# foolwood/SiamMask

Measured on AMD Instinct MI355X. Metric: frames/sec (255x255 search, 127x127 template), higher is better.
Workload: dtype f16

## Files before the change

siammask_amd/_lib.py:

```python
import ctypes
import os
import subprocess

import torch

_HERE = os.path.dirname(os.path.abspath(__file__))
LIB_PATH = os.environ.get("SMK_LIB") or os.path.join(_HERE, "libsiammask_hip.so")
CSRC = os.path.join(_HERE, "csrc")

DTYPE = {"f32": 0, "fp32": 0, "float32": 0, "f16": 1, "fp16": 1, "float16": 1, "half": 1,
         "f16x3": 2}
VARIANT = {"rpn": 0, "base": 1, "sharp": 2}
TRACK_BOX, TRACK_MASK, TRACK_NO_MASK_HEAD = 0, 1, 2
HP_STRIDE = 4

SYMBOLS = (
    "smk_version", "smk_last_error", "smk_create", "smk_destroy", "smk_set_weight",
    "smk_finalize_weights", "smk_template", "smk_track", "smk_refine", "smk_set_decode_params", "smk_decode", "smk_step", "smk_set_graph_mode", "smk_seq_status", "smk_seq_sync_check", "smk_set_result_ring", "smk_result_ring_cursor", "smk_set_pipeline", "smk_pipeline_join", "smk_pipeline_observe",
    "smk_debug_read", "smk_debug_seq_inject", "smk_tune", "smk_tune_get", "smk_profile", "smk_profile_dump", "smk_op_conv2d_ex", "smk_op_conv2d", "smk_op_dw_xcorr",
    "smk_op_maxpool3x3s2", "smk_op_stem_pool", "smk_op_l1_block", "smk_op_conv_seq", "smk_host_conv2d_ex", "smk_host_plan_conv", "smk_host_plan_seq", "smk_host_arena_elems", "smk_bench_conv", "smk_packed_size", "smk_export_packed",
    "smk_import_packed", "smk_crop_resize", "smk_paste_mask", "smk_paste_labels", "smk_mask_rbox_workspace", "smk_mask_rbox",
    "smk_trk_state_bytes", "smk_trk_set", "smk_trk_plan", "smk_trk_advance", "smk_crop_resize_dev", "smk_paste_mask_dev",
    "smk_vos_score", "smk_vos_score_dev", "smk_host_trk_plan", "smk_host_trk_advance",
    "smk_vos_score_ex", "smk_vos_score_dev_ex", "smk_label_rects", "smk_frame_sums", "smk_trk_start", "smk_crop_exemplar_dev",
    "smk_host_trk_start", "smk_vot_overlap", "smk_host_vot_overlap",
    "smk_crop_resize_dev_v", "smk_crop_exemplar_dev_v", "smk_frame_sums_v", "smk_trk_start_v", "smk_host_trk_start_v",
    "smk_paste_mask_dev_v", "smk_vot_overlap_dev",
    "smk_set_stream_hp", "smk_trk_advance_hp", "smk_host_trk_advance_hp",
)


class ConvGeom(ctypes.Structure):
    _fields_ = [(n, ctypes.c_int) for n in (
        "B", "Cin", "H", "W", "Cout", "k", "stride", "pad", "dil", "relu", "res_mode",
        "win", "ups", "Hl", "Wl", "org_y", "org_x", "pos_mul", "pos_add", "cin_off", "cin_len")]


class SeqOp(ctypes.Structure):
    _fields_ = [("g", ConvGeom), ("src", ctypes.c_int), ("res_src", ctypes.c_int), ("sync", ctypes.c_int),
                ("cfg", ctypes.c_int), ("kstag", ctypes.c_int), ("w_host", ctypes.c_void_p), ("b_host", ctypes.c_void_p),
                ("y_dev", ctypes.c_void_p)]


class TrkCfg(ctypes.Structure):
    _fields_ = [("context_amount", ctypes.c_double), ("lr", ctypes.c_double)] + [(n, ctypes.c_int) for n in (
        "exemplar_size", "instance_size", "total_stride", "base_size", "score_size", "mask_size")]


class ImageRef(ctypes.Structure):
    _fields_ = [("data", ctypes.c_void_p), ("row_bytes", ctypes.c_int64), ("w", ctypes.c_int32), ("h", ctypes.c_int32)]


class SmkError(RuntimeError):
    code = 0


E_SEQ = -6


def build_library(force=False, verbose=False):
    if force:
        subprocess.check_call(["make", "-C", CSRC, "clean"], stdout=subprocess.DEVNULL)
    out = subprocess.run(["make", "-C", CSRC, "-j", "4"], stdout=subprocess.PIPE,
                         stderr=subprocess.STDOUT, universal_newlines=True)
    if verbose or out.returncode != 0:
        print(out.stdout)
    if out.returncode != 0:
        raise SmkError("building libsiammask_hip.so failed")
    return LIB_PATH


_lib = None


def lib():
    global _lib
    if _lib is not None:
        return _lib
    if not os.path.exists(LIB_PATH):
        raise SmkError(
            "%s is missing: the HIP extension has not been built (run `python -c 'import "
            "__graft_entry__ as g; g.build()'` or `make -C siammask_amd/csrc`). There is no "
            "CPU fallback." % LIB_PATH)
    L = ctypes.CDLL(LIB_PATH)
    vp, ci, fp = ctypes.c_void_p, ctypes.c_int, ctypes.c_void_p
    L.smk_version.restype = ci
    L.smk_last_error.restype = ctypes.c_char_p
    L.smk_create.argtypes = [ctypes.POINTER(vp), ci, ci, ci, ci]
    L.smk_destroy.argtypes = [vp]
    L.smk_set_weight.argtypes = [vp, ctypes.c_char_p, fp, ctypes.POINTER(ctypes.c_int64), ci]
    L.smk_finalize_weights.argtypes = [vp]
    L.smk_template.argtypes = [vp, fp, ci, vp]
    L.smk_track.argtypes = [vp, fp, ci, ci, fp, fp, fp, vp]
    L.smk_refine.argtypes = [vp, vp, ci, ci, fp, vp]
    L.smk_set_decode_params.argtypes = [vp, fp, ci, ci, ctypes.c_double, ctypes.c_double]
    L.smk_decode.argtypes = [vp, fp, fp, ci, fp, vp, fp, vp]
    L.smk_step.argtypes = [vp, fp, ci, ci, fp, fp, fp, fp, fp, fp, vp]
    L.smk_set_graph_mode.argtypes = [vp, ci]
    L.smk_debug_seq_inject.argtypes = [vp, ci]
    L.smk_set_result_ring.argtypes = [vp, vp, vp, ci, ci]
    L.smk_set_pipeline.argtypes = [vp, ci]
    L.smk_pipeline_join.argtypes = [vp, vp]
    L.smk_pipeline_observe.argtypes = [vp, vp]
    L.smk_result_ring_cursor.argtypes = [vp, ctypes.POINTER(ci), ci, vp]
    L.smk_seq_sync_check.argtypes = [vp, vp, ctypes.POINTER(ci)]
    L.smk_tune.argtypes = [ctypes.c_char_p, ci]
    L.smk_tune_get.argtypes = [ctypes.c_char_p, ctypes.POINTER(ci)]
    L.smk_profile.argtypes = [vp, ci]
    L.smk_profile_dump.argtypes = [vp, ctypes.c_char_p, ci]
    ip = ctypes.POINTER(ci)
    L.smk_debug_read.argtypes = [vp, ctypes.c_char_p, fp, ip, ip, ip, vp]
    gp = ctypes.POINTER(ConvGeom)
    L.smk_op_conv2d_ex.argtypes = [ci, ci, gp, fp, fp, fp, fp, vp, fp, vp]
    L.smk_op_conv2d.argtypes = [ci, ci, fp, ci, ci, ci, ci, fp, fp, ci, ci, ci, ci, ci, ci, fp, fp, vp]
    L.smk_op_dw_xcorr.argtypes = [ci, fp, fp, ci, ci, ci, ci, ci, ci, fp, vp]
    L.smk_op_maxpool3x3s2.argtypes = [ci, fp, ci, ci, ci, ci, fp, vp]
    L.smk_op_stem_pool.argtypes = [fp, fp, fp, ci, ci, fp, fp, vp]
    L.smk_op_l1_block.argtypes = [fp] * 9 + [ci, ci, ci, fp, vp]
    L.smk_host_conv2d_ex.argtypes = [gp, fp, fp, fp, fp, vp, fp]
    L.smk_host_plan_conv.argtypes = [gp, ci, ci, ip, ip, ip, ip]
    L.smk_host_arena_elems.argtypes = [ci, ci, ci, ctypes.POINTER(ctypes.c_uint64)]
    L.smk_packed_size.argtypes = [vp, ctypes.POINTER(ctypes.c_uint64)]
    L.smk_export_packed.argtypes = [vp, vp, ctypes.c_uint64]
    L.smk_import_packed.argtypes = [vp, vp, ctypes.c_uint64]
    L.smk_crop_resize.argtypes = [vp, ctypes.c_int64, ci, ci, vp, vp, ci, ci, fp, vp]
    L.smk_paste_mask.argtypes = [fp, ci, vp, ci, ci, ci, ctypes.c_float, ctypes.c_float, vp, fp, vp]
    L.smk_paste_labels.argtypes = [fp, ci, vp, ci, ci, ci, ctypes.c_float, ctypes.c_float, vp, vp]
    L.smk_mask_rbox_workspace.argtypes = [ci, ci, ci]
    L.smk_mask_rbox.argtypes = [vp, ci, ci, ci, ctypes.c_double, vp, ctypes.c_size_t, vp, vp]
    cp = ctypes.POINTER(TrkCfg)
    L.smk_trk_state_bytes.argtypes = [ci]
    L.smk_trk_set.argtypes = [vp, ci, vp, vp, vp, ci, ci, vp]
    L.smk_trk_plan.argtypes = [vp, ci, cp, vp]
    L.smk_trk_advance.argtypes = [vp, ci, cp, vp, ci, vp, ci, vp]
    L.smk_host_trk_plan.argtypes = [vp, ci, cp]
    L.smk_host_trk_advance.argtypes = [vp, ci, cp, vp, ci, vp, ci]
    L.smk_crop_resize_dev.argtypes = [vp, ctypes.c_int64, ci, ci, vp, ci, ci, fp, vp]
    L.smk_paste_mask_dev.argtypes = [fp, fp, ci, ci, vp, ci, ci, ci, ci, ctypes.c_float, ctypes.c_float, vp, fp, vp]
    cf, u32 = ctypes.c_float, ctypes.c_uint32
    L.smk_vos_score.argtypes = [fp, ci, vp, ci, ci, ci, cf, vp, vp, u32, vp, ci, cf, vp, vp, vp]
    L.smk_vos_score_dev.argtypes = [fp, fp, ci, ci, vp, ci, ci, ci, ci, cf, vp, vp, u32, vp, ci, cf, vp, vp, vp]
    L.smk_vos_score_ex.argtypes = L.smk_vos_score.argtypes[:-1] + [u32, vp, vp]
    L.smk_vos_score_dev_ex.argtypes = L.smk_vos_score_dev.argtypes[:-1] + [u32, vp, vp]
    i64 = ctypes.c_int64
    L.smk_label_rects.argtypes = [vp, ci, ci, vp, ci, vp, vp]
    L.smk_frame_sums.argtypes = [vp, i64, ci, ci, ci, vp, vp]
    L.smk_trk_start.argtypes = [vp, ci, cp, u32, vp, vp, vp, vp, i64, ci, ci, vp, vp, vp]
    L.smk_host_trk_start.argtypes = [vp, ci, cp, u32, vp, vp, vp, vp, i64, ci, ci, vp, vp]
    L.smk_crop_exemplar_dev.argtypes = [vp, i64, ci, ci, vp, vp, vp, u32, ci, ci, fp, vp]
    L.smk_vot_overlap.argtypes = [vp, ci, vp, vp, ci, ci, ci, vp, vp, vp]
    L.smk_host_vot_overlap.argtypes = [vp, vp, ci, ci, ci, vp, vp]
    L.smk_crop_resize_dev_v.argtypes = [vp, vp, ci, ci, fp, vp]
    L.smk_crop_exemplar_dev_v.argtypes = [vp, vp, vp, vp, u32, ci, ci, fp, vp]
    L.smk_frame_sums_v.argtypes = [vp, ci, vp, vp]
    L.smk_trk_start_v.argtypes = [vp, ci, cp, u32, vp, vp, vp, vp, i64, vp, vp, vp, vp]
    L.smk_host_trk_start_v.argtypes = [vp, ci, cp, u32, vp, vp, vp, vp, i64, vp, vp, vp]
    L.smk_paste_mask_dev_v.argtypes = [fp, fp, ci, ci, vp, ci, ci, ci, ci, vp, cf, cf, vp, vp]
    L.smk_vot_overlap_dev.argtypes = [vp, ci, vp, vp, vp, ci, vp, vp, vp]
    L.smk_set_stream_hp.argtypes = [vp, vp]
    L.smk_trk_advance_hp.argtypes = [vp, ci, cp, vp, vp, ci, vp, ci, vp]
    L.smk_host_trk_advance_hp.argtypes = [vp, ci, cp, vp, vp, ci, vp, ci]
    L.smk_op_conv_seq.argtypes = [ctypes.POINTER(SeqOp), ci, fp, ci, ctypes.POINTER(ctypes.c_float), fp, ip, vp]
    L.smk_host_plan_seq.argtypes = [ctypes.POINTER(SeqOp), ci, ci, ip, ip, ip]
    L.smk_bench_conv.argtypes = [ci, ci, gp, ci, ci, ctypes.POINTER(ctypes.c_float), vp]
    for name in SYMBOLS:
        fn = getattr(L, name)
        if name not in ("smk_last_error",):
            fn.restype = ctypes.c_size_t if name in ("smk_mask_rbox_workspace", "smk_trk_state_bytes") else ci
    _lib = L
    for kv in filter(None, os.environ.get("SMK_TUNE", "").split(",")):
        k, v = kv.split("=")
        check(L.smk_tune(k.strip().encode(), int(v)))
    return L


def check(rc):
    if rc != 0:
        msg = lib().smk_last_error()
        e = SmkError("libsiammask_hip error %d: %s" % (rc, msg.decode() if msg else "?"))
        e.code = rc
        raise e


def current_stream_ptr():
    return ctypes.c_void_p(torch.cuda.current_stream().cuda_stream)


def tune(**kw):
    for k, v in kw.items():
        check(lib().smk_tune(k.encode(), int(v)))


def tune_get(key):
    v = ctypes.c_int(0)
    check(lib().smk_tune_get(key.encode(), ctypes.byref(v)))
    return v.value
```

siammask_amd/csrc/conv_plan.cpp:

```cpp
#include "conv_plan.h"

#include <algorithm>
#include <cstdio>
#include <cstdlib>
#include <cstring>

using namespace smk;

TileChoice tile_from_code(int code, const ConvParams &p, int dtype) {
    TileChoice t = choose_tile(p, dtype);
    static const int tb[6][2] = {{0, 0}, {128, 128}, {128, 64}, {64, 128}, {64, 64}, {256, 128}};
    const int tile = code & 15, kt = (code >> 4) & 3, st = (code >> 6) & 3;
    if (tile >= 1 && tile <= 5) {
        t.bm = tb[tile][0]; t.bn = tb[tile][1];
        t.kt = (t.bm == 64 && t.bn == 64) ? 256 : 128;
        t.stages = (t.bm == 128 && t.bn == 128) ? 2 : 3;
    }
    if (kt) t.kt = kt == 2 ? 256 : 128;
    if (t.bm == 64 && t.bn == 64) t.kt = 256;
    if (t.bm == 256) t.kt = 128;
    if (st) t.stages = st + 1;
    return t;
}

// ... 85 lines not shown
                (int)L[i].Kpad, (int)L[i].Nst, (int)L[i + 1].Nst, L[i].res, (int)L[i].relu, (int)L[i + 1].relu, (int)L[i + 1].Ho, (int)L[i + 1].Hs);
    return ok;
}
static bool seq_pair_fusable_why(const SeqLayer *L, int i, int *code, int *why) {
    const SeqLayer &a = L[i], &b = L[i + 1];
    auto plain1x1 = [](const SeqLayer &l) {
        return l.kh == 1 && l.kw == 1 && l.stride == 1 && l.stride_x == 1 && l.pad == 0 && l.org_y == 0 && l.org_x == 0 &&
               l.Hl == l.Hs && l.Wl == l.Ws && l.Ho == l.Hs && l.Wo == l.Ws && l.Ci == l.Kpad;
    };
    if (!plain1x1(a) || !a.sync) { *why = 1; return false; }
    if (!plain1x1(b)) { *why = 2; return false; }
    if (!a.res || a.res_mode != RES_PRE_RELU || !a.relu) { *why = 1; return false; }
    if (b.res || b.res_mode != RES_NONE) { *why = 3; return false; }
    if (b.in != a.out) { *why = 1; return false; }
    if (b.cin_off != a.cout_off || b.Cs != a.Cos || b.Ci != a.Nst || b.Hs != a.Ho || b.Ws != a.Wo) { *why = 4; return false; }
    if (b.out == a.out || b.out == a.res || b.out == a.in) { *why = 5; return false; }
    auto has_bar = [&](int k) { return L[k].sync && L[k].cfg != SEQ_CFG_C3C1_L3 && L[k].cfg != SEQ_CFG_C3C1_L2 && L[k].cfg != SEQ_CFG_C3C1P_L3 && L[k].cfg != SEQ_CFG_C3C1P_L2; };
    int pend = -1;
    for (int k = i - 1; k >= 0; --k)
        if (has_bar(k)) { pend = k; break; }
    for (int j = i - 1; j >= 0; --j)
        if (L[j].out == a.res) {
            bool passed = false;
            for (int k = j; k < pend; ++k) passed = passed || has_bar(k);
            if (!passed) { *why = 6; return false; }
            break;
        }
    for (int j = i - 1; j >= 0; --j)
        if (L[j].out == a.in) {
            if (j > pend) { *why = 7; return false; }
            break;
        }
    if (a.Kpad == 256 && a.Nst == 1024 && b.Nst == 256) *code = SEQ_CFG_C3C1_L3;
    else if (a.Kpad == 128 && a.Nst == 512 && b.Nst == 128) *code = SEQ_CFG_C3C1_L2;
    else { *why = 8; return false; }
    return true;
}

bool seq_pair_fits(const SeqLayer *L, int i, int B, int *code) {
    if (!seq_pair_fusable(L, i, code)) return false;
    const size_t px = (size_t)B * L[i].Ho * L[i].Wo;
    const size_t widest = std::max(std::max((size_t)L[i].Cs, (size_t)L[i].Cos), std::max((size_t)L[i].res_Cs, (size_t)L[i + 1].Cos));
    return px * widest * 2 < 0x7fff0000u && L[i].in_bytes < 0x7fff0000u;
}


static int seq_fuse_pairs(SeqLayer *L, int n, int B, const char *locked, bool have_xch) {
    if (!g_tune.seq_fuse) return 0;
    int fused = 0;
    for (int i = 0; i + 1 < n; ++i) {
        int code = 0;
        if (locked && (locked[i] || locked[i + 1])) continue;
        if (L[i].cfg >= SEQ_CFG_C3C1_L3 || L[i + 1].cfg >= SEQ_CFG_C3C1_L3 || !seq_pair_fits(L, i, B, &code)) continue;
        if (g_tune.seq_fuse == 2 && code != SEQ_CFG_C3C1_L3) continue;
        if (have_xch && g_tune.seq_pair2d && (g_tune.seq_pair2d == 1 || code == SEQ_CFG_C3C1_L3))
            code = code == SEQ_CFG_C3C1_L3 ? SEQ_CFG_C3C1P_L3 : SEQ_CFG_C3C1P_L2;
        L[i].cfg = (signed char)code;
        L[i + 1].cfg = (signed char)SEQ_CFG_C3C1_2ND;
        if (!(g_tune.seq_kstag_mask & 1)) L[i].kstag = 0;
        ++fused;
        ++i;
    }
    return fused;
}

static bool read_after_list(const std::vector<const void *> &read_after, const void *y) {
    return std::find(read_after.begin(), read_after.end(), y) != read_after.end();
}

static int seq_fuse_triples(SeqLayer *L, int i0, int i1, int n, const void *const *wstd, const char *locked,
                            const std::vector<const void *> &read_after) {
    if (!g_tune.seq_fuse3) return 0;
    auto group_has_bar = [&](int k) {
        const int cf = L[k].cfg;
        if (cf == SEQ_CFG_C3C1_L3 || cf == SEQ_CFG_C3C1_L2 || cf == SEQ_CFG_C3C1P_L3 || cf == SEQ_CFG_C3C1P_L2 || cf == SEQ_CFG_C2C3C1_L3 ||
            cf == SEQ_CFG_C2C3C1_L2 || cf == SEQ_CFG_C2C3C1_MID)
            return false;
        return L[k].sync != 0;
    };
    int fused = 0;
    for (int i = i0; i + 2 < i1; ++i) {
        SeqLayer &c2 = L[i], &c3 = L[i + 1], &c1 = L[i + 2];
        if (locked && (locked[i] || locked[i + 1] || locked[i + 2])) continue;
        if ((c3.cfg != SEQ_CFG_C3C1_L3 && c3.cfg != SEQ_CFG_C3C1_L2) || c1.cfg != SEQ_CFG_C3C1_2ND) continue;
        if (c2.cfg != SEQ_CFG_HALO128 && c2.cfg != SEQ_CFG_HALO64 && c2.cfg > 9) continue;
        const int code = c3.cfg == SEQ_CFG_C3C1_L3 ? SEQ_CFG_C2C3C1_L3 : SEQ_CFG_C2C3C1_L2;
        if (g_tune.seq_fuse3 == 2 && code != SEQ_CFG_C2C3C1_L3) continue;
        const int kc = c3.Kpad;
        if (c2.kh != 3 || c2.kw != 3 || c2.stride != 1 || c2.stride_x != 1 || c2.pad != c2.dil || c2.dil < 1 || c2.dil > 2) continue;
        if (c2.Ci != kc || c2.Nst != kc || c2.Kpad != 9 * kc || !c2.relu || c2.res || c2.res_mode != RES_NONE || !c2.sync) continue;
        if (c2.org_y || c2.org_x || c2.Hl != c2.Hs || c2.Wl != c2.Ws || c2.Ho != c2.Hs || c2.Wo != c2.Ws) continue;
        if (c2.Wo > 32 || c2.Wo < 24 || c2.Wo + 2 * c2.dil > 35) continue;
        if (c3.in != c2.out || c3.cin_off != c2.cout_off || c3.Cs != c2.Cos || c3.Hs != c2.Ho || c3.Ws != c2.Wo) continue;
        if (!wstd[i]) continue;
        bool other_reader = read_after_list(read_after, c2.out);
        for (int j = i + 2; j < n; ++j) {
            if (L[j].in == c2.out || L[j].res == c2.out) { other_reader = true; break; }
            if (L[j].out == c2.out) { other_reader = false; break; }
        }
        if (other_reader || c2.out == c3.res || c2.out == c1.out || c2.out == c3.out) continue;
        int pend = -1;
        for (int k = i - 1; k >= i0; --k)
            if (group_has_bar(k)) { pend = k; break; }
        bool in_ok = true;
        for (int j = i - 1; j >= i0; --j)
            if (L[j].out == c2.in) { in_ok = j <= pend; break; }
        if (!in_ok) continue;
        int res_late = 0;
        for (int j = i - 1; j >= i0; --j)
            if (L[j].out == c3.res) {
                bool passed = false;
                for (int k = j; k < pend; ++k) passed = passed || group_has_bar(k);
                const bool own_rows = L[j].cfg == SEQ_CFG_C2C3C1_MID && L[j].Ho == c3.Ho && L[j].Wo == c3.Wo;
                if (!passed && !own_rows) res_late = 1;
                break;
            }
        c2.cfg = (signed char)code;
        c2.wgt_frag = wstd[i];
        c2.sync = 0;
        c3.cfg = (signed char)SEQ_CFG_C2C3C1_MID;
        c3.a_stage = (signed char)res_late;
        ++fused;
        i += 2;
    }
    return fused;
}

static int seq_mark_resident(SeqLayer *L, int i0, int i1, int n, const SeqPlanEnv &env, const std::vector<const void *> &read_after) {
    if (!g_tune.seq_yres || env.B > 8) return 0;
    int prev = -1, marked = 0;
    for (int i = i0; i + 1 < i1; ++i) {
        const int cfg = L[i].cfg;
        if (cfg != SEQ_CFG_C3C1_L3 && cfg != SEQ_CFG_C3C1_L2) continue;
        const int p = prev;
        prev = i;
        if (p < 0 || L[p].cfg != cfg || i != p + 3) continue;
        const int mid = L[p + 2].cfg;
        if (mid != SEQ_CFG_HALO64 && mid != SEQ_CFG_HALO128) continue;
        if ((L[i].Ho * L[i].Wo + 31) / 32 > env.nslots || L[i].Ho != L[p].Ho || L[i].Wo != L[p].Wo) continue;
        if (L[i].res != L[p].out || L[i].res_Cs != L[p].Cos || L[i].res_coff != L[p].cout_off) continue;
        L[i].a_stage |= SEQ_YRES_IN;
        L[p + 2].a_stage |= SEQ_LDS_HI;
        ++marked;
        bool others = read_after_list(read_after, L[p].out);
        for (int j = 0; j < n && !others; ++j) {
            if (j != p + 1 && L[j].in == L[p].out) others = true;
            if (j != i && L[j].res == L[p].out) others = true;
        }
        if (!others) L[p].a_stage |= SEQ_YRES_NOSTORE;
    }
    return marked;
}

SeqPlanStats plan_seq(std::vector<SeqRec> &rec, const SeqPlanEnv &env, const char *locked, const std::vector<const void *> &read_after) {
    const int n = (int)rec.size();
    std::vector<SeqLayer> L(n);
    std::vector<const void *> wstd(n);
    for (int i = 0; i < n; ++i) { L[i] = rec[i].L; wstd[i] = rec[i].wstd; }
    const bool xch = env.have_xch && env.nslots % 2 == 0 && env.nslots / 2 <= SEQ_XCH_PAIRS;
    SeqPlanStats st;
    for (int i0 = 0; i0 < n; i0 += SEQ_MAX) {
        const int i1 = std::min(n, i0 + SEQ_MAX);
        st.pairs = seq_fuse_pairs(L.data() + i0, i1 - i0, env.B, locked ? locked + i0 : nullptr, xch);
        st.triples = seq_fuse_triples(L.data(), i0, i1, n, wstd.data(), locked, read_after);
        st.resident = seq_mark_resident(L.data(), i0, i1, n, env, read_after);
    }
    for (int i = 0; i < n; ++i) rec[i].L = L[i];
    return st;
}

double seq_fabric_bytes(const SeqLayer *L, int n, int B, const void *late_read) {
    double ext = 0.0;
    for (int i = 0; i < n; ++i) {
        const SeqLayer &l = L[i];
        bool in_inside = false, res_inside = l.res == nullptr, out_read = false;
        for (int j = 0; j < n; ++j) {
            if (j < i && L[j].out == l.in) in_inside = true;
            if (j < i && l.res && L[j].out == l.res) res_inside = true;
            if (j > i && (L[j].in == l.out || L[j].res == l.out)) out_read = true;
        }
        bool in_counted = false, res_counted = false;
        for (int j = 0; j < i; ++j) {
            if (L[j].in == l.in || L[j].res == l.in) in_counted = true;
            if (l.res && (L[j].in == l.res || L[j].res == l.res)) res_counted = true;
        }
        const double px_in = (double)B * l.Hs * l.Ws, px_out = (double)B * l.Ho * l.Wo;
        ext += (double)l.Nst * l.Kpad * 2.0;
        if (!in_inside && !in_counted) ext += px_in * l.Cs * 2.0;
        if (!res_inside && !res_counted) ext += px_out * l.res_Cs * 2.0;
        if (!out_read || l.out == late_read) ext += px_out * l.Nst * 2.0;
    }
    return ext;
}

const int WREG_TILE[9][2] = {{0, 0}, {64, 256}, {64, 128}, {64, 64}, {128, 256}, {128, 128}, {128, 64}, {96, 256}, {32, 64}};
int wreg_choice(const ConvParams &p, const ConvOpt &o, int dtype, long ncu) {
    if (o.algo_naive || !conv_wreg_eligible(p, dtype)) return 0;
    if (o.wreg) return o.wreg;
    if (g_tune.wreg >= 2) return g_tune.wreg - 1;
    if (!g_tune.wreg) return 0;
    const long K = (long)p.kh * p.kw * p.Ci;
    if (g_tune.wreg_policy == 1) {
        if (p.kh > 3) return 0;
        if (p.kh == 3 && p.stride == 1 && K <= 1152) return 0;
        if (p.M > 16384 && !(p.Nst >= 512 || (K >= 2304 && p.Nst >= 128) || (K >= 1024 && p.Nst >= 256) ||
                             (p.kh == 3 && p.stride == 2)))
            return 0;
        static const int cand[4] = {4, 1, 2, 3};
        const int nr = (p.Nst + 63) / 64 * 64, ng = p.groups > 0 ? p.groups : 1;
        for (int ci = 0; ci < 4; ++ci) {
            const int bm = WREG_TILE[cand[ci]][0], bn = WREG_TILE[cand[ci]][1];
            if (bn > nr && bn > 64) continue;
            if ((long)((p.M + bm - 1) / bm) * ((p.Nst + bn - 1) / bn) * ng >= 150) {
                if (cand[ci] == 4 && g_tune.wreg96) {
                    const long tn = (p.Nst + 255) / 256 * ng;
                    const long t128 = (long)((p.M + 127) / 128) * tn, t96 = (long)((p.M + 95) / 96) * tn;
                    if (((t128 + ncu - 1) / ncu) * 128 > ((t96 + ncu - 1) / ncu) * 96 && t96 <= 4 * ncu) return 7;
                }
                return cand[ci];
            }
        }
        if (g_tune.wreg32 && (long)((p.M + 63) / 64) * ((p.Nst + 63) / 64) * ng < g_tune.wreg32) return 8;
        return 3;
    }
    if (p.M < 4096) return 0;
    if (p.kh == 3 && K >= 2304 && p.Nst >= 512)
        return ((long)((p.M + 127) / 128) * ((p.Nst + 255) / 256) >= 200) ? 4 : 1;
    if (p.M > 16384) return 0;
    if (p.kh == 1 && K >= 512 && p.Nst <= 256) return p.Nst >= 192 ? 2 : 3;
    if (p.kh == 3 && p.stride == 2 && K >= 1152 && p.Nst <= 128) return 3;
    return 0;
}
int wreg_stages(int ctx_dtype, int B) {
    if (g_tune.wreg_stages) return g_tune.wreg_stages;
    return (ctx_dtype == DT_F16X3 || (B >= 1 && B <= 2)) ? 4 : 3;
}
int wreg_stages_from_code(int code) {
    const int st = (code >> 6) & 3;
    return st == 0 ? wreg_stages(DT_F16, 0) : (st == 1 ? 8 : (st == 2 ? 3 : 4));
}

bool pp_choice(const ConvParams &p, const ConvOpt &o, int dtype, long ncu) {
    if (!g_tune.pp || o.algo_naive || o.halo || o.wreg || o.tile_code || !conv_pp_eligible(p, dtype)) return false;
    const long K = (long)p.kh * p.kw * p.Ci;
    const long tiles = (long)((p.M + 255) / 256) * ((p.Nst + 255) / 256);
    const long rounds = (tiles + ncu - 1) / ncu;
    if (tiles < 200 || tiles * 10 < rounds * ncu * 9 || p.Nst < 256 || (p.Nst % 256) != 0) return false;
    return g_tune.pp == 2 || K >= 2304;
}

ConvPlan plan_conv(const ConvParams &p, const ConvOpt &o, const PackedConv &pc, int dtype, int B, long ncu) {
    const int kd = kdtype(dtype);
    ConvPlan pl;
    pl.tile = tile_from_code(o.tile_code, p, kd);
    if (o.algo_naive) { pl.kind = CK_NAIVE; return pl; }
    if (dtype == DT_F16 && g_tune.chain_mask != 2 && !o.tile_code && !o.halo && !o.wreg && mask_head_eligible(p, kd)) { pl.kind = CK_MHEAD; return pl; }
    int bm = halo_choice(pc, p, o, kd);
    if (bm && !o.halo && conv_ksplit(p, kd, pl.tile) > 1) bm = 0;
    if (pp_choice(p, o, kd, ncu)) { pl.kind = CK_PP; return pl; }
    const int wr = (o.halo || (bm && !o.wreg && g_tune.wreg < 2 && g_tune.wreg_policy == 0)) ? 0 : wreg_choice(p, o, kd, ncu);
    if (wr) {
        pl.kind = CK_WREG; pl.wreg = wr; pl.stages = wreg_stages(dtype, B);
    } else if (bm && conv_halo_eligible(p, kd, bm)) {
        pl.kind = CK_HALO; pl.halo_bm = bm;
    }
    return pl;
}

ConvPlan plan_conv_batch(const ConvBatch &cb, const ConvOpt *const o[], int lead, int dtype, int B, long ncu) {
    const int kd = kdtype(dtype);
    ConvPlan pl;
    int wr = wreg_choice(cb.p[lead], *o[lead], kd, ncu);
    for (int i = 0; i < cb.n && wr; ++i)
        if (!wreg_choice(cb.p[i], *o[i], kd, ncu) || (cb.p[i].groups > 1) != (cb.p[0].groups > 1)) wr = 0;
    if (wr) {
        pl.kind = CK_WREG; pl.wreg = wr; pl.stages = wreg_stages(dtype, B);
    } else {
        pl.tile = tile_from_code(o[lead]->tile_code, cb.p[lead], kd);
    }
    return pl;
}

std::string plan_kernel_name(const ConvPlan &pl, int dtype, int out_mode, int merged) {
    const char *dt = dtname(kdtype(dtype));
    char kn[80], mg[16] = "";
    if (merged) snprintf(mg, sizeof(mg), ",merged%d", merged);
    switch (pl.kind) {
    case CK_NAIVE: return "conv_naive";
    case CK_PP: return "conv_pp<f16,256x256>";
    case CK_MHEAD: return "mask_head<f16,128px,nchw>";
    case CK_HALO: snprintf(kn, sizeof(kn), "conv3x3_halo<%s,%dx128>", dt, pl.halo_bm); break;
    case CK_WREG: snprintf(kn, sizeof(kn), "conv_wreg<%s,%dx%d,s%d%s>", dt, WREG_TILE[pl.wreg][0], WREG_TILE[pl.wreg][1], pl.stages, mg); break;
    default:
        snprintf(kn, sizeof(kn), "conv_igemm<%s,%dx%dx%d,s%d,%s%s>", dt, pl.tile.bm, pl.tile.bn, pl.tile.kt, pl.tile.stages,
                 out_mode == OUT_NCHW_F32 ? "nchw" : "nhwc", mg);
    }
    return kn;
}
```

siammask_amd/csrc/conv_plan.h:

```cpp
#pragma once
#include <string>
#include <vector>

#include "smk_kernels.h"

struct Act {
    void *p = nullptr;
    int H = 0, W = 0, C = 0;
};

struct PackedConv {
    void *w = nullptr;
    void *w_halo = nullptr;
    void *w_frag = nullptr;
    void *w_frag_halo = nullptr;
    void *w_frag16 = nullptr;
    float *bias = nullptr;
    int N = 0;
    int rows = 0;
    int group_rows = 0;
    int groups = 1;
    int Ci = 0, k = 1, K = 0, Kpad = 0;
    int kw = 0;
    int alg_k = 0;
    float *oscale = nullptr;
    int x3_ct = 0, x3_nreal = 0;
    bool x3 = false;
};

struct ConvOpt {
    int stride = 1, pad = 0, dil = 1, relu = 0;
    int stride_x = 0;
    const Act *res = nullptr;
    int res_mode = smk::RES_NONE;
    int res_coff = 0;
    int cin_off = 0;
    int cout_off = 0;
    int n_override = 0;
    int groups = 1;
    bool win = false;
    int Hl = 0, Wl = 0, org_y = 0, org_x = 0;
    const int *pos = nullptr;
    int pos_mul = 0, pos_add = 0;
    bool ups = false;
    float *nchw_out = nullptr;
    int algo_naive = 0;
    int tile_code = 0;
    int halo = 0;
    int wreg = 0;
};

inline int kdtype(int dtype) { return dtype == smk::DT_F16X3 ? smk::DT_F16 : dtype; }
inline const char *dtname(int dt) { return dt == smk::DT_F16 ? "f16" : "f32"; }

#pragma GCC visibility push(hidden)

enum ConvKernel { CK_NAIVE, CK_IGEMM, CK_HALO, CK_WREG, CK_PP, CK_MHEAD };
struct ConvPlan {
    int kind = CK_IGEMM;
    smk::TileChoice tile{};
    int halo_bm = 0;
    int wreg = 0;
    int stages = 0;
};

extern const int WREG_TILE[9][2];

smk::TileChoice tile_from_code(int code, const smk::ConvParams &p, int dtype);
int halo_choice(const PackedConv &pc, const smk::ConvParams &p, const ConvOpt &o, int dtype);
int wreg_choice(const smk::ConvParams &p, const ConvOpt &o, int dtype, long ncu);
int wreg_stages(int ctx_dtype, int B);
int wreg_stages_from_code(int code);
bool pp_choice(const smk::ConvParams &p, const ConvOpt &o, int dtype, long ncu);

ConvPlan plan_conv(const smk::ConvParams &p, const ConvOpt &o, const PackedConv &pc, int dtype, int B, long ncu);
ConvPlan plan_conv_batch(const smk::ConvBatch &cb, const ConvOpt *const *o, int lead, int dtype, int B, long ncu);
std::string plan_kernel_name(const ConvPlan &pl, int dtype, int out_mode, int merged = 0);

bool seq_halo_ok(const smk::ConvParams &p, int bm);
bool seq_layer_from(const smk::ConvParams &p, int dtype, smk::SeqLayer &L, int force_halo = 0);
bool seq_pair_fusable(const smk::SeqLayer *L, int i, int *code);
bool seq_pair_fits(const smk::SeqLayer *L, int i, int B, int *code);

struct SeqRec {
    smk::SeqLayer L;
    const void *wstd = nullptr;
    std::string id;
};
struct SeqPlanEnv {
    int B = 0;
    int nslots = 0;
    bool have_xch = false;
};
struct SeqPlanStats { int pairs = 0, triples = 0, resident = 0; };

SeqPlanStats plan_seq(std::vector<SeqRec> &rec, const SeqPlanEnv &env, const char *locked, const std::vector<const void *> &read_after);
double seq_fabric_bytes(const smk::SeqLayer *L, int n, int B, const void *late_read);

#pragma GCC visibility pop
```

siammask_amd/csrc/conv_seq.hip:

```cpp
#include <hip/hip_runtime.h>
#include <type_traits>
#include "smk_kernels.h"

namespace smk {

#include "wreg_tile.inc"
#include "c3c1_tile.inc"
#ifdef SMK_MEASURE
#include "c3c1p_tile.inc"
#endif
#include "c3c1s_tile.inc"
#include "wreg_halo_tile.inc"

#ifndef SMK_HALO_D128
#define SMK_HALO_D128 3
#endif
#ifndef SMK_HALO_SB128
#define SMK_HALO_SB128 0
#endif
constexpr int HALO_D128 = SMK_HALO_D128, HALO_SB128 = SMK_HALO_SB128, HALO_D64 = 6;
constexpr int SEQ_POLL_TID = 256;
constexpr int SEQ_CLK2_STRIDE = 12;

__device__ __forceinline__ void seq_raise(const SeqArgs &a, int code) {
    __hip_atomic_store(a.err, code, __ATOMIC_RELAXED, __HIP_MEMORY_SCOPE_AGENT);
    if (a.err_host) __hip_atomic_store(a.err_host, code, __ATOMIC_RELAXED, __HIP_MEMORY_SCOPE_SYSTEM);
}

__device__ __forceinline__ void team_arrive(unsigned *cnt) {
    asm volatile("s_waitcnt vmcnt(0) lgkmcnt(0)" ::: "memory");
    __builtin_amdgcn_s_barrier();
    asm volatile("" ::: "memory");
    if (threadIdx.x == SEQ_POLL_TID)
        __hip_atomic_fetch_add(cnt, 1u, __ATOMIC_RELAXED, __HIP_MEMORY_SCOPE_WORKGROUP);
}

__device__ __forceinline__ unsigned team_poll(const unsigned *cnt, bool spoll) {
    if (spoll) {
        unsigned v;
        asm volatile("s_load_dword %0, %1, 0x0 glc\n\ts_waitcnt lgkmcnt(0)" : "=s"(v) : "s"(cnt) : "memory");
        return v;
    }
    return __hip_atomic_load(cnt, __ATOMIC_RELAXED, __HIP_MEMORY_SCOPE_AGENT);
}

struct TeamWait {
    const SeqArgs *a;
    unsigned *cnt;
    unsigned target;
    int *abort_sh;
    __device__ __forceinline__ bool operator()() const {
        if (target == 0) return true;
        if (threadIdx.x == SEQ_POLL_TID) {
            const unsigned long long t0 = wall_clock64();
            while (team_poll(cnt, (a->flags & 1) != 0) < target) {
                __builtin_amdgcn_s_sleep(1);
                if (wall_clock64() - t0 > 20000000ull) {
                    seq_raise(*a, 2);
                    *abort_sh = 1;
                    break;
                }
            }
        }
        asm volatile("s_waitcnt lgkmcnt(0)" ::: "memory");
        __builtin_amdgcn_s_barrier();
        asm volatile("" ::: "memory");
        return *(__attribute__((address_space(3))) volatile int *)abort_sh == 0;
    }
};

template <int NPW, int CLK = 0, int T3 = 0>
__global__ __launch_bounds__((4 + NPW) * 64, 1) void conv_seq_kernel(const SeqArgs a) {
    constexpr int SEQ_LDS0 = (!T3 || WregLds<4, 3>::v > C3C1Lds<256, 1024, 256>::vx) ? WregLds<4, 3>::v : C3C1Lds<256, 1024, 256>::vx;
    constexpr int SEQ_LDS = SEQ_LDS0 > SEQ_YRES_BYTES + 2 * HALO_PB ? SEQ_LDS0 : SEQ_YRES_BYTES + 2 * HALO_PB;
    static_assert(4 * 64 * 68 * 4 <= 2 * HALO_PB && C3C1Lds<256, 1024, 256>::A_OFF == SEQ_YRES_BYTES && C3C1Lds<128, 512, 128>::A_OFF <= SEQ_YRES_BYTES, "resident Y");
    __shared__ __attribute__((aligned(16))) unsigned char smem[SEQ_LDS];
    static_assert(C3C1Lds<256, 1024, 256>::v <= WregLds<4, 3>::v && C3C1Lds<128, 512, 128>::vx <= SEQ_LDS && SEQ_LDS + 64 <= 160 * 1024, "LDS of the fused tiles");
    static_assert(NPW == 4, "c3c1_tile computes on all eight waves");
    __shared__ int ctl[4];
    const int nslots = gridDim.x >> 3;
    unsigned xcc;
    asm volatile("s_getreg_b32 %0, hwreg(HW_REG_XCC_ID)" : "=s"(xcc));
    const int team = (int)(xcc & 7);
    unsigned *cnt = a.bar + team * 32;
    if (threadIdx.x == 0) {
        const unsigned t = __hip_atomic_fetch_add(cnt + 2, 1u, __ATOMIC_RELAXED, __HIP_MEMORY_SCOPE_WORKGROUP);
        const int e = __hip_atomic_load(a.err, __ATOMIC_RELAXED, __HIP_MEMORY_SCOPE_AGENT);
        ctl[0] = (int)t;
        ctl[1] = e;
        ctl[2] = 0;
    }
    __syncthreads();
    const int slot = ctl[0];
    if (ctl[1]) return;
    if (slot >= nslots) {
        if (threadIdx.x == 0) seq_raise(a, 1);
        return;
    }
    unsigned pending = 0;
    const bool clk = CLK != 0 && a.clk && team == 0 && slot == 0 && threadIdx.x == 0;
    if (clk) a.clk[0] = wall_clock64();
    bool alive = true;
    for (int li = 0; li < a.n && alive; ++li) {
        const SeqLayer &L = a.L[li];
        const int cfg = L.cfg;
        const bool fusedp = cfg == SEQ_CFG_C3C1P_L3 || cfg == SEQ_CFG_C3C1P_L2;
        const bool fused = cfg == SEQ_CFG_C3C1_L3 || cfg == SEQ_CFG_C3C1_L2;
        const bool fused3 = cfg == SEQ_CFG_C2C3C1_L3 || cfg == SEQ_CFG_C2C3C1_L2;
        const bool halo = cfg == SEQ_CFG_HALO128 || cfg == SEQ_CFG_HALO64;
        const int bn = (cfg == 0 || cfg == 3 || cfg == 16 || cfg == 17) ? 256 : ((cfg == 2 || cfg == 9 || cfg == 18) ? 64 : 128);
        const int bm = (cfg == 3 || cfg == 4 || cfg == 9 || cfg == 16) ? 128 : 64;
        const int tilesN = (L.Nst + bn - 1) / bn;
        const int hw = L.Ho * L.Wo;
        const int halo_rpt = halo ? (cfg == SEQ_CFG_HALO128 ? 128 : 64) / L.Wo : 1;
        const int halo_tn = (L.Nst + 63) >> 6;
        const int tiles = fused3 ? L.Ho : fused ? (hw + 31) / 32 : (halo ? ((L.Ho + halo_rpt - 1) / halo_rpt) * halo_tn : ((hw + bm - 1) / bm) * tilesN);
#ifdef SMK_MEASURE
        if (T3 != 0 && fusedp) {
            const int npairs = nslots >> 1, pr = slot >> 1, hcu = slot & 1;
            int rt = (hw + npairs - 1) / npairs;
            if (rt > 64) rt = 64;
            const int ptiles = (hw + rt - 1) / rt;
            float *slabs = (float *)((unsigned char *)a.xch + (size_t)((team * SEQ_XCH_PAIRS + pr) * 4) * SEQ_XCH_SLAB);
            for (int img = team; img < a.B && alive; img += 8)
                for (int t = pr; t < ptiles && alive; t += npairs) {
                    unsigned long long *tclk = nullptr;
                    if constexpr (CLK != 0)
                        tclk = (a.clk2 && team == 0 && slot == 0 && img == team && t == pr) ? a.clk2 + SEQ_CLK2_STRIDE * li : nullptr;
                    const TeamWait w{&a, cnt, pending, &ctl[2]};
                    pending = 0;
                    const int fm0 = img * hw + t * rt;
                    int fme = fm0 + rt;
                    if (fme > (img + 1) * hw) fme = (img + 1) * hw;
                    if constexpr (T3 != 0) {
                    if (cfg == SEQ_CFG_C3C1P_L3)
                        alive = c3c1p_tile<256, 1024, 256, CLK>(L, a.L[li + 1], fm0, fme, a.B * hw, hcu, pr, npairs, cnt + 8 + pr, slabs, a, &ctl[2], &ctl[3], smem, tclk, w);
                    else
                        alive = c3c1p_tile<128, 512, 128, CLK>(L, a.L[li + 1], fm0, fme, a.B * hw, hcu, pr, npairs, cnt + 8 + pr, slabs, a, &ctl[2], &ctl[3], smem, tclk, w);
                    }
                }
        } else
#endif
        {
        const int nk = L.Kpad >> 6;
        const int kt0 = L.kstag ? (slot * nk) / nslots : 0;
        for (int img = team; img < a.B && alive; img += 8)
            for (int t = slot; t < tiles && alive; t += nslots) {
                const int tm = t / tilesN, tn = t - tm * tilesN;
                const int m0 = img * hw + tm * bm, m_end = (img + 1) * hw;
                unsigned long long *tclk = nullptr;
                if constexpr (CLK != 0)
                    tclk = (a.clk2 && team == 0 && slot == 0 && img == team && t == slot) ? a.clk2 + SEQ_CLK2_STRIDE * li : nullptr;
                const TeamWait w{&a, cnt, pending, &ctl[2]};
                pending = 0;
                if constexpr (T3 != 0)
                if (fused3) {
                    const int fm0 = img * hw + t * L.Wo;
                    if (cfg == SEQ_CFG_C2C3C1_L3) alive = c3c1_tile<256, 1024, 256, CLK, TeamWait, 1>(a.L[li + 1], a.L[li + 2], fm0, fm0 + L.Wo, a.B * hw, slot, nslots, smem, tclk, w, &L, img, t);
                    else alive = c3c1_tile<128, 512, 128, CLK, TeamWait, 1>(a.L[li + 1], a.L[li + 2], fm0, fm0 + L.Wo, a.B * hw, slot, nslots, smem, tclk, w, &L, img, t);
                }
                if (T3 != 0 && fused3) {}
                else if (fused) {
                    const int fm0 = img * hw + t * 32;
                    if (cfg == SEQ_CFG_C3C1_L3) alive = c3c1_tile<256, 1024, 256, CLK>(L, a.L[li + 1], fm0, m_end, a.B * hw, slot, nslots, smem, tclk, w);
                    else alive = c3c1_tile<128, 512, 128, CLK>(L, a.L[li + 1], fm0, m_end, a.B * hw, slot, nslots, smem, tclk, w);
                }
                else if (halo) {
                    const int ty = t / halo_tn, hn0 = (t - ty * halo_tn) * 64;
                    const bool hi = (L.a_stage & SEQ_LDS_HI) != 0;
                    unsigned char *hsm = smem + (hi ? SEQ_YRES_BYTES : 0);
                    if (cfg == SEQ_CFG_HALO128) alive = wreg_halo_tile<4, NPW, HALO_D128, HALO_SB128, CLK>(L, img, ty, hn0, hsm, tclk, slot, nslots, w, hi);
                    else alive = wreg_halo_tile<2, NPW, HALO_D64, 0, CLK>(L, img, ty, hn0, hsm, tclk, slot, nslots, w, hi);
                }
                else if (cfg == 0) alive = wreg_tile<2, 4, 1, 3, 16, 2, NPW, CLK>(L, 0, m0, m_end, tn * 256, smem, tclk, kt0, w);
                else if (cfg == 1) alive = wreg_tile<2, 2, 2, 3, 16, 2, NPW, CLK>(L, 0, m0, m_end, tn * 128, smem, tclk, kt0, w);
                else if (cfg == 3) alive = wreg_tile<4, 4, 1, 3, 16, 1, NPW, CLK>(L, 0, m0, m_end, tn * 256, smem, tclk, kt0, w);
                else if (cfg == 4) alive = wreg_tile<4, 2, 2, 3, 16, 1, NPW, CLK>(L, 0, m0, m_end, tn * 128, smem, tclk, kt0, w);
                else if (T3 != 0 && cfg == 9) { if constexpr (T3 != 0) alive = wreg_tile<4, 1, 4, 3, 16, 2, NPW, CLK>(L, 0, m0, m_end, tn * 64, smem, tclk, kt0, w); }
                else if (T3 != 0 && cfg == 5) { if constexpr (T3 != 0) alive = wreg_tile<2, 2, 2, 5, 16, 4, NPW, CLK>(L, 0, m0, m_end, tn * 128, smem, tclk, kt0, w); }
#ifdef SMK_MEASURE
                else if (cfg == 6) alive = wreg_tile<2, 2, 2, 3, 16 | 0x100, 2, NPW, CLK>(L, 0, m0, m_end, tn * 128, smem, tclk, kt0, w);
                else if (cfg == 7) alive = wreg_tile<2, 2, 2, 3, 16 | 0x200, 2, NPW, CLK>(L, 0, m0, m_end, tn * 128, smem, tclk, kt0, w);
                else if (cfg == 8) alive = wreg_tile<2, 2, 2, 3, 16 | 0x400, 2, NPW, CLK>(L, 0, m0, m_end, tn * 128, smem, tclk, kt0, w);
                else if (cfg == 10) alive = wreg_tile<2, 2, 2, 3, 16 | 0x300, 2, NPW, CLK>(L, 0, m0, m_end, tn * 128, smem, tclk, kt0, w);
                else if (cfg == 11) alive = wreg_tile<2, 2, 2, 3, 16 | 0x700, 2, NPW, CLK>(L, 0, m0, m_end, tn * 128, smem, tclk, kt0, w);
                else if (cfg == 12) alive = wreg_tile<2, 2, 2, 3, 16 | 0x1700, 2, NPW, CLK>(L, 0, m0, m_end, tn * 128, smem, tclk, kt0, w);
                else if (cfg == 13) alive = wreg_tile<2, 2, 2, 3, 16 | 0x800, 2, NPW, CLK>(L, 0, m0, m_end, tn * 128, smem, tclk, kt0, w);
                else if (cfg == 14) alive = wreg_tile<2, 2, 2, 3, 16 | 0x1000, 2, NPW, CLK>(L, 0, m0, m_end, tn * 128, smem, tclk, kt0, w);
                else if (cfg == 15) alive = wreg_tile<2, 2, 2, 3, 16 | 0x2000, 2, NPW, CLK>(L, 0, m0, m_end, tn * 128, smem, tclk, kt0, w);
                else if (cfg == 16) alive = wreg_tile<4, 4, 1, 3, 16 | 0x2000, 1, NPW, CLK>(L, 0, m0, m_end, tn * 256, smem, tclk, kt0, w);
                else if (cfg == 17) alive = wreg_tile<2, 4, 1, 3, 16 | 0x2000, 2, NPW, CLK>(L, 0, m0, m_end, tn * 256, smem, tclk, kt0, w);
                else if (cfg == 18) alive = wreg_tile<2, 1, 4, 3, 16 | 0x2000, 2, NPW, CLK>(L, 0, m0, m_end, tn * 64, smem, tclk, kt0, w);
#endif
                else alive = wreg_tile<2, 1, 4, 3, 16, 2, NPW, CLK>(L, 0, m0, m_end, tn * 64, smem, tclk, kt0, w);
            }
        }
        if (clk) a.clk[1 + 2 * li] = wall_clock64();
        if (!alive) break;
        if (fused3) {
            if (clk) a.clk[2 + 2 * li] = a.clk[3 + 2 * li] = a.clk[4 + 2 * li] = a.clk[5 + 2 * li] = wall_clock64();
            li += 2;
        }
        if (fused || fusedp) {
            if (clk) a.clk[2 + 2 * li] = a.clk[3 + 2 * li] = wall_clock64();
            ++li;
        }
        if (a.L[li].bar_ord) {
            if (pending) {
                const TeamWait w{&a, cnt, pending, &ctl[2]};
                pending = 0;
                if (!w()) break;
            }
            team_arrive(cnt);
            if constexpr (CLK != 0) {
                if (a.clk2 && team == 0 && threadIdx.x == 0) a.clk2[SEQ_CLK2_STRIDE * SEQ_MAX + li * 32 + slot] = wall_clock64();
            }
            pending = (unsigned)a.L[li].bar_ord * (unsigned)nslots;
        }
        if (clk) a.clk[2 + 2 * li] = wall_clock64();
    }
    if (!alive || ctl[2]) return;
    asm volatile("s_waitcnt vmcnt(0) lgkmcnt(0)" ::: "memory");
    __syncthreads();
    if (threadIdx.x == 0) {
        const unsigned prev = __hip_atomic_fetch_add(cnt + 1, 1u, __ATOMIC_RELAXED, __HIP_MEMORY_SCOPE_WORKGROUP);
        if (prev == (unsigned)nslots - 1) {
            __hip_atomic_store(cnt, 0u, __ATOMIC_RELAXED, __HIP_MEMORY_SCOPE_WORKGROUP);
            __hip_atomic_store(cnt + 1, 0u, __ATOMIC_RELAXED, __HIP_MEMORY_SCOPE_WORKGROUP);
            __hip_atomic_store(cnt + 2, 0u, __ATOMIC_RELAXED, __HIP_MEMORY_SCOPE_WORKGROUP);
            for (int i = 8; i < 32; ++i) __hip_atomic_store(cnt + i, 0u, __ATOMIC_RELAXED, __HIP_MEMORY_SCOPE_WORKGROUP);
            if (a.exit_sem) {
                const unsigned t = __hip_atomic_fetch_add(a.exit_sem + 1, 1u, __ATOMIC_RELAXED, __HIP_MEMORY_SCOPE_AGENT);
                if (t == 7u) {
                    __hip_atomic_store(a.exit_sem + 1, 0u, __ATOMIC_RELAXED, __HIP_MEMORY_SCOPE_AGENT);
                    __hip_atomic_fetch_add(a.exit_sem, 1u, __ATOMIC_RELAXED, __HIP_MEMORY_SCOPE_AGENT);
                }
            }
        }
    }
}

template <int K3, int N3, int N1>
__global__ __launch_bounds__(512, 1) void conv_pair_kernel(const SeqLayer L3, const SeqLayer L1, const int M) {
    __shared__ __attribute__((aligned(16))) unsigned char smem[C3C1Lds<K3, N3, N1>::v];
    const int m0 = (int)blockIdx.x * 32;
    (void)c3c1_tile<K3, N3, N1, 0>(L3, L1, m0, M, M, (int)(blockIdx.x & 31), 32, smem, nullptr, NoHoist());
}

template <int K3, int N3, int N1>
__global__ __launch_bounds__(512, 1) void conv_pair64_kernel(const SeqLayer L3, const SeqLayer L1, const int M) {
    __shared__ __attribute__((aligned(16))) unsigned char smem[C3C1SLds<K3, N3, N1>::v];
    c3c1s_tile<K3, N3, N1>(L3, L1, (int)blockIdx.x * 64, M, M, smem);
}

int launch_conv_pair(const SeqLayer &L3, const SeqLayer &L1, int code, int M, void *stream, int rows) {
    if (M < 1 || (code != SEQ_CFG_C3C1_L3 && code != SEQ_CFG_C3C1_L2) || (rows != 32 && rows != 64)) return -1;
    if (rows == 64) {
        const dim3 grid64((M + 63) / 64), block64(512);
        if (code == SEQ_CFG_C3C1_L3) hipLaunchKernelGGL((conv_pair64_kernel<256, 1024, 256>), grid64, block64, 0, (hipStream_t)stream, L3, L1, M);
        else hipLaunchKernelGGL((conv_pair64_kernel<128, 512, 128>), grid64, block64, 0, (hipStream_t)stream, L3, L1, M);
        return hipGetLastError() == hipSuccess ? 0 : -4;
    }
    const dim3 grid((M + 31) / 32), block(512);
    if (code == SEQ_CFG_C3C1_L3) hipLaunchKernelGGL((conv_pair_kernel<256, 1024, 256>), grid, block, 0, (hipStream_t)stream, L3, L1, M);
    else hipLaunchKernelGGL((conv_pair_kernel<128, 512, 128>), grid, block, 0, (hipStream_t)stream, L3, L1, M);
    return hipGetLastError() == hipSuccess ? 0 : -4;
}

__global__ void xcc_census_kernel(int *out) {
    unsigned xcc;
    asm volatile("s_getreg_b32 %0, hwreg(HW_REG_XCC_ID)" : "=s"(xcc));
    if (threadIdx.x == 0) out[blockIdx.x] = (int)(xcc & 0xf);
}

int launch_conv_seq(const SeqArgs &a_in, int grid, void *stream) {
    if (a_in.n < 1 || a_in.n > SEQ_MAX || grid < 8 || (grid & 7) || !a_in.bar || !a_in.err) return -1;
    SeqArgs a = a_in;
    unsigned short ord = 0;
    for (int li = 0; li < a.n; ++li) {
        const int cfg = a.L[li].cfg;
        a.L[li].bar_ord = 0;
        const bool first = cfg == SEQ_CFG_C3C1_L3 || cfg == SEQ_CFG_C3C1_L2 || cfg == SEQ_CFG_C3C1P_L3 || cfg == SEQ_CFG_C3C1P_L2;
        if (cfg == SEQ_CFG_C2C3C1_L3 || cfg == SEQ_CFG_C2C3C1_L2) {
            if (li + 2 >= a.n) return -1;
            if (a.L[li + 1].cfg != SEQ_CFG_C2C3C1_MID || a.L[li + 2].cfg != SEQ_CFG_C3C1_2ND) return -1;
            if (a.L[li].Wo + 2 * a.L[li].dil > 35 || a.L[li].Wo > 32) return -1;
            continue;
        }
        if (cfg == SEQ_CFG_C2C3C1_MID) {
            const int pc = li ? a.L[li - 1].cfg : -1;
            if (pc != SEQ_CFG_C2C3C1_L3 && pc != SEQ_CFG_C2C3C1_L2) return -1;
            continue;
        }
        if (first) {
            if (li + 1 >= a.n || a.L[li + 1].cfg != SEQ_CFG_C3C1_2ND) return -1;
            if ((cfg == SEQ_CFG_C3C1P_L3 || cfg == SEQ_CFG_C3C1P_L2) && (!a.xch || (grid >> 3) % 2 || (grid >> 4) > SEQ_XCH_PAIRS)) return -1;
            continue;
        }
        if (cfg == SEQ_CFG_C3C1_2ND) {
            const int pc = li ? a.L[li - 1].cfg : -1;
            if (pc != SEQ_CFG_C3C1_L3 && pc != SEQ_CFG_C3C1_L2 && pc != SEQ_CFG_C3C1P_L3 && pc != SEQ_CFG_C3C1P_L2 && pc != SEQ_CFG_C2C3C1_MID) return -1;
        }
        if (a.L[li].sync && li + 1 < a.n) a.L[li].bar_ord = ++ord;
    }
    bool triples = false;
    for (int li = 0; li < a.n; ++li) {
        const int cf = a.L[li].cfg;
        triples = triples || cf == SEQ_CFG_C2C3C1_L3 || cf == SEQ_CFG_C2C3C1_L2 || cf == SEQ_CFG_C3C1P_L3 || cf == SEQ_CFG_C3C1P_L2 || cf == 5 || cf == 9;
    }
    if (triples) {
#ifdef SMK_MEASURE
        if (a.clk || a.clk2) hipLaunchKernelGGL((conv_seq_kernel<4, 1, 1>), dim3(grid), dim3(512), 0, (hipStream_t)stream, a);
        else hipLaunchKernelGGL((conv_seq_kernel<4, 0, 1>), dim3(grid), dim3(512), 0, (hipStream_t)stream, a);
#else
        return -5;
#endif
    } else if (a.clk || a.clk2)
        hipLaunchKernelGGL((conv_seq_kernel<4, 1>), dim3(grid), dim3(512), 0, (hipStream_t)stream, a);
    else hipLaunchKernelGGL((conv_seq_kernel<4, 0>), dim3(grid), dim3(512), 0, (hipStream_t)stream, a);
    return hipGetLastError() == hipSuccess ? 0 : -4;
}

int conv_seq_occupancy() {
    int nb = 0;
    if (hipOccupancyMaxActiveBlocksPerMultiprocessor(&nb, conv_seq_kernel<4, 0>, 512, 0) != hipSuccess) return 0;
    return nb;
}

int xcc_census(int grid, int *out_host) {
    int *d = nullptr;
    if (hipMalloc((void **)&d, sizeof(int) * grid) != hipSuccess) return -4;
    hipLaunchKernelGGL(xcc_census_kernel, dim3(grid), dim3(384), 0, 0, d);
    hipError_t e = hipMemcpy(out_host, d, sizeof(int) * grid, hipMemcpyDeviceToHost);
    hipFree(d);
    return e == hipSuccess ? 0 : -4;
}

}
```

siammask_amd/csrc/engine.cpp:

```cpp
#include <hip/hip_runtime_api.h>

#include <cmath>
#include <cstdarg>
#include <tuple>
#include <cstdio>
#include <cstdlib>
#include <cstring>
#include <functional>
#include <map>
#include <memory>
#include <string>
#include <vector>

#include "../../include/siammask_hip.h"
#include "../../include/siammask_hip_test.h"
#include "conv_plan.h"
#include "smk_kernels.h"
#include "tracker_state.h"
#include "vot_overlap.h"

using namespace smk;

static thread_local std::string g_err;

// ... 614 lines not shown
    HIPCHK(hipMemset(c->buf[id][copy], 0, bytes));
    return 0;
}

static int alloc_copies(smk_ctx *c, int depth) {
    for (int id = 0; id < T_COUNT; ++id)
        if (ARENA[id].twice_from && depth >= ARENA[id].twice_from && !c->buf[id][1]) CHK(alloc_buf(c, id, 1));
    return 0;
}

static int build_arena(smk_ctx *c) {
    uint64_t total = 0;
    CHK(arena_elems(c->dtype, c->variant, 0, &total));
    for (int id = 0; id < T_COUNT; ++id) {
        const ArenaRow &t = ARENA[id];
        if (t.refine && c->variant != SMK_VARIANT_SHARP) continue;
        if (row_aliased(t, c->dtype)) c->buf[id][0] = c->buf[t.alias][0];
        else CHK(alloc_buf(c, id, 0));
    }
    HIPCHK(hipMalloc((void **)&c->pos_dev, sizeof(int) * 2 * c->maxB));
    HIPCHK(hipMemset(c->pos_dev, 0, sizeof(int) * 2 * c->maxB));
    HIPCHK(hipMalloc((void **)&c->ks_part, KS_PART_FLOATS * sizeof(float)));
    HIPCHK(hipMalloc((void **)&c->ks_cnt, KS_CNT * sizeof(unsigned)));
    HIPCHK(hipMalloc((void **)&c->seq_bar, 8 * 32 * sizeof(unsigned)));
    HIPCHK(hipMemset(c->seq_bar, 0, 8 * 32 * sizeof(unsigned)));
    HIPCHK(hipMalloc((void **)&c->seq_err, sizeof(int)));
    HIPCHK(hipMemset(c->seq_err, 0, sizeof(int)));
    if (c->dtype == DT_F16) {
        HIPCHK(hipMalloc((void **)&c->seq_xch, SEQ_XCH_BYTES));
        HIPCHK(hipMemset(c->seq_xch, 0, SEQ_XCH_BYTES));
    }
    HIPCHK(hipHostMalloc((void **)&c->seq_err_host, 64, hipHostMallocMapped));
    *c->seq_err_host = 0;
    HIPCHK(hipHostGetDevicePointer((void **)&c->seq_err_hdev, c->seq_err_host, 0));
    HIPCHK(hipMemset(c->ks_cnt, 0, KS_CNT * sizeof(unsigned)));
    HIPCHK(hipMalloc(&c->dec_scratch, (size_t)c->maxB * DEC_SCRATCH_PER_STREAM));
    HIPCHK(hipMemset(c->dec_scratch, 0, (size_t)c->maxB * DEC_SCRATCH_PER_STREAM));
    return 0;
}

static int act(Act &a, smk_ctx *c, int id, int H = 0, int W = 0) {
    const ArenaRow &t = ARENA[id];
    const bool second = c->parity_now && t.twice_from && (t.twice_from == 1 || c->pipe_depth >= t.twice_from);
    a.p = c->buf[id][second ? 1 : 0];
    a.H = H > 0 ? H : t.H;
    a.W = H > 0 ? W : t.W;
    a.C = t.C * (t.per_branch ? nbranch(c) : 1) * ((c->dtype == DT_F16X3 && !t.refine) ? X3_PLANES : 1);
    if (!a.p || a.W < 1 || (size_t)a.H * a.W > (size_t)t.H * t.W)
        return fail(SMK_E_STATE, "internal: view %d x %d of arena tensor %s (%d x %d, copy %d)", a.H, a.W, t.name, t.H, t.W, (int)second);
    return 0;
}
#define ACT(...) ({ Act a_; CHK(act(a_, __VA_ARGS__)); a_; })
static int branch_off(const smk_ctx *c, int g) { return g * 256 * (c->dtype == DT_F16X3 ? X3_PLANES : 1); }

struct ConvEnv {
    int dtype = DT_F32, device = 0;
    float *ks_part = nullptr;
    unsigned *ks_cnt = nullptr;
    int wave_prio = 0;
};
static ConvEnv conv_env(const smk_ctx *c) { return {c->dtype, c->device, c->ks_part, c->ks_cnt, c->wave_prio_now}; }

static int conv_params(const ConvEnv &env, const PackedConv &pc, const Act &in, const Act *out, int B,
                       const ConvOpt &o, ConvParams &p) {
    memset(&p, 0, sizeof(p));
    p.in = in.p;
    p.wgt = pc.w;
    p.wgt_frag = pc.w_frag;
    p.wgt_frag_halo = pc.w_frag_halo;
    p.bias = pc.bias;
    p.oscale = pc.oscale;
    p.pos = o.pos;
    p.B = B;
    p.Hs = in.H; p.Ws = in.W; p.Cs = in.C;
    p.cin_off = o.cin_off;
    p.Ci = pc.Ci;
    p.x3_ct = pc.x3_ct; p.x3_nreal = pc.x3_nreal;
    p.x3_in = pc.x3 ? pc.Ci / 3 : 0;
    p.Hl = (o.win || o.ups) ? o.Hl : in.H;
    p.Wl = (o.win || o.ups) ? o.Wl : in.W;
    p.org_y = o.org_y; p.org_x = o.org_x;
    p.pos_mul = o.pos_mul; p.pos_add = o.pos_add;
    p.ups = o.ups ? 1 : 0;
    p.kh = pc.k;
    p.kw = pc.kw ? pc.kw : pc.k;
    p.stride = o.stride; p.pad = o.pad; p.dil = o.dil;
    p.stride_x = o.stride_x ? o.stride_x : o.stride;
    p.Ho = (p.Hl + 2 * o.pad - o.dil * (p.kh - 1) - 1) / p.stride + 1;
    p.Wo = (p.Wl + 2 * o.pad - o.dil * (p.kw - 1) - 1) / p.stride_x + 1;
    p.K = pc.K; p.Kpad = pc.Kpad;
    p.N = o.n_override ? o.n_override : pc.N;
    p.M = B * p.Ho * p.Wo;
    p.relu = o.relu;
    p.groups = o.groups;
    if (o.groups > 1) {
        p.g_cin_off = pc.x3 ? pc.Ci / 3 * X3_PLANES : pc.Ci;
        p.g_wgt_off = pc.group_rows;
        p.g_cout_off = pc.group_rows * (pc.x3 ? X3_PLANES : 1);
    }
    if (o.nchw_out) {
        p.out = o.nchw_out;
        p.out_mode = OUT_NCHW_F32;
        p.Nst = rup(p.N, 4);
    } else {
        if (!out) return fail(SMK_E_ARG, "conv without output");
        if (out->H != p.Ho || out->W != p.Wo)
            return fail(SMK_E_ARG, "internal: conv output %dx%d != buffer %dx%d", p.Ho, p.Wo, out->H, out->W);
        p.out = out->p;
        p.out_mode = OUT_NHWC;
        p.Cos = out->C;
        p.cout_off = o.cout_off;
        p.Nst = rup(p.N, 8);
        if (pc.x3) {
            p.x3_out = o.groups > 1 ? pc.group_rows : out->C / X3_PLANES;
            if (out->C % X3_PLANES || o.cout_off + (o.groups - 1) * X3_PLANES * pc.group_rows + p.x3_out + p.Nst > out->C)
                return fail(SMK_E_ARG, "internal: split conv output channels exceed buffer");
        } else if (o.cout_off + (o.groups - 1) * pc.group_rows + p.Nst > out->C)
            return fail(SMK_E_ARG, "internal: conv output channels exceed buffer");
    }
    p.xcd_mode = g_tune.xcd_mode;
    if (o.nchw_out && g_tune.nchw_tn_major && p.xcd_mode == 1 && p.M >= 20000 && (double)p.M * p.N * 4 >= 4.0e6) p.xcd_mode = 2;
    p.prio = g_tune.prio;
    p.wave_prio = env.wave_prio;
    {
        const double ib = (double)B * in.H * in.W * in.C * esize(env.dtype), wb = (double)pc.rows * pc.Kpad * esize(env.dtype);
        p.buf_lds = (g_tune.buf_lds && ib < 2.0e9 && wb < 2.0e9) ? 1 : 0;
        p.a_stage = g_tune.a_stage;
        p.res_nt = g_tune.res_nt;
        p.in_bytes = (unsigned)(ib < 4.0e9 ? ib : 0);
        p.w_bytes = (unsigned)(wb < 4.0e9 ? wb : 0);
    }
    p.nt_store = (g_tune.nt_store && o.nchw_out && (double)p.M * p.N * 4 >= 4.0e6) ? 1 : 0;
    p.ci_shift = -1;
    for (int sh = 0; sh < 16; ++sh)
        if ((1 << sh) == p.Ci) p.ci_shift = sh;
    p.kw_magic = 65536 / p.kw + 1;
    p.zero = env.device >= 0 ? zero_page() : nullptr;
    if (env.device >= 0 && !p.zero) return fail(SMK_E_HIP, "could not allocate the zero page");
    if (o.res) {
        p.res = o.res->p;
        p.res_Cs = o.res->C;
        p.res_coff = o.res_coff;
        p.res_mode = o.res_mode;
        if (pc.x3) p.x3_res = o.res->C / X3_PLANES;
    }
    p.ksplit = 1;
    p.ks_part = env.ks_part;
    p.ks_cnt = env.ks_cnt;
    p.ks_part_cap = env.ks_part ? KS_PART_FLOATS : 0;
    p.ks_cnt_cap = env.ks_cnt ? KS_CNT : 0;
    return 0;
}

static SeqPlanStats g_seq_last;

static void seq_print_clk(const SeqArgs &a, const SeqRec *r, const char *idn, const unsigned long long *h,
                          const unsigned long long *h2) {
    fprintf(stderr, "[seq clk] %s total %.2f us\n", idn, (h[2 * a.n] - h[0]) / 100.0);
    for (int i = 0; i < a.n; ++i)
        fprintf(stderr, "[seq clk]   %-10s cfg %d sync %d kstag %d  tiles %.2f us  arrive %.2f us\n", r[i].id.c_str(), a.L[i].cfg,
                a.L[i].sync, a.L[i].kstag, (h[1 + 2 * i] - h[2 * i]) / 100.0, (h[2 + 2 * i] - h[1 + 2 * i]) / 100.0);
    if (!h2) return;
    for (int i = 0; i < a.n; ++i) {
        const unsigned long long *ar = h2 + 12 * SEQ_MAX + 32 * i;
        unsigned long long mn = ~0ull, mx = 0;
        int nz = 0;
        double sum = 0.0;
        for (int q = 0; q < 32; ++q)
            if (ar[q]) { mn = std::min(mn, ar[q]); mx = std::max(mx, ar[q]); ++nz; }
        if (nz < 2) continue;
        for (int q = 0; q < 32; ++q)
            if (ar[q]) sum += (double)(mx - ar[q]);
        unsigned long long rel = 0;
        for (int j = i + 1; j < a.n && !rel; ++j) rel = h2[12 * j + 7];
        fprintf(stderr, "[seq arrive] %-10s %2d workgroups: first -> last arrival %.2f us, mean wait for the last one %.2f us, last arrival -> slot 0 "
                "released %.2f us\n", r[i].id.c_str(), nz, (mx - mn) / 100.0, sum / nz / 100.0, rel > mx ? (rel - mx) / 100.0 : -1.0);
    }
    for (int i = 0; i < a.n; ++i) {
        const unsigned long long *t = h2 + 12 * i;
        if (!t[0] || !t[6]) continue;
        const double us = (t[6] - t[0]) / 100.0;
        if (a.L[i].cfg == SEQ_CFG_C3C1P_L3 || a.L[i].cfg == SEQ_CFG_C3C1P_L2) {
            fprintf(stderr, "[seq clk2]  %-10s first tile (pair split, fused with the next 1x1): team wait %.2f | activation rows -> LDS %.2f | "
                    "conv3 K loop %.2f | residual -> Y %.2f | Y = relu(..) %.2f | Y stores + second K loop + slab + arrive %.2f | partner wait + add %.2f | "
                    "stores %.2f us | %.0f MHz\n",
                    r[i].id.c_str(), (t[7] - t[0]) / 100.0, (t[1] - t[7]) / 100.0, (t[2] - t[1]) / 100.0, (t[3] - t[2]) / 100.0,
                    (t[4] - t[3]) / 100.0, (t[5] - t[4]) / 100.0, (t[10] - t[5]) / 100.0, (t[6] - t[10]) / 100.0, us > 0 ? (double)(t[9] - t[8]) / us : 0.0);
            continue;
        }
        if (a.L[i].cfg == SEQ_CFG_C2C3C1_L3 || a.L[i].cfg == SEQ_CFG_C2C3C1_L2) {
            fprintf(stderr, "[seq clk2]  %-10s first tile (3x3 + conv3 + the next 1x1): prologue + team wait %.2f | patch -> LDS + conv2 %.2f | "
                    "conv3 K loop %.2f | residual -> Y %.2f | Y = relu(..) %.2f | Y stores + second K loop %.2f | its epilogue + stores %.2f us | %.0f MHz\n",
                    r[i].id.c_str(), (t[7] - t[0]) / 100.0, (t[1] - t[7]) / 100.0, (t[2] - t[1]) / 100.0, (t[3] - t[2]) / 100.0,
                    (t[4] - t[3]) / 100.0, (t[5] - t[4]) / 100.0, (t[6] - t[5]) / 100.0, us > 0 ? (double)(t[9] - t[8]) / us : 0.0);
            continue;
        }
        if (a.L[i].cfg == SEQ_CFG_C3C1_L3 || a.L[i].cfg == SEQ_CFG_C3C1_L2) {
            fprintf(stderr, "[seq clk2]  %-10s first tile (fused with the next 1x1): team wait %.2f | activation rows -> LDS %.2f | "
                    "conv3 K loop %.2f | residual -> Y %.2f | Y = relu(..) %.2f | Y stores + second K loop %.2f | its epilogue + stores %.2f us | %.0f MHz\n",
                    r[i].id.c_str(), (t[7] - t[0]) / 100.0, (t[1] - t[7]) / 100.0, (t[2] - t[1]) / 100.0, (t[3] - t[2]) / 100.0,
                    (t[4] - t[3]) / 100.0, (t[5] - t[4]) / 100.0, (t[6] - t[5]) / 100.0, us > 0 ? (double)(t[9] - t[8]) / us : 0.0);
            continue;
        }
        fprintf(stderr, "[seq clk2]  %-10s first tile: prologue %.2f | team wait %.2f | first operands %.2f | K loop %.2f | other waves %.2f | "
                "acc -> LDS %.2f | bias/res/stores %.2f | end sync %.2f us | %.0f MHz\n", r[i].id.c_str(),
                t[7] ? (t[7] - t[0]) / 100.0 : 0.0, 0.0, t[7] ? (t[1] - t[7]) / 100.0 : (t[1] - t[0]) / 100.0, (t[2] - t[1]) / 100.0,
                (t[3] - t[2]) / 100.0, (t[4] - t[3]) / 100.0, (t[5] - t[4]) / 100.0, (t[6] - t[5]) / 100.0,
                us > 0 ? (double)(t[9] - t[8]) / us : 0.0);
    }
}

static int seq_flush(smk_ctx *c, StepRec &rec, int B, hipStream_t s) {
    const size_t n = c->seq.rec.size();
    if (!n) return 0;
    const void *p2 = ACT(c, T_P2).p;
    std::vector<const void *> read_after{p2};
    for (int id : {c->p3_id, (int)T_SEARCH, (int)T_ZF, (int)T_XS}) read_after.push_back(ACT(c, id).p);
    g_seq_last = plan_seq(c->seq.rec, {B, c->seq_grid >> 3, c->seq_xch != nullptr}, nullptr, read_after);
    for (size_t i0 = 0; i0 < n; i0 += SEQ_MAX) {
        SeqArgs a;
        memset(&a, 0, sizeof(a));
        a.n = (int)(n - i0 < (size_t)SEQ_MAX ? n - i0 : SEQ_MAX);
        a.B = B;
        a.flags = g_tune.seq_spoll ? 1 : 0;
        a.bar = c->seq_bar;
        a.xch = c->seq_xch;
        a.err = c->seq_err;
        a.err_host = c->seq_err_hdev;
        a.exit_sem = (rec.seq_exit && i0 + SEQ_MAX >= n) ? c->pipe_cnt + 7 : nullptr;
        if (a.exit_sem) rec.seq_exit_done = true;
        const SeqRec *r = c->seq.rec.data() + i0;
        for (int i = 0; i < a.n; ++i) a.L[i] = r[i].L;
        const char *ck = getenv("SMK_SEQ_CLK");
        const bool want_clk = ck != nullptr && !c->graph_mode;
        const bool want_clk2 = want_clk && !strcmp(ck, "2");
        if (want_clk && !c->seq_clk) HIPCHK(hipMalloc((void **)&c->seq_clk, sizeof(unsigned long long) * (2 * SEQ_MAX + 1)));
        if (want_clk2 && !c->seq_clk2) HIPCHK(hipMalloc((void **)&c->seq_clk2, sizeof(unsigned long long) * (12 + 32) * SEQ_MAX));
        if (want_clk2) HIPCHK(hipMemsetAsync(c->seq_clk2, 0, sizeof(unsigned long long) * (12 + 32) * SEQ_MAX, s));
        a.clk = want_clk ? c->seq_clk : nullptr;
        a.clk2 = want_clk2 ? c->seq_clk2 : nullptr;
        char idn[96];
        snprintf(idn, sizeof(idn), "seq[%s..%s]", r[0].id.c_str(), r[a.n - 1].id.c_str());
        const double fr = (double)a.n / (double)n;
        ProfScope ps(c, s, idn, "conv_seq", c->seq.flop * fr, c->seq.bytes * fr);
        ps.ext_bytes(seq_fabric_bytes(a.L, a.n, B, p2));
        if (launch_conv_seq(a, c->seq_grid, s))
            return fail(SMK_E_HIP, "launch of %s failed: %s", idn, hipGetErrorString(hipGetLastError()));
        c->seq_pending = rec.has_seq = true;
        if (want_clk) {
            unsigned long long h[2 * SEQ_MAX + 1], h2[(12 + 32) * SEQ_MAX];
            HIPCHK(hipStreamSynchronize(s));
            HIPCHK(hipMemcpy(h, c->seq_clk, sizeof(h), hipMemcpyDeviceToHost));
            if (want_clk2) HIPCHK(hipMemcpy(h2, c->seq_clk2, sizeof(h2), hipMemcpyDeviceToHost));
            seq_print_clk(a, r, idn, h, want_clk2 ? h2 : nullptr);
        }
    }
    c->seq.clear();
    return 0;
}

static int seq_health(smk_ctx *c) {
    if (!c->seq_err_host) return 0;
    const int e = *(volatile int *)c->seq_err_host;
    if (!e) return 0;
    (void)hipDeviceSynchronize();
    c->seq_fail = e;
    if (e != 3) c->seq_grid = 0;
    else c->pipe_depth = 0;
    if (c->pipe_cnt) {
        const unsigned init[16] = {1u, 0u};
        (void)hipMemcpy(c->pipe_cnt, init, sizeof(init), hipMemcpyHostToDevice);
    }
    *(volatile int *)c->seq_err_host = 0;
    (void)hipMemset(c->seq_err, 0, sizeof(int));
    (void)hipMemset(c->seq_bar, 0, 8 * 32 * sizeof(unsigned));
    for (auto &kv : c->graphs) hipGraphExecDestroy(kv.second);
    c->graphs.clear();
    c->graph_used.clear();
    c->graph_has_seq.clear();
    c->seq_pending = false;
    c->tail_pending = false;
    c->tail2_pending = false;
    c->template_B = 0;
    c->track_B = 0;
    if (e == 3)
        return fail(SMK_E_SEQ, "conv_seq_kernel reported: (pipelined step) a gate waited 0.2 s (a tail's gate: 5 s) for its partner on the other stream -- something serialises "
                    "the two queues of this context (a profiler collecting counters does); the results of the calls enqueued on this context "
                    "since then are invalid (the cached template included) and frame steps are serial from here on: call template() again and "
                    "re-submit the frame");
    return fail(SMK_E_SEQ, "conv_seq_kernel reported %s: the results of the calls enqueued on this context since then are invalid "
                "(the cached template included); persistent sequences are now off for this context (per-layer kernels from here "
                "on): call template() again and re-submit the frame",
                e == 1 ? "an uneven distribution of workgroups over the XCDs" : "a team-barrier time-out (another kernel held CUs "
                "for more than 0.2 s, or a second persistent kernel ran beside it)");
}

static bool seq_wanted(const smk_ctx *c, int B) {
    if (!g_tune.seq || c->seq_grid <= 0 || c->dtype != DT_F16) return false;
    if (B >= g_tune.seq_min_batch && B <= g_tune.seq_max_batch) return true;
    if (B == g_tune.seq_extra_batch) return true;
    return B % 8 == 0 && B <= g_tune.seq_mult_max;
}

static void conv_work(const PackedConv &pc, const ConvParams &p, int B, int dtype, double &flop, double &bytes) {
    const int ng = p.groups > 0 ? p.groups : 1;
    const double kreal = pc.alg_k ? (double)pc.alg_k : (double)p.kh * p.kw * p.Ci;
    const size_t es = esize(kdtype(dtype));
    flop += 2.0 * p.M * (double)p.N * kreal * ng;
    bytes += (double)B * (p.ups ? p.Hs * p.Ws : (double)p.Hl * p.Wl) * p.Ci * es * ng + (double)p.M * p.N * ng * (p.out_mode == OUT_NCHW_F32 ? 4 : es) +
             (double)p.N * kreal * es * ng + (p.res ? (double)p.M * p.N * es : 0.0);
}

static int launch_plan(const ConvPlan &pl, ConvBatch &cb, const void *w_halo, int dtype, hipStream_t s, const char *what) {
    int rc;
    switch (pl.kind) {
    case CK_PP: rc = launch_conv_pp(cb.p[0], s); break;
    case CK_WREG: rc = launch_conv_wreg_batch(cb, WREG_TILE[pl.wreg][0], WREG_TILE[pl.wreg][1], pl.stages, s); break;
    case CK_HALO: {
        ConvParams ph = cb.p[0];
        ph.wgt = w_halo;
        rc = launch_conv_halo(ph, dtype, pl.halo_bm, s);
        break;
    }
    case CK_NAIVE: rc = launch_conv_naive(cb.p[0], dtype, s); break;
    case CK_MHEAD: rc = launch_mask_head(cb.p[0], s); break;
    default: rc = launch_conv_mfma_batch(cb, dtype, pl.tile, s);
    }
    if (rc == 1) return fail(SMK_E_STATE, "internal: %s is not eligible for the kernel planned for it", what);
    if (rc) return fail(SMK_E_HIP, "launch of %s failed: %s", what, hipGetErrorString(hipGetLastError()));
    return 0;
}

static int run_conv(smk_ctx *c, const char *id, const Act &in, const Act *out, int B, const ConvOpt &o,
                    hipStream_t s, StepRec *rec = nullptr) {
    auto it = c->conv.find(id);
    if (it == c->conv.end()) return fail(SMK_E_STATE, "internal: conv %s not packed", id);
    ConvBatch cb;
    cb.n = 1;
    ConvParams &p = cb.p[0];
    CHK(conv_params(conv_env(c), it->second, in, out, B, o, p));
    double flop = 0.0, bytes = 0.0;
    conv_work(it->second, p, B, c->dtype, flop, bytes);
    if (c->seq_on) {
        SeqLayer L;
        if (!o.algo_naive && !o.halo && !o.wreg && !o.tile_code && seq_layer_from(p, kdtype(c->dtype), L)) {
            c->seq.rec.push_back({L, p.wgt_frag, id});
            c->seq.flop += flop;
            c->seq.bytes += bytes;
            return 0;
        }
        if (!rec) return fail(SMK_E_STATE, "internal: conv %s recorded into a sequence without a step record", id);
        CHK(seq_flush(c, *rec, B, s));
    }
    const ConvPlan pl = plan_conv(p, o, it->second, c->dtype, B, c->ncu);
    ProfScope ps(c, s, id, plan_kernel_name(pl, c->dtype, p.out_mode), flop, bytes);
    char what[80];
    snprintf(what, sizeof(what), "conv %s", id);
    return launch_plan(pl, cb, it->second.w_halo, kdtype(c->dtype), s, what);
}

struct ConvJob { const char *id; const Act *in; const Act *out; ConvOpt o; };

static int run_conv_jobs(smk_ctx *c, const std::vector<ConvJob> &jobs, int B, int lead, hipStream_t s, StepRec *rec = nullptr) {
    if (jobs.empty() || (int)jobs.size() > CONV_BATCH_MAX) return fail(SMK_E_ARG, "internal: bad conv job count");
    if (c->seq_on) {
        const size_t n0 = c->seq.rec.size();
        for (auto &j : jobs) CHK(run_conv(c, j.id, *j.in, j.out, B, j.o, s, rec));
        if (c->seq.rec.size() == n0 + jobs.size())
            for (size_t i = n0; i + 1 < c->seq.rec.size(); ++i) c->seq.rec[i].L.sync = 0;
        return 0;
    }
    ConvBatch cb;
    cb.n = (int)jobs.size();
    bool split_for_halo = g_tune.halo != 0;
    int n_halo = 0;
    for (int i = 0; i < cb.n; ++i) {
        auto it = c->conv.find(jobs[i].id);
        if (it == c->conv.end()) return fail(SMK_E_STATE, "internal: conv %s not packed", jobs[i].id);
        CHK(conv_params(conv_env(c), it->second, *jobs[i].in, jobs[i].out, B, jobs[i].o, cb.p[i]));
        const int bm = halo_choice(it->second, cb.p[i], jobs[i].o, kdtype(c->dtype));
        if (bm) ++n_halo;
        if (bm == 64 || (bm == 0 && cb.p[i].kh == 3)) split_for_halo = false;
    }
    const bool merge_ok = g_tune.merge && (g_tune.merge == 2 || B <= g_tune.merge_max_batch);
    if ((c->prof && !c->prof_merge) || cb.n == 1 || !merge_ok || (split_for_halo && n_halo)) {
        for (auto &j : jobs) CHK(run_conv(c, j.id, *j.in, j.out, B, j.o, s));
        return 0;
    }
    double mflop = 0.0, mbytes = 0.0;
    std::string mid;
    const ConvOpt *opts[CONV_BATCH_MAX];
    for (int i = 0; i < cb.n; ++i) {
        opts[i] = &jobs[i].o;
        if (!c->prof) continue;
        conv_work(c->conv.find(jobs[i].id)->second, cb.p[i], B, c->dtype, mflop, mbytes);
        mid += (i ? "+" : "") + std::string(jobs[i].id);
    }
    const ConvPlan pl = plan_conv_batch(cb, opts, lead, c->dtype, B, c->ncu);
    ProfScope ps(c, s, mid.c_str(), plan_kernel_name(pl, c->dtype, cb.p[lead].out_mode, cb.n), mflop, mbytes);
    char what[80];
    snprintf(what, sizeof(what), "merged conv %s..", jobs[0].id);
    return launch_plan(pl, cb, nullptr, kdtype(c->dtype), s, what);
}

static int run_conv_pair(smk_ctx *c, const char *id3, const Act &in3, const Act &out3, const ConvOpt &o3, const char *id1,
                         const Act &out1, const ConvOpt &o1, int B, hipStream_t s) {
    if (c->dtype != DT_F16 || !g_tune.pair_launch || c->seq_on || (c->prof && !c->prof_merge)) return 1;
    if (g_tune.pair_launch == 1 && B < 3) return 1;
    const int pair_rows = g_tune.pair_launch == 3 ? 64 : (g_tune.pair_launch == 2 ? 32 : (B >= 9 ? 64 : 32));
    auto i3 = c->conv.find(id3), i1 = c->conv.find(id1);
    if (i3 == c->conv.end() || i1 == c->conv.end() || o1.win || o1.ups || o1.pos) return 1;
    ConvParams p3, p1;
    if (conv_params(conv_env(c), i3->second, in3, &out3, B, o3, p3) || conv_params(conv_env(c), i1->second, out3, &out1, B, o1, p1)) return 1;
    SeqLayer L[2];
    if (!seq_layer_from(p3, c->dtype, L[0], -1) || !seq_layer_from(p1, c->dtype, L[1], -1)) return 1;
    int code = 0;
    if (!seq_pair_fits(L, 0, B, &code)) return 1;
    const size_t es = esize(c->dtype);
    const double flop = 2.0 * p3.M * ((double)p3.N * p3.Ci + (double)p1.N * p1.Ci);
    const double bytes = ((double)p3.M * (p3.Ci + 2.0 * p3.N + p1.N) + (double)p3.N * p3.Ci + (double)p1.N * p1.Ci) * es;
    char kn[48];
    snprintf(kn, sizeof(kn), "conv_pair<f16,%d-%d-%d>", p3.Ci, p3.N, p1.N);
    const std::string pid = std::string(id3) + "+" + id1;
    ProfScope ps(c, s, pid.c_str(), kn, flop, bytes);
    if (launch_conv_pair(L[0], L[1], code, p3.M, s, pair_rows)) return fail(SMK_E_HIP, "launch of pair %s failed: %s", pid.c_str(), hipGetErrorString(hipGetLastError()));
    return 0;
}

enum { PH_FRONT = 1, PH_BACK = 2, PH_ALL = 3 };
static int run_backbone(smk_ctx *c, StepRec &rec, const float *x, int B, int S, hipStream_t s, int phase = PH_ALL, int search_nb = 0,
                        bool *search_done = nullptr) {
    const int s0 = (S - 7) / 2 + 1;
    const int s1 = (s0 + 2 - 3) / 2 + 1;
    const int s2 = (s1 - 3) / 2 + 1;
    Act p0 = ACT(c, T_P0, s0, s0);
    Act x1 = ACT(c, T_X1, s1, s1);
    auto stem_it = c->conv.find("stem");
    if (stem_it == c->conv.end()) return fail(SMK_E_STATE, "internal: conv stem not packed");
    if (!(phase & PH_FRONT)) {
    } else if (c->dtype == DT_F16 && g_tune.stem_fused && stem_it->second.w_frag) {
        StemPoolParams sp_{x, stem_it->second.w_frag, stem_it->second.bias, p0.p, x1.p, B, S, s0, s1, stem_it->second.Kpad, c->wave_prio_now};
        ProfScope ps(c, s, "stem_pool", "stem_pool", 2.0 * B * s0 * s0 * 64.0 * 147.0,
                     (double)B * (3.0 * S * S * 4 + ((double)s0 * s0 + (double)s1 * s1) * 64 * 2));
        if (launch_stem_pool(sp_, s)) return fail(SMK_E_HIP, "stem_pool launch failed: %s", hipGetErrorString(hipGetLastError()));
    } else if (c->dtype == DT_F16X3) {
        Act xin = ACT(c, T_XIN, S, S);
        CvtInParams ci{x, xin.p, B, 3, S, S, 8, 0, 1};
// ... 726 lines not shown
    return 0;
}

int smk_seq_sync_check(smk_ctx *c, void *stream, int *synced) {
    if (synced) *synced = 0;
    if (!c) return fail(SMK_E_ARG, "ctx is NULL");
    if (!c->seq_pending) return 0;
    HIPCHK(hipSetDevice(c->device));
    HIPCHK(hipStreamSynchronize((hipStream_t)stream));
    if (synced) *synced = 1;
    c->seq_pending = false;
    return seq_health(c);
}

int smk_set_graph_mode(smk_ctx *c, int enable) {
    if (!c) return fail(SMK_E_ARG, "ctx is NULL");
    c->graph_mode = enable != 0;
    return 0;
}

int smk_template(smk_ctx *c, const float *z, int B, void *stream) {
    if (!c || !z) return fail(SMK_E_ARG, "smk_template: null argument");
    if (!c->finalized) return fail(SMK_E_STATE, "smk_template: weights not finalized");
    if (B < 1 || B > c->maxB) return fail(SMK_E_ARG, "smk_template: batch %d not in [1,%d]", B, c->maxB);
    HIPCHK(hipSetDevice(c->device));
    CHK(seq_health(c));
    hipStream_t s = (hipStream_t)stream;
    CHK(pipe_join(c, s, true));
    c->parity_now = c->last_parity = 0;
    GraphKey key{0, B, 0, {z}};
    StepRec rec;
    int rc = run_maybe_graph(c, key, s, rec, [&](hipStream_t st) { return seq_template(c, rec, z, B, st); });
    if (rc) return rc;
    c->template_B = B;
    c->track_B = 0;
    return 0;
}

int smk_track(smk_ctx *c, const float *x, int B, int flags, float *cls, float *loc, float *mask, void *stream) {
    if (!c || !x || !cls || !loc) return fail(SMK_E_ARG, "smk_track: null argument");
    if (!c->finalized) return fail(SMK_E_STATE, "smk_track: weights not finalized");
    if (c->template_B == 0) return fail(SMK_E_STATE, "smk_track: smk_template has not been called");
    if (B != c->template_B)
        return fail(SMK_E_ARG, "smk_track: batch %d != template batch %d (models/rpn.py:33 requires equality)", B,
                    c->template_B);
    if ((flags & SMK_TRACK_MASK) && c->variant == SMK_VARIANT_RPN)
        return fail(SMK_E_ARG, "smk_track: the rpn variant has no mask branch");
    if ((flags & SMK_TRACK_MASK) && !(flags & SMK_TRACK_NO_MASK_HEAD) && !mask)
        return fail(SMK_E_ARG, "smk_track: mask_out is NULL");
    HIPCHK(hipSetDevice(c->device));
    CHK(seq_health(c));
    hipStream_t s = (hipStream_t)stream;
    CHK(pipe_join(c, s, true));
    c->parity_now = c->last_parity = 0;
    GraphKey key{1, B, flags, {x, cls, loc, mask}};
    StepRec rec;
    int rc = run_maybe_graph(c, key, s, rec, [&](hipStream_t st) { return seq_track(c, rec, x, B, flags, cls, loc, mask, st); });
    if (rc) return rc;
    c->track_B = (flags & SMK_TRACK_MASK) ? B : 0;
    return 0;
}

int smk_refine(smk_ctx *c, const int32_t *pos, int on_device, int B, float *out, void *stream) {
    if (!c || !pos || !out) return fail(SMK_E_ARG, "smk_refine: null argument");
    if (c->variant != SMK_VARIANT_SHARP) return fail(SMK_E_ARG, "smk_refine: only the sharp variant has a Refine module");
    if (c->track_B == 0) return fail(SMK_E_STATE, "smk_refine: needs a preceding smk_track with SMK_TRACK_MASK");
    if (B != c->track_B) return fail(SMK_E_ARG, "smk_refine: batch %d != tracked batch %d", B, c->track_B);
    HIPCHK(hipSetDevice(c->device));
    CHK(seq_health(c));
    hipStream_t s = (hipStream_t)stream;
    CHK(pipe_join(c, s, true));
    c->parity_now = c->last_parity;
    if (!on_device) {
        for (int i = 0; i < 2 * B; ++i)
            if (pos[i] < 0 || pos[i] >= 25) return fail(SMK_E_ARG, "smk_refine: pos[%d]=%d outside [0,25)", i, pos[i]);
        HIPCHK(hipMemcpyAsync(c->pos_dev, pos, sizeof(int) * 2 * B, hipMemcpyHostToDevice, s));
    } else {
        HIPCHK(hipMemcpyAsync(c->pos_dev, pos, sizeof(int) * 2 * B, hipMemcpyDeviceToDevice, s));
    }
    GraphKey key{2, B, c->parity_now, {out}};
    StepRec rec;
    return run_maybe_graph(c, key, s, rec, [&](hipStream_t st) { return seq_refine(c, rec, B, out, st); });
}

enum { KNOB_RAW = 0, KNOB_BOOL = -1 };
struct Knob { const char *name; int *slot; const char *accept; int conv; const char *product; };
#ifdef SMK_MEASURE
static int g_measure_build = 1;
#else
static int g_measure_build = 0;
#endif
static const Knob KNOBS[] = {
    {"xcd_mode", &g_tune.xcd_mode, "*", KNOB_RAW, nullptr},
    {"force_tile", &g_tune.force_tile, "0..5", KNOB_RAW, nullptr},
    {"min_blocks_x16", &g_tune.min_blocks_x16, "*", KNOB_RAW, nullptr},
    {"stages", &g_tune.stages, "0|2..4", KNOB_RAW, nullptr},
    {"kt", &g_tune.kt, "0|128|256", KNOB_RAW, nullptr},
    {"prio", &g_tune.prio, "-1..3", KNOB_RAW, nullptr},
    {"nt_store", &g_tune.nt_store, "*", KNOB_BOOL, nullptr},
    {"merge", &g_tune.merge, "0..2", KNOB_RAW, nullptr},
    {"merge_max_batch", &g_tune.merge_max_batch, "*", KNOB_RAW, nullptr},
    {"rf_wreg", &g_tune.rf_wreg, "*", KNOB_RAW, nullptr},
    {"rf_tile2", &g_tune.rf_tile2, "0..5", KNOB_RAW, nullptr},
    {"nchw_tn_major", &g_tune.nchw_tn_major, "*", KNOB_BOOL, nullptr},
    {"chain", &g_tune.chain, "*", KNOB_BOOL, nullptr},
    {"chain_mask", &g_tune.chain_mask, "0..2", KNOB_RAW, nullptr},
    {"corr_head", &g_tune.corr_head, "*", KNOB_BOOL, nullptr},
    {"pair_launch", &g_tune.pair_launch, "0..3", KNOB_RAW, nullptr},
    {"halo", &g_tune.halo, "0|1|64|128", KNOB_RAW, nullptr},
    {"halo_db", &g_tune.halo_db, "*", KNOB_BOOL, nullptr},
    {"ksplit", &g_tune.ksplit, "0|1|2|4", KNOB_RAW, nullptr},
    {"xc_ch", &g_tune.xc_ch, "32|64", KNOB_RAW, nullptr},
    {"xc_full", &g_tune.xc_full, "0..2", KNOB_RAW, nullptr},
    {"stem_fused", &g_tune.stem_fused, "*", KNOB_BOOL, nullptr},
    {"l1_fused", &g_tune.l1_fused, "*", KNOB_BOOL, nullptr},
    {"buf_lds", &g_tune.buf_lds, "*", KNOB_BOOL, nullptr},
    {"a_stage", &g_tune.a_stage, "*", KNOB_BOOL, nullptr},
    {"wreg", &g_tune.wreg, "0..7", KNOB_RAW, nullptr},
    {"wreg_policy", &g_tune.wreg_policy, "0|1", KNOB_RAW, nullptr},
    {"wreg_stages", &g_tune.wreg_stages, "0|3..8", KNOB_RAW, "0|3|4"},
    {"wreg96", &g_tune.wreg96, "*", KNOB_BOOL, nullptr},
    {"wreg32", &g_tune.wreg32, "0..4096", KNOB_RAW, nullptr},
    {"npw", &g_tune.npw, "2|4", KNOB_RAW, nullptr},
    {"res_nt", &g_tune.res_nt, "*", KNOB_BOOL, nullptr},
    {"pp", &g_tune.pp, "0..2", KNOB_RAW, nullptr},
    {"x3_fused", &g_tune.x3_fused, "*", KNOB_BOOL, nullptr},
    {"ablate", &g_tune.ablate, "*", 127, "0"},
    {"front_occ1", &g_tune.front_occ1, "*", 3, "0"},
    {"seq", &g_tune.seq, "*", KNOB_BOOL, nullptr},
    {"seq_spoll", &g_tune.seq_spoll, "*", KNOB_BOOL, nullptr},
    {"seq_kstag", &g_tune.seq_kstag, "0..2", KNOB_RAW, nullptr},
    {"seq_kstag_mask", &g_tune.seq_kstag_mask, "*", 7, nullptr},
    {"seq_tall", &g_tune.seq_tall, "0..2", KNOB_RAW, nullptr},
    {"seq_fuse", &g_tune.seq_fuse, "0..3", KNOB_RAW, nullptr},
    {"seq_fuse3", &g_tune.seq_fuse3, "0..2", KNOB_RAW, "0"},
    {"seq_pair2d", &g_tune.seq_pair2d, "0..2", KNOB_RAW, "0"},
    {"seq_deep", &g_tune.seq_deep, "*", KNOB_BOOL, "0"},
    {"seq_ds128", &g_tune.seq_ds128, "*", KNOB_BOOL, nullptr},
    {"seq_halo", &g_tune.seq_halo, "*", KNOB_BOOL, nullptr},
    {"seq_yres", &g_tune.seq_yres, "*", KNOB_BOOL, nullptr},
    {"seq_search", &g_tune.seq_search, "*", KNOB_BOOL, nullptr},
    {"seq_first_stage", &g_tune.seq_first_stage, "0..3", KNOB_RAW, "1..3"},
    {"seq_min_batch", &g_tune.seq_min_batch, ">=1", KNOB_RAW, nullptr},
    {"seq_max_batch", &g_tune.seq_max_batch, ">=1", KNOB_RAW, nullptr},
    {"seq_extra_batch", &g_tune.seq_extra_batch, "*", KNOB_RAW, nullptr},
    {"seq_mult_max", &g_tune.seq_mult_max, ">=0", KNOB_RAW, nullptr},
    {"main_prio", &g_tune.main_prio, "0..3", KNOB_RAW, nullptr},
    {"pipe_late", &g_tune.pipe_late, "*", KNOB_BOOL, nullptr},
    {"seq_fused_last", &g_seq_last.pairs, nullptr, KNOB_RAW, nullptr},
    {"seq_yres_last", &g_seq_last.resident, nullptr, KNOB_RAW, nullptr},
    {"seq_fused3_last", &g_seq_last.triples, nullptr, KNOB_RAW, nullptr},
    {"measure_build", &g_measure_build, nullptr, KNOB_RAW, nullptr},
};

static bool knob_accepts(const char *spec, int v) {
    if (!strcmp(spec, "*")) return true;
    for (const char *t = spec; t; t = strchr(t, '|') ? strchr(t, '|') + 1 : nullptr) {
        if (t[0] == '>' && t[1] == '=') {
            if (v >= atoi(t + 2)) return true;
            continue;
        }
        char *e = nullptr;
        const long lo = strtol(t, &e, 10), hi = (e[0] == '.' && e[1] == '.') ? strtol(e + 2, nullptr, 10) : lo;
        if (v >= lo && v <= hi) return true;
    }
    return false;
}

static const Knob *find_knob(const char *key) {
    for (const Knob &k : KNOBS)
        if (!strcmp(key, k.name)) return &k;
    return nullptr;
}

int smk_tune(const char *key, int value) {
    if (!key) return fail(SMK_E_ARG, "smk_tune: key is NULL");
    const Knob *k = find_knob(key);
    if (!k) return fail(SMK_E_ARG, "smk_tune: unknown key %s", key);
    if (!k->accept) return fail(SMK_E_ARG, "smk_tune: %s is a read-only diagnostic", key);
    if (!knob_accepts(k->accept, value)) return fail(SMK_E_ARG, "smk_tune: %s takes %s, not %d", key, k->accept, value);
#ifndef SMK_MEASURE
    if (k->product && !knob_accepts(k->product, value))
        return fail(SMK_E_ARG, "smk_tune: %s %d is a measured alternative, only in a library built with `make MEASURE=1` (this one takes %s)",
                    key, value, k->product);
#endif
    if (k->slot == &g_tune.rf_wreg && (((value >> 4) & 15) > 8 || ((value >> 8) & 15) > 8))
        return fail(SMK_E_ARG, "smk_tune: rf_wreg tile codes (bits 4..7, 8..11) 0..8");
    *k->slot = k->conv == KNOB_BOOL ? value != 0 : (k->conv > 0 ? value & k->conv : value);
    return 0;
}

int smk_tune_get(const char *key, int *value) {
    if (!key || !value) return fail(SMK_E_ARG, "smk_tune_get: null argument");
    const Knob *k = find_knob(key);
    if (!k) return fail(SMK_E_ARG, "smk_tune_get: unknown key %s", key);
    *value = *k->slot;
    return 0;
}

int smk_profile(smk_ctx *c, int enable) {
    if (!c) return fail(SMK_E_ARG, "ctx is NULL");
    c->prof_recs.clear();
    c->prof_pool_next = 0;
    if (enable && c->prof_pool.empty()) {
        c->prof_pool.resize(2 * 1024);
        for (auto &ev : c->prof_pool) HIPCHK(hipEventCreate(&ev));
        HIPCHK(hipDeviceSynchronize());
    }
    c->prof = enable != 0;
    c->prof_merge = enable == 2;
    return 0;
}

int smk_profile_dump(smk_ctx *c, char *buf, int cap) {
    if (!c || !buf || cap < 64) return fail(SMK_E_ARG, "smk_profile_dump: bad argument");
    HIPCHK(hipSetDevice(c->device));
    HIPCHK(hipDeviceSynchronize());
    struct Agg { std::string kernel; double ms = 0, flop = 0, bytes = 0, ext = 0; int calls = 0; };
    std::vector<std::pair<std::string, Agg>> order;
    std::map<std::string, size_t> idx;
    for (auto &r : c->prof_recs) {
        float ms = 0.f;
        if (hipEventElapsedTime(&ms, r.e0, r.e1) != hipSuccess) ms = 0.f;
        auto it = idx.find(r.id);
        if (it == idx.end()) { idx[r.id] = order.size(); order.push_back({r.id, Agg()}); it = idx.find(r.id); }
        Agg &a = order[it->second].second;
        a.kernel = r.kernel; a.ms += ms; a.flop += r.flop; a.bytes += r.bytes; a.ext += r.ext_bytes; a.calls++;
    }
    c->prof_recs.clear();
    c->prof_pool_next = 0;
    std::string js = "[";
    for (size_t i = 0; i < order.size(); ++i) {
        char line[512];
        const Agg &a = order[i].second;
        snprintf(line, sizeof(line), "%s{\"id\":\"%s\",\"kernel\":\"%s\",\"calls\":%d,\"ms\":%.6f,\"flop\":%.6e,\"bytes\":%.6e,\"ext_bytes\":%.6e}",
                 i ? "," : "", order[i].first.c_str(), a.kernel.c_str(), a.calls, a.ms, a.flop, a.bytes, a.ext);
        js += line;
    }
    js += "]";
    if ((int)js.size() + 1 > cap) return fail(SMK_E_ARG, "smk_profile_dump: buffer too small (%zu needed)", js.size() + 1);
    memcpy(buf, js.c_str(), js.size() + 1);
    return 0;
}

static void fill_decode_params(smk_ctx *c, const float *cls, const float *loc, int B, const double *target_wh, int *pos_out,
                               double *box_out, DecodeParams &p) {
    memset(&p, 0, sizeof(p));
    p.cls = cls; p.loc = loc; p.target_wh = target_wh; p.window = c->window_dev;
    p.pos_out = pos_out; p.box_out = box_out;
    {
        char *q = (char *)c->dec_scratch;
        p.part_val = (double *)q;             q += (size_t)c->maxB * 8 * 8;
        p.part_box = (double *)q;             q += (size_t)c->maxB * 64 * 8;
        p.part_idx = (int *)q;                q += (size_t)c->maxB * 8 * 4;
        p.arrived = (unsigned *)q;
    }
    p.B = B; p.A = 5; p.S = 25; p.stride = c->anchor_stride;
    for (int i = 0; i < 5; ++i) { p.anchor_w[i] = c->anchor_w[i]; p.anchor_h[i] = c->anchor_h[i]; }
    p.penalty_k = c->penalty_k; p.window_influence = c->window_influence;
    p.hp = c->stream_hp;
}

static void hp_graph_key(const smk_ctx *c, int64_t &pk, int64_t &wi) {
    memcpy(&pk, &c->penalty_k, 8); memcpy(&wi, &c->window_influence, 8);
    if (c->stream_hp) { pk = (int64_t)(intptr_t)c->stream_hp; wi = -1; }
}

static int seq_decode(smk_ctx *c, const StepRec &rec, const float *cls, const float *loc, int B, const double *target_wh, int *pos_out,
                      double *box_out, hipStream_t s) {
    DecodeParams p;
    fill_decode_params(c, cls, loc, B, target_wh, pos_out, box_out, p);
    if (rec.ring && c->ring_box && box_out) {
        p.ring_box = c->ring_box; p.ring_cursor = c->ring_cursor; p.ring_done = (unsigned *)(c->ring_cursor + 1);
        p.ring_rows = c->ring_rows; p.ring_advance = 1;
        if (rec.ring_refine) {
            p.ring_cursor = c->ring_cursor + 2; p.ring_done = (unsigned *)(c->ring_cursor + 3);
        } else {
            p.ring_also = c->ring_cursor + 2;
        }
    }
    if (rec.mark_fold) { p.mark = c->pipe_cnt + 2; p.mark_arrived = c->pipe_cnt + 4; }
    ProfScope ps(c, s, "decode", "decode", 0.0, (double)B * 30 * 625 * 4);
    if (launch_decode(p, s)) return fail(SMK_E_HIP, "decode launch failed");
    return 0;
}

int smk_set_decode_params(smk_ctx *c, const float *anchor_wh, int n_anchor, int stride, double penalty_k,
                          double window_influence) {
    if (!c) return fail(SMK_E_ARG, "ctx is NULL");
    if (anchor_wh) {
        if (n_anchor != 5) return fail(SMK_E_ARG, "smk_set_decode_params: kernels are specialised for 5 anchors");
        for (int i = 0; i < 5; ++i) { c->anchor_w[i] = anchor_wh[2 * i]; c->anchor_h[i] = anchor_wh[2 * i + 1]; }
    }
    if (stride > 0) c->anchor_stride = stride;
    c->penalty_k = penalty_k;
    c->window_influence = window_influence;
    CHK(pipe_quiesce(c));
    for (auto &kv : c->graphs) hipGraphExecDestroy(kv.second);
    c->graphs.clear();
    c->graph_used.clear();
    return 0;
}

int smk_set_stream_hp(smk_ctx *c, const double *hp_dev) {
    if (!c) return fail(SMK_E_ARG, "ctx is NULL");
    HIPCHK(hipSetDevice(c->device));
    if (hp_dev) {
        hipPointerAttribute_t at;
        memset(&at, 0, sizeof(at));
        if (hipPointerGetAttributes(&at, hp_dev) != hipSuccess) {
            (void)hipGetLastError();
            return fail(SMK_E_ARG, "smk_set_stream_hp: %p is not device memory", (const void *)hp_dev);
        }
        if (at.type != hipMemoryTypeDevice || (uintptr_t)hp_dev % 8)
            return fail(SMK_E_ARG, "smk_set_stream_hp: %p is not (8-byte aligned) device memory", (const void *)hp_dev);
    }
    CHK(pipe_quiesce(c));
    c->stream_hp = hp_dev;
    return 0;
}

int smk_decode(smk_ctx *c, const float *cls, const float *loc, int B, const double *target_wh, int32_t *pos_out,
               double *box_out, void *stream) {
// ... 369 lines not shown
    case 6: pl.kind = CK_PP; return conv_pp_eligible(p, dtype) ? 0 : 1;
    case 7: pl.kind = CK_MHEAD; return mask_head_eligible(p, dtype) ? 0 : 1;
    default: pl.kind = CK_IGEMM; pl.tile = tile_from_code(code, p, dtype); return 0;
    }
}

int smk_op_conv2d_ex(int dtype, int algo, const smk_conv_geom *g, const float *x_dev, const float *w_host,
                     const float *b_host, const float *res_dev, const int32_t *pos_host, float *y_dev,
                     void *stream) {
    if (!g || !x_dev || !w_host || !y_dev) return fail(SMK_E_ARG, "smk_op_conv2d_ex: null argument");
    if (dtype != DT_F32 && dtype != DT_F16 && dtype != DT_F16X3) return fail(SMK_E_ARG, "bad dtype");
    const bool x3 = dtype == DT_F16X3;
    if (x3 && (((algo & 0xff) != 0 && (algo & 0xff) != 5) || g->cin_off || g->cin_len))
        return fail(SMK_E_ARG, "smk_op_conv2d_ex: split-operand convolutions: algo 0 (conv_igemm_kernel) or 5 (conv_wreg_kernel), no channel slice");
    const int ctx_dtype = dtype;
    dtype = kdtype(dtype);
    hipStream_t s = (hipStream_t)stream;
    PackedConv pc; Act in; ConvOpt o; int Ho, Wo;
    CHK(fill_geom(g, pc, in, o, Ho, Wo));
    std::vector<float> rows, bias;
    pack_host(g, pc, w_host, b_host, rows, bias);
    if (x3) {
        const int Ci0 = pc.Ci, K1 = pc.Kpad;
        pc.x3 = true;
        pc.alg_k = g->k * g->k * Ci0;
        pc.Ci = 3 * Ci0;
        pc.K = g->k * g->k * pc.Ci;
        pc.Kpad = rup(pc.K, KPAD_ALIGN);
        std::vector<float> osc;
        split_rows_x3(rows, pc.rows, K1, pc.Kpad, g->k * g->k, Ci0, osc);
        CHK(upload_oscale(pc, osc));
        in.C *= X3_PLANES;
    }
    std::vector<float> fused;
    if (x3 && g_tune.x3_fused && fuse_rows_x3(rows, pc, g->k * g->k, pc.Ci / 3, fused)) CHK(upload_packed(pc, rows, bias, dtype, &fused));
    else
    CHK(upload_packed(pc, rows, bias, dtype));
    TmpBufs tmp;
    tmp.v.push_back(pc.w); tmp.v.push_back(pc.bias);
    if (pc.w_frag) tmp.v.push_back(pc.w_frag);
    if (pc.w_frag16) tmp.v.push_back(pc.w_frag16);
    if (pc.oscale) tmp.v.push_back(pc.oscale);
    const size_t es = esize(dtype);
    CHK(tmp.alloc(&in.p, (size_t)g->B * g->H * g->W * in.C * es));
    CvtInParams ci{x_dev, in.p, g->B, g->Cin, g->H, g->W, x3 ? in.C / X3_PLANES : in.C, 0, x3 ? 1 : 0};
    if (x3 ? launch_cvt_in_x3(ci, s) : launch_cvt_in(ci, dtype, s)) return fail(SMK_E_HIP, "cvt_in launch failed");
    int *pos_dev = nullptr;
    if (pos_host) {
        CHK(tmp.alloc((void **)&pos_dev, sizeof(int) * 2 * g->B));
        HIPCHK(hipMemcpyAsync(pos_dev, pos_host, sizeof(int) * 2 * g->B, hipMemcpyHostToDevice, s));
        o.pos = pos_dev;
    }
    const int mode = algo & 0xff;
    const bool nchw = (mode == 2 || mode == 3 || mode == 7);
    if (mode == 4) {
        CHK(upload_halo_pack(pc, rows, dtype));
        if (pc.w_frag_halo) tmp.v.push_back(pc.w_frag_halo);
        if (pc.w_halo) tmp.v.push_back(pc.w_halo);
    }
    Act out, res;
    out.H = Ho; out.W = Wo; out.C = rup(g->Cout, 8) * (x3 ? X3_PLANES : 1);
    if (res_dev && g->res_mode) {
        if (nchw) return fail(SMK_E_ARG, "residual is not supported with the NCHW epilogue");
        res = out;
        CHK(tmp.alloc(&res.p, (size_t)g->B * Ho * Wo * out.C * es));
        CvtInParams cr{res_dev, res.p, g->B, g->Cout, Ho, Wo, x3 ? out.C / X3_PLANES : out.C, 0, x3 ? 1 : 0};
        if (x3 ? launch_cvt_in_x3(cr, s) : launch_cvt_in(cr, dtype, s)) return fail(SMK_E_HIP, "cvt_in launch failed");
        o.res = &res; o.res_mode = g->res_mode;
    }
    ConvEnv env;
    env.dtype = ctx_dtype;
    HIPCHK(hipGetDevice(&env.device));
    CHK(op_ks_scratch(env));
    ConvParams p;
    if (nchw) {
        o.nchw_out = y_dev;
        CHK(conv_params(env, pc, in, nullptr, g->B, o, p));
    } else {
        CHK(tmp.alloc(&out.p, (size_t)g->B * Ho * Wo * out.C * es));
        CHK(conv_params(env, pc, in, &out, g->B, o, p));
    }
    ConvPlan pl;
    const int prc = plan_from_algo(algo, p, dtype, pl);
    if (prc < 0) return fail(SMK_E_ARG, "smk_op_conv2d_ex: wreg tile code 1..8");
    if (prc)
        return fail(SMK_E_ARG, "smk_op_conv2d_ex: %s", pl.kind == CK_HALO ? "geometry is not eligible for the halo kernel"
                    : (pl.kind == CK_WREG ? "geometry / dtype is not eligible for conv_wreg_kernel"
                       : (pl.kind == CK_MHEAD ? "geometry / dtype is not eligible for mask_head_kernel (fp16, 1x1, Cin = 256, Cout <= 4096, no ReLU)"
                          : "geometry / dtype is not eligible for conv_pp_kernel")));
    ConvBatch cb;
    cb.n = 1;
    cb.p[0] = p;
    CHK(launch_plan(pl, cb, pc.w_halo, dtype, s, "conv"));
    if (!nchw) {
        CvtOutParams co{out.p, y_dev, g->B, g->Cout, Ho, Wo, out.C, 0, x3 ? out.C / X3_PLANES : 0};
        if (x3 ? launch_cvt_out_x3(co, s) : launch_cvt_out(co, dtype, s)) return fail(SMK_E_HIP, "cvt_out launch failed");
    }
    HIPCHK(hipStreamSynchronize(s));
    return 0;
}

static int seq_op_records(const smk_seq_op *ops, int n, const Act &xin, int device, const std::function<int(int, PackedConv &)> &pack,
                          const std::function<int(void **, size_t)> &alloc, std::vector<SeqRec> &rec, std::vector<Act> &outs) {
    const int dtype = DT_F16, B = ops[0].g.B;
    ConvEnv env;
    env.dtype = dtype;
    env.device = device;
    rec.assign(n, SeqRec());
    outs.assign(n, Act());
    for (int i = 0; i < n; ++i) {
        const smk_seq_op &op = ops[i];
        if (!op.w_host) return fail(SMK_E_ARG, "smk_op_conv_seq: layer %d has no weights", i);
        if (op.src >= i || op.res_src >= i) return fail(SMK_E_ARG, "smk_op_conv_seq: layer %d reads a later layer", i);
        if (op.g.B != B || op.g.win || op.g.ups) return fail(SMK_E_ARG, "smk_op_conv_seq: layer %d: one batch, no windows", i);
        const Act &in = op.src < 0 ? xin : outs[op.src];
        const int cin_have = op.src < 0 ? ops[0].g.Cin : ops[op.src].g.Cout;
        if (op.g.H != in.H || op.g.W != in.W || op.g.Cin != cin_have)
            return fail(SMK_E_ARG, "smk_op_conv_seq: layer %d geometry does not match its source", i);
        PackedConv pc; Act gin; ConvOpt o; int Ho, Wo;
        CHK(fill_geom(&op.g, pc, gin, o, Ho, Wo));
        CHK(pack(i, pc));
        outs[i].H = Ho; outs[i].W = Wo; outs[i].C = rup(op.g.Cout, 8);
        CHK(alloc(&outs[i].p, (size_t)B * Ho * Wo * outs[i].C * esize(dtype)));
        Act res;
        if (op.g.res_mode) {
            if (op.res_src < -1) return fail(SMK_E_ARG, "smk_op_conv_seq: layer %d wants a residual without a source", i);
            res = op.res_src < 0 ? xin : outs[op.res_src];
            if (res.H != Ho || res.W != Wo || res.C != outs[i].C)
                return fail(SMK_E_ARG, "smk_op_conv_seq: layer %d: residual shape differs from the output", i);
            o.res = &res; o.res_mode = op.g.res_mode;
        }
        ConvParams p;
        CHK(conv_params(env, pc, in, &outs[i], B, o, p));
        SeqLayer &L = rec[i].L;
        const int force_halo = op.cfg == SEQ_CFG_HALO128 ? 128 : (op.cfg == SEQ_CFG_HALO64 ? 64 : (op.cfg >= 0 ? -1 : 0));
        if (!seq_layer_from(p, dtype, L, force_halo)) return fail(SMK_E_ARG, "smk_op_conv_seq: layer %d cannot run inside a sequence%s", i, force_halo > 0 ? " on the patch-sharing tile" : "");
        if (op.cfg >= 0 && force_halo <= 0) {
#ifdef SMK_MEASURE
            if (op.cfg > 18) return fail(SMK_E_ARG, "smk_op_conv_seq: cfg 0..18");
#else
            if (op.cfg > 9 || (op.cfg >= 6 && op.cfg <= 8))
                return fail(SMK_E_ARG, "smk_op_conv_seq: cfg 0..5, 9 (6..8, 10..18 are measurement tiles: `make MEASURE=1`)");
#endif
            L.cfg = (signed char)op.cfg;
        }
        if (op.kstag >= 0) L.kstag = (signed char)(op.kstag != 0);
        L.sync = (signed char)(op.sync != 0);
        rec[i].wstd = pc.w_frag;
        rec[i].id = "op" + std::to_string(i);
    }
    return 0;
}

static SeqPlanStats plan_seq_ops(const smk_seq_op *ops, std::vector<SeqRec> &rec, const std::vector<Act> &outs, int grid) {
    std::vector<char> locked(rec.size());
    std::vector<const void *> read_after;
    for (size_t i = 0; i < rec.size(); ++i) {
        locked[i] = ops[i].cfg >= 0;
        if (ops[i].y_dev) read_after.push_back(outs[i].p);
    }
    return plan_seq(rec, {ops[0].g.B, grid >> 3, true}, locked.data(), read_after);
}

int smk_op_conv_seq(const smk_seq_op *ops, int n, const float *x_dev, int iters, float *usec_out, float *clk_us_out,
                    int *n_fused_out, void *stream) {
    if (!ops || !x_dev || n < 1 || n > SEQ_MAX || iters < 1) return fail(SMK_E_ARG, "smk_op_conv_seq: bad argument (1..%d layers)", SEQ_MAX);
    hipStream_t s = (hipStream_t)stream;
    const int dtype = DT_F16;
    const size_t es = esize(dtype);
    int dev = 0;
    HIPCHK(hipGetDevice(&dev));
    hipDeviceProp_t prop;
    HIPCHK(hipGetDeviceProperties(&prop, dev));
    const int grid = seq_grid_for(prop.multiProcessorCount);
    if (!grid) return fail(SMK_E_STATE, "smk_op_conv_seq: the XCD placement / occupancy check failed on this device");
    TmpBufs tmp;
    const int B = ops[0].g.B;
    Act xin;
    xin.H = ops[0].g.H; xin.W = ops[0].g.W; xin.C = rup(ops[0].g.Cin, 8);
    CHK(tmp.alloc(&xin.p, (size_t)B * xin.H * xin.W * xin.C * es));
    CvtInParams ci{x_dev, xin.p, B, ops[0].g.Cin, xin.H, xin.W, xin.C, 0};
    if (launch_cvt_in(ci, dtype, s)) return fail(SMK_E_HIP, "cvt_in launch failed");
    std::vector<PackedConv> packs(n);
    auto pack = [&](int i, PackedConv &pc) -> int {
        const smk_seq_op &op = ops[i];
        int same = -1;
        for (int j = 0; j < i && same < 0; ++j)
            if (ops[j].w_host == op.w_host && ops[j].b_host == op.b_host && ops[j].g.Cout == op.g.Cout &&
                ops[j].g.Cin == op.g.Cin && ops[j].g.k == op.g.k && ops[j].g.cin_len == op.g.cin_len) same = j;
        if (same >= 0) {
            pc.w = packs[same].w; pc.bias = packs[same].bias; pc.w_frag = packs[same].w_frag; pc.w_frag_halo = packs[same].w_frag_halo;
        } else {
            std::vector<float> rows, bias;
            pack_host(&op.g, pc, op.w_host, op.b_host, rows, bias);
            CHK(upload_packed(pc, rows, bias, dtype));
            if (pc.k == 3) CHK(upload_halo_pack(pc, rows, dtype));
            tmp.v.push_back(pc.w); tmp.v.push_back(pc.bias);
            if (pc.w_frag) tmp.v.push_back(pc.w_frag);
            if (pc.w_frag16) tmp.v.push_back(pc.w_frag16);
            if (pc.w_halo) tmp.v.push_back(pc.w_halo);
            if (pc.w_frag_halo) tmp.v.push_back(pc.w_frag_halo);
        }
        packs[i] = pc;
        return 0;
    };
    std::vector<SeqRec> rec;
    std::vector<Act> outs;
    CHK(seq_op_records(ops, n, xin, dev, pack, [&](void **p, size_t bytes) { return tmp.alloc(p, bytes); }, rec, outs));
    g_seq_last = plan_seq_ops(ops, rec, outs, grid);
    SeqArgs a;
    memset(&a, 0, sizeof(a));
    a.n = n; a.B = B;
    a.flags = g_tune.seq_spoll ? 1 : 0;
    for (int i = 0; i < n; ++i) a.L[i] = rec[i].L;
    unsigned *bar = nullptr;
    int *err = nullptr;
    unsigned long long *clk = nullptr, *clk2 = nullptr;
    CHK(tmp.alloc((void **)&bar, 8 * 32 * sizeof(unsigned)));
    CHK(tmp.alloc((void **)&err, sizeof(int)));
    CHK(tmp.alloc((void **)&clk, sizeof(unsigned long long) * (2 * SEQ_MAX + 1)));
    const char *ck = getenv("SMK_SEQ_CLK");
    const bool want2 = ck && !strcmp(ck, "2");
    if (want2) CHK(tmp.alloc((void **)&clk2, sizeof(unsigned long long) * (12 + 32) * SEQ_MAX));
    float *xch = nullptr;
    CHK(tmp.alloc((void **)&xch, SEQ_XCH_BYTES));
    a.bar = bar; a.xch = xch; a.err = err; a.err_host = nullptr; a.clk = clk; a.clk2 = clk2;
    if (n_fused_out) {
        *n_fused_out = 0;
        for (int i = 0; i < n; ++i) *n_fused_out += a.L[i].cfg == SEQ_CFG_C3C1_2ND;
    }
    hipEvent_t e0, e1;
    HIPCHK(hipEventCreate(&e0));
    HIPCHK(hipEventCreate(&e1));
    SeqArgs a_run = a;
    a_run.clk = nullptr; a_run.clk2 = nullptr;
    if (launch_conv_seq(a_run, grid, s)) return fail(SMK_E_HIP, "conv_seq launch failed: %s", hipGetErrorString(hipGetLastError()));
    HIPCHK(hipEventRecord(e0, s));
    for (int it = 1; it < iters; ++it)
        if (launch_conv_seq(a_run, grid, s)) return fail(SMK_E_HIP, "conv_seq launch failed: %s", hipGetErrorString(hipGetLastError()));
    HIPCHK(hipEventRecord(e1, s));
    if (launch_conv_seq(a, grid, s)) return fail(SMK_E_HIP, "conv_seq launch failed: %s", hipGetErrorString(hipGetLastError()));
    HIPCHK(hipStreamSynchronize(s));
    float ms = 0.f;
    if (iters > 1) HIPCHK(hipEventElapsedTime(&ms, e0, e1));
    (void)hipEventDestroy(e0); (void)hipEventDestroy(e1);
    if (usec_out) *usec_out = iters > 1 ? ms * 1000.f / (iters - 1) : 0.f;
    int e = 0;
    HIPCHK(hipMemcpy(&e, err, sizeof(int), hipMemcpyDeviceToHost));
    if (e) return fail(SMK_E_HIP, "conv_seq_kernel reported %s", e == 1 ? "an uneven distribution of workgroups over the XCDs" : "a team-barrier time-out");
    {
        unsigned long long h[2 * SEQ_MAX + 1], h2[(12 + 32) * SEQ_MAX];
        HIPCHK(hipMemcpy(h, clk, sizeof(h), hipMemcpyDeviceToHost));
        if (clk_us_out)
            for (int i = 0; i < n; ++i) {
                clk_us_out[2 * i] = (float)((h[1 + 2 * i] - h[2 * i]) / 100.0);
                clk_us_out[2 * i + 1] = (float)((h[2 + 2 * i] - h[1 + 2 * i]) / 100.0);
            }
        if (ck) {
            if (want2) HIPCHK(hipMemcpy(h2, clk2, sizeof(h2), hipMemcpyDeviceToHost));
            seq_print_clk(a, rec.data(), "smk_op_conv_seq", h, want2 ? h2 : nullptr);
        }
    }
    for (int i = 0; i < n; ++i)
        if (ops[i].y_dev) {
            CvtOutParams co{outs[i].p, ops[i].y_dev, B, ops[i].g.Cout, outs[i].H, outs[i].W, outs[i].C, 0};
            if (launch_cvt_out(co, dtype, s)) return fail(SMK_E_HIP, "cvt_out launch failed");
        }
    HIPCHK(hipStreamSynchronize(s));
    return 0;
}

int smk_op_conv2d(int dtype, int algo, const float *x_dev, int B, int Cin, int H, int W, const float *w_host,
                  const float *b_host, int Cout, int k, int stride, int pad, int dil, int relu,
                  const float *res_dev, float *y_dev, void *stream) {
    smk_conv_geom g;
    memset(&g, 0, sizeof(g));
    g.B = B; g.Cin = Cin; g.H = H; g.W = W; g.Cout = Cout; g.k = k; g.stride = stride; g.pad = pad; g.dil = dil;
    g.relu = relu; g.res_mode = res_dev ? RES_PRE_RELU : RES_NONE;
    return smk_op_conv2d_ex(dtype, algo, &g, x_dev, w_host, b_host, res_dev, nullptr, y_dev, stream);
}

int smk_op_dw_xcorr(int dtype, const float *x_dev, const float *k_dev, int B, int C, int H, int W, int kh, int kw,
                    float *y_dev, void *stream) {
    if (!x_dev || !k_dev || !y_dev) return fail(SMK_E_ARG, "smk_op_dw_xcorr: null argument");
    if (C % 64 != 0) return fail(SMK_E_ARG, "smk_op_dw_xcorr: C must be a multiple of 64");
    if (kh > 5 || kw > 5 || kh > H || kw > W || (W - kw + 1 + 1) / 2 > 13)
        return fail(SMK_E_ARG, "smk_op_dw_xcorr: unsupported geometry");
    hipStream_t s = (hipStream_t)stream;
    TmpBufs tmp;
    const size_t es = esize(dtype);
    const int Ho = H - kh + 1, Wo = W - kw + 1;
    void *x, *k, *y;
    CHK(tmp.alloc(&x, (size_t)B * H * W * C * es));
    CHK(tmp.alloc(&k, (size_t)B * kh * kw * C * es));
    CHK(tmp.alloc(&y, (size_t)B * Ho * Wo * C * es));
    CvtInParams cx{x_dev, x, B, C, H, W, C, 0}, ck{k_dev, k, B, C, kh, kw, C, 0};
    if (launch_cvt_in(cx, dtype, s) || launch_cvt_in(ck, dtype, s)) return fail(SMK_E_HIP, "cvt_in launch failed");
    XcorrParams xp{x, k, y, B, H, W, kh, kw, Ho, Wo, C, C};
    if (launch_xcorr(xp, dtype, s)) return fail(SMK_E_HIP, "xcorr launch failed");
    CvtOutParams co{y, y_dev, B, C, Ho, Wo, C, 0};
    if (launch_cvt_out(co, dtype, s)) return fail(SMK_E_HIP, "cvt_out launch failed");
    HIPCHK(hipStreamSynchronize(s));
    return 0;
}

int smk_op_maxpool3x3s2(int dtype, const float *x_dev, int B, int C, int H, int W, float *y_dev, void *stream) {
    if (!x_dev || !y_dev) return fail(SMK_E_ARG, "smk_op_maxpool3x3s2: null argument");
    if (C % 8 != 0) return fail(SMK_E_ARG, "smk_op_maxpool3x3s2: C must be a multiple of 8");
    hipStream_t s = (hipStream_t)stream;
    TmpBufs tmp;
    const size_t es = esize(dtype);
    const int Ho = (H + 2 - 3) / 2 + 1, Wo = (W + 2 - 3) / 2 + 1;
    void *x, *y;
    CHK(tmp.alloc(&x, (size_t)B * H * W * C * es));
    CHK(tmp.alloc(&y, (size_t)B * Ho * Wo * C * es));
    CvtInParams cx{x_dev, x, B, C, H, W, C, 0};
    if (launch_cvt_in(cx, dtype, s)) return fail(SMK_E_HIP, "cvt_in launch failed");
    PoolParams pp{x, y, B, H, W, C, Ho, Wo};
    if (launch_maxpool(pp, dtype, s)) return fail(SMK_E_HIP, "maxpool launch failed");
    CvtOutParams co{y, y_dev, B, C, Ho, Wo, C, 0};
    if (launch_cvt_out(co, dtype, s)) return fail(SMK_E_HIP, "cvt_out launch failed");
    HIPCHK(hipStreamSynchronize(s));
    return 0;
}

constexpr size_t OP_GUARD = 4096;
constexpr int OP_GUARD_BYTE = 0xA5;
struct GuardedBuf {
    unsigned char *base = nullptr;
    size_t bytes = 0;
    void *p() const { return base + OP_GUARD; }
    int alloc(TmpBufs &tmp, size_t n, hipStream_t s) {
        HIPCHK(hipMalloc((void **)&base, n + 2 * OP_GUARD));
        tmp.v.push_back(base);
        bytes = n;
        HIPCHK(hipMemsetAsync(base, OP_GUARD_BYTE, OP_GUARD, s));
        HIPCHK(hipMemsetAsync(base + OP_GUARD, 0xFF, n, s));
        HIPCHK(hipMemsetAsync(base + OP_GUARD + n, OP_GUARD_BYTE, OP_GUARD, s));
        return 0;
    }
    int check(const char *entry, const char *name) const {
        std::vector<unsigned char> h(2 * OP_GUARD);
        HIPCHK(hipMemcpy(h.data(), base, OP_GUARD, hipMemcpyDeviceToHost));
        HIPCHK(hipMemcpy(h.data() + OP_GUARD, base + OP_GUARD + bytes, OP_GUARD, hipMemcpyDeviceToHost));
        for (size_t i = 0; i < 2 * OP_GUARD; ++i)
            if (h[i] != OP_GUARD_BYTE)
                return fail(SMK_E_STATE, "%s: the kernel wrote outside the %s buffer (guard band %s it, byte %d)", entry, name,
                            i < OP_GUARD ? "before" : "after", (int)(i % OP_GUARD));
        return 0;
    }
};

static int op_pack(TmpBufs &tmp, PackedConv &pc, int Cin, int Cout, int k, const float *w, const float *b) {
    smk_conv_geom g;
    memset(&g, 0, sizeof(g));
    g.B = 1; g.Cin = Cin; g.H = g.W = k; g.Cout = Cout; g.k = k; g.stride = 1; g.dil = 1;
    Act in; ConvOpt o; int Ho, Wo;
    CHK(fill_geom(&g, pc, in, o, Ho, Wo));
    std::vector<float> rows, bias;
    pack_host(&g, pc, w, b, rows, bias);
    const int rc = upload_packed(pc, rows, bias, DT_F16);
    for (void *q : {pc.w, (void *)pc.bias, pc.w_frag, pc.w_frag16})
        if (q) tmp.v.push_back(q);
    return rc;
}

int smk_op_stem_pool(const float *x_dev, const float *w_host, const float *b_host, int S, int B, float *p0_dev, float *x1_dev,
                     void *stream) {
    if (!x_dev || !w_host || !b_host || !p0_dev || !x1_dev) return fail(SMK_E_ARG, "smk_op_stem_pool: null argument");
    if (S < 7 || S > 8192) return fail(SMK_E_ARG, "smk_op_stem_pool: S = %d (7 .. 8192)", S);
    if (B < 1 || B > 1024) return fail(SMK_E_ARG, "smk_op_stem_pool: B = %d (1 .. 1024)", B);
    hipStream_t s = (hipStream_t)stream;
    const int s0 = (S - 7) / 2 + 1, s1 = (s0 - 1) / 2 + 1;
    PackedConv pc = stem_pack_geom();
    std::vector<float> rows((size_t)pc.rows * pc.Kpad, 0.f), bias(pc.rows, 0.f);
    const std::vector<double> one(64, 1.0), shift(b_host, b_host + 64);
    stem_pair_rows(rows, bias, pc.Kpad, w_host, one.data(), shift.data());
    TmpBufs tmp;
    const int rc = upload_packed(pc, rows, bias, DT_F16);
    for (void *q : {pc.w, (void *)pc.bias, pc.w_frag, pc.w_frag16})
        if (q) tmp.v.push_back(q);
    CHK(rc);
    if (!pc.w_frag) return fail(SMK_E_STATE, "smk_op_stem_pool: internal: the stem has no fragment-order pack");
    GuardedBuf p0, x1;
    CHK(p0.alloc(tmp, (size_t)B * s0 * s0 * 64 * 2, s));
    CHK(x1.alloc(tmp, (size_t)B * s1 * s1 * 64 * 2, s));
    StemPoolParams sp{x_dev, pc.w_frag, pc.bias, p0.p(), x1.p(), B, S, s0, s1, pc.Kpad, 0};
    if (launch_stem_pool(sp, s)) return fail(SMK_E_HIP, "stem_pool launch failed: %s", hipGetErrorString(hipGetLastError()));
    CvtOutParams c0{p0.p(), p0_dev, B, 64, s0, s0, 64, 0}, c1{x1.p(), x1_dev, B, 64, s1, s1, 64, 0};
    if (launch_cvt_out(c0, DT_F16, s) || launch_cvt_out(c1, DT_F16, s)) return fail(SMK_E_HIP, "cvt_out launch failed");
    HIPCHK(hipStreamSynchronize(s));
    CHK(p0.check("smk_op_stem_pool", "p0"));
    CHK(x1.check("smk_op_stem_pool", "x1"));
    return 0;
}

int smk_op_l1_block(const float *x_dev, const float *w1_host, const float *b1_host, const float *w2_host, const float *b2_host,
                    const float *w3_host, const float *b3_host, const float *wd_host, const float *bd_host, int Cin, int S, int B,
                    float *y_dev, void *stream) {
    if (!x_dev || !w1_host || !b1_host || !w2_host || !b2_host || !w3_host || !b3_host || !y_dev)
        return fail(SMK_E_ARG, "smk_op_l1_block: null argument");
    if (Cin != 64 && Cin != 256) return fail(SMK_E_ARG, "smk_op_l1_block: Cin = %d (64: block 0 with its projection, 256)", Cin);
    if (Cin == 64 && (!wd_host || !bd_host)) return fail(SMK_E_ARG, "smk_op_l1_block: Cin = 64 needs the projection shortcut wd, bd");
    if (Cin == 256 && (wd_host || bd_host)) return fail(SMK_E_ARG, "smk_op_l1_block: Cin = 256 has an identity shortcut: wd, bd must be null");
    if (S < 1 || S > 4096) return fail(SMK_E_ARG, "smk_op_l1_block: S = %d (1 .. 4096)", S);
    if (B < 1 || B > 1024) return fail(SMK_E_ARG, "smk_op_l1_block: B = %d (1 .. 1024)", B);
    hipStream_t s = (hipStream_t)stream;
    TmpBufs tmp;
    PackedConv p1, p2, p3, pd;
    CHK(op_pack(tmp, p1, Cin, 64, 1, w1_host, b1_host));
    CHK(op_pack(tmp, p2, 64, 64, 3, w2_host, b2_host));
    CHK(op_pack(tmp, p3, 64, 256, 1, w3_host, b3_host));
// ... 627 lines not shown
    if (g->pos_mul) {
        CHK(tmp.alloc((void **)&pos_dev, sizeof(int) * 2 * g->B));
        std::vector<int> ph(2 * g->B);
        for (int i = 0; i < 2 * g->B; ++i) ph[i] = 8 + (i * 5) % 9;
        HIPCHK(hipMemcpy(pos_dev, ph.data(), ph.size() * 4, hipMemcpyHostToDevice));
        o.pos = pos_dev;
    }
    const int mode = algo & 0xff;
    if (mode == 5 || mode == 7) pc.w_frag = pc.w;
    Act out, res;
    out.H = Ho; out.W = Wo; out.C = rup(g->Cout, 8);
    float *nchw = nullptr;
    const bool nchw_mode = mode == 2 || mode == 7;
    if (nchw_mode) {
        CHK(tmp.alloc((void **)&nchw, (size_t)g->B * g->Cout * Ho * Wo * 4));
        o.nchw_out = nchw;
    } else {
        CHK(tmp.alloc(&out.p, (size_t)g->B * Ho * Wo * out.C * es));
        if (with_res) {
            res = out;
            CHK(fill(&res.p, (size_t)g->B * Ho * Wo * out.C, 1.0f, 3));
            o.res = &res; o.res_mode = RES_PRE_RELU;
        }
    }
    ConvEnv env;
    env.dtype = dtype;
    HIPCHK(hipGetDevice(&env.device));
    CHK(op_ks_scratch(env));
    ConvParams p;
    CHK(conv_params(env, pc, in, nchw_mode ? nullptr : &out, g->B, o, p));
    ConvPlan pl;
    const int prc = plan_from_algo(mode == 1 || mode == 3 ? algo & ~0xff : algo, p, dtype, pl);
    if (prc < 0) return fail(SMK_E_ARG, "smk_bench_conv: wreg tile code 1..8");
    if (prc && pl.kind == CK_HALO) return fail(SMK_E_HIP, "conv launch failed or geometry not eligible");
    if (prc) return fail(SMK_E_ARG, "smk_bench_conv: not eligible for %s", pl.kind == CK_WREG ? "conv_wreg_kernel" : (pl.kind == CK_MHEAD ? "mask_head_kernel" : "conv_pp_kernel"));
    auto launch = [&]() {
        ConvBatch cb;
        cb.n = 1;
        cb.p[0] = p;
        return launch_plan(pl, cb, p.wgt, dtype, s, "conv");
    };
    hipEvent_t e0, e1;
    HIPCHK(hipEventCreate(&e0));
    HIPCHK(hipEventCreate(&e1));
    for (int i = 0; i < 3; ++i) CHK(launch());
    HIPCHK(hipEventRecord(e0, s));
    for (int i = 0; i < iters; ++i) CHK(launch());
    HIPCHK(hipEventRecord(e1, s));
    HIPCHK(hipEventSynchronize(e1));
    float ms = 0.f;
    HIPCHK(hipEventElapsedTime(&ms, e0, e1));
    (void)hipEventDestroy(e0); (void)hipEventDestroy(e1);
    *usec_out = ms * 1000.f / iters;
    return 0;
}

int smk_host_conv2d_ex(const smk_conv_geom *g, const float *x, const float *w, const float *b, const float *res,
                       const int32_t *pos, float *y) {
    if (!g || !x || !w || !y) return fail(SMK_E_ARG, "smk_host_conv2d_ex: null argument");
    PackedConv pc; Act in; ConvOpt o; int Ho, Wo;
    CHK(fill_geom(g, pc, in, o, Ho, Wo));
    std::vector<float> rows, bias;
    pack_host(g, pc, w, b, rows, bias);
    std::vector<float> xin((size_t)g->B * g->H * g->W * in.C, 0.f);
    for (int bb = 0; bb < g->B; ++bb)
        for (int c = 0; c < g->Cin; ++c)
            for (int yy = 0; yy < g->H; ++yy)
                for (int xx = 0; xx < g->W; ++xx)
                    xin[(((size_t)bb * g->H + yy) * g->W + xx) * in.C + c] =
                        x[(((size_t)bb * g->Cin + c) * g->H + yy) * g->W + xx];
    in.p = xin.data();
    pc.w = rows.data();
    pc.bias = bias.data();
    o.pos = pos;
    Act out;
    out.H = Ho; out.W = Wo; out.C = rup(g->Cout, 8);
    std::vector<float> obuf((size_t)g->B * Ho * Wo * out.C, 0.f);
    out.p = obuf.data();
    ConvEnv env;
    env.device = -1;
    ConvParams p;
    CHK(conv_params(env, pc, in, &out, g->B, o, p));
    for (int m = 0; m < p.M; ++m) {
        const RowInfo r = row_info(p, m, p.pos);
        for (int n = 0; n < g->Cout; ++n) {
            double acc = 0.0;
            for (int kvec = 0; kvec < p.K; kvec += 4) {
                const KDecode d = decode_k(kvec, p.Ci, p.kw);
                const long off = gather_offset(p, r, d, p.cin_off);
                if (off < 0) continue;
                for (int e = 0; e < 4; ++e) acc += (double)xin[off + e] * (double)rows[(size_t)n * p.Kpad + kvec + e];
            }
            double v = acc + bias[n];
            const int hw = Ho * Wo, bb = m / hw, ps = m - bb * hw;
            const double rv = (res && g->res_mode) ? res[((size_t)bb * g->Cout + n) * hw + ps] : 0.0;
            if (g->res_mode == RES_PRE_RELU) v += rv;
            if (g->relu) v = v > 0 ? v : 0;
            if (g->res_mode == RES_POST_RELU) v += rv;
            y[((size_t)bb * g->Cout + n) * hw + ps] = (float)v;
        }
    }
    return 0;
}

static void fake_pack(PackedConv &pc, int dtype) {
    static float dummy[64];
    pc.w = dummy; pc.bias = dummy;
    if (has_frag_pack(pc, dtype)) pc.w_frag = dummy;
    if (has_frag16_pack(pc, dtype)) pc.w_frag16 = dummy;
    if (has_halo_pack(pc, dtype)) pc.w_halo = dummy;
    if (has_frag_halo_pack(pc, dtype)) pc.w_frag_halo = dummy;
}

int smk_host_plan_conv(const smk_conv_geom *g, int dtype, int with_res, int *kernel, int *bm, int *bn, int *seq_cfg) {
    if (!g || !kernel || !bm || !bn || !seq_cfg) return fail(SMK_E_ARG, "smk_host_plan_conv: null argument");
    if (dtype != DT_F32 && dtype != DT_F16) return fail(SMK_E_ARG, "smk_host_plan_conv: dtype");
    PackedConv pc; Act in; ConvOpt o; int Ho, Wo;
    CHK(fill_geom(g, pc, in, o, Ho, Wo));
    static float dummy[64];
    in.p = dummy;
    fake_pack(pc, dtype);
    Act out, res;
    out.H = Ho; out.W = Wo; out.C = rup(g->Cout, 8); out.p = dummy;
    res = out;
    if (with_res) { o.res = &res; o.res_mode = RES_PRE_RELU; }
    ConvEnv env;
    env.device = -1;
    env.dtype = dtype;
    ConvParams p;
    CHK(conv_params(env, pc, in, &out, g->B, o, p));
    const ConvPlan pl = plan_conv(p, o, pc, dtype, g->B, MI355X_CUS);
    switch (pl.kind) {
    case CK_PP: *kernel = 3; *bm = 256; *bn = 256; break;
    case CK_WREG: *kernel = 2; *bm = WREG_TILE[pl.wreg][0]; *bn = WREG_TILE[pl.wreg][1]; break;
    case CK_HALO: *kernel = 1; *bm = pl.halo_bm; *bn = 128; break;
    default: *kernel = 0; *bm = pl.tile.bm; *bn = pl.tile.bn;
    }
    SeqLayer L;
    *seq_cfg = seq_layer_from(p, dtype, L) ? (int)L.cfg : -1;
    return 0;
}

int smk_host_plan_seq(const smk_seq_op *ops, int n, int grid, int *cfg, int *sync, int *a_stage) {
    if (!ops || n < 1 || n > 4 * SEQ_MAX || grid < 8 || grid % 8 || !cfg || !sync || !a_stage)
        return fail(SMK_E_ARG, "smk_host_plan_seq: bad argument (1..%d layers, a grid of whole teams)", 4 * SEQ_MAX);
    static char tensors[4 * SEQ_MAX + 1];
    Act xin;
    xin.H = ops[0].g.H; xin.W = ops[0].g.W; xin.C = rup(ops[0].g.Cin, 8); xin.p = tensors;
    int next = 1;
    std::vector<SeqRec> rec;
    std::vector<Act> outs;
    CHK(seq_op_records(ops, n, xin, -1, [](int, PackedConv &pc) { fake_pack(pc, DT_F16); return 0; },
                       [&](void **p, size_t) { *p = tensors + next++; return 0; }, rec, outs));
    plan_seq_ops(ops, rec, outs, grid);
    for (int i = 0; i < n; ++i) {
        cfg[i] = rec[i].L.cfg;
        sync[i] = rec[i].L.sync;
        a_stage[i] = rec[i].L.a_stage;
    }
    return 0;
}

int smk_host_arena_elems(int dtype, int variant, int pipe_depth, uint64_t *elems_per_image) {
    if (!elems_per_image) return fail(SMK_E_ARG, "smk_host_arena_elems: null argument");
    if (dtype != DT_F32 && dtype != DT_F16 && dtype != DT_F16X3) return fail(SMK_E_ARG, "smk_host_arena_elems: bad dtype %d", dtype);
    if (variant < SMK_VARIANT_RPN || variant > SMK_VARIANT_SHARP) return fail(SMK_E_ARG, "smk_host_arena_elems: bad variant %d", variant);
    if (pipe_depth < 0 || pipe_depth > 2) return fail(SMK_E_ARG, "smk_host_arena_elems: depth %d", pipe_depth);
    return arena_elems(dtype, variant, pipe_depth, elems_per_image);
}

}
```

siammask_amd/csrc/smk_kernels.h:

```cpp
#pragma once
#include <stdint.h>

#if defined(__HIPCC__)
#define SMK_HD __host__ __device__ inline
#else
#define SMK_HD inline
#endif

namespace smk {

enum { DT_F32 = 0, DT_F16 = 1, DT_F16X3 = 2 };
enum { RES_NONE = 0, RES_PRE_RELU = 1, RES_POST_RELU = 2 };
enum { OUT_NHWC = 0, OUT_NCHW_F32 = 1 };

constexpr int NPAD_ALIGN = 128;
constexpr int KPAD_ALIGN = 128;

struct ConvParams {
    const void *in;
    const void *wgt;
    const void *wgt_frag;
    const void *wgt_frag_halo;
    const float *bias;
    const void *res;
    void *out;
    const int *pos;
    const void *zero;
    int B;
    int Hs, Ws, Cs;
    int cin_off;
    int Ci;
    int Hl, Wl;
    int org_y, org_x;
    int pos_mul, pos_add;
    int ups;
    int Ho, Wo;
    int kh, kw, stride, pad, dil;
    int stride_x;
    int K, Kpad;
    int N;
    int Nst;
    int M;
    int Cos, cout_off;
    int res_Cs, res_coff;
    int relu, res_mode, out_mode;
    int groups;
    int g_cin_off;
    int g_wgt_off;
    int g_cout_off;
    int xcd_mode;
    int ci_shift;
    int kw_magic;
    int prio;
    int wave_prio;
    int buf_lds;
    int a_stage;
    int res_nt;
    unsigned in_bytes, w_bytes;
    int nt_store;
    int x3_out, x3_res, x3_in;
    int x3_ct, x3_nreal;
    const float *oscale;
    int ksplit;
    float *ks_part;
    unsigned *ks_cnt;
    size_t ks_part_cap;
    int ks_cnt_cap;
};

constexpr int CONV_BATCH_MAX = 4;
struct ConvBatch {
    int n;
    int start[CONV_BATCH_MAX + 1];
    ConvParams p[CONV_BATCH_MAX];
};

struct SeqLayer {
    const void *in;
    const void *wgt_frag;
    const float *bias;
    const void *res;
    void *out;
    unsigned in_bytes, w_bytes;
    int kw_magic;
    unsigned short Hs, Ws, Hl, Wl, Ho, Wo, Cs, cin_off, Ci, Kpad, Nst, Cos, res_Cs, res_coff, cout_off, bar_ord;
    short org_y, org_x;
    signed char kh, kw, stride, stride_x, pad, dil, relu, res_mode, ci_shift;
    signed char cfg;
    signed char sync;
    signed char a_stage;
    signed char kstag;
    signed char res_nt;
    static constexpr const int *pos = nullptr;
    static constexpr int pos_mul = 0, pos_add = 0, ups = 0, g_cin_off = 0, g_wgt_off = 0, g_cout_off = 0;
    static constexpr int x3_out = 0, x3_res = 0, x3_in = 0, x3_ct = 0, x3_nreal = 0;
    static constexpr const float *oscale = nullptr;
};
static_assert(sizeof(SeqLayer) == 104, "SeqLayer packing");
constexpr int SEQ_CFG_C3C1_L3 = 20;
constexpr int SEQ_CFG_C3C1_L2 = 21;
constexpr int SEQ_CFG_C3C1_2ND = 22;
constexpr int SEQ_CFG_C3C1P_L3 = 26;
constexpr int SEQ_CFG_C3C1P_L2 = 27;
constexpr int SEQ_CFG_C2C3C1_L3 = 28;
constexpr int SEQ_CFG_C2C3C1_L2 = 29;
constexpr int SEQ_CFG_C2C3C1_MID = 30;
constexpr int SEQ_XCH_SLAB = 32768;
constexpr int SEQ_XCH_PAIRS = 16;
constexpr size_t SEQ_XCH_BYTES = (size_t)8 * SEQ_XCH_PAIRS * 4 * SEQ_XCH_SLAB;
constexpr int SEQ_CFG_HALO128 = 24;
constexpr int SEQ_CFG_HALO64 = 25;
constexpr int SEQ_YRES_IN = 2, SEQ_YRES_NOSTORE = 4, SEQ_LDS_HI = 8;
constexpr int SEQ_YRES_BYTES = 65536;
constexpr int SEQ_MAX = 36;
struct SeqArgs {
    int n, B;
    int flags, pad_;
    unsigned *bar;
    float *xch;
    int *err;
    int *err_host;
    unsigned long long *clk;
    unsigned long long *clk2;
    unsigned *exit_sem;
    SeqLayer L[SEQ_MAX];
};
static_assert(sizeof(SeqArgs) <= 4096, "the layer list travels in the kernel-argument segment");

struct Tuning {
    int xcd_mode = 1;
    int force_tile = 0;
    int min_blocks_x16 = 16;
    int stages = 0;
    int kt = 0;
    int prio = 0;
    int nt_store = 1;
    int halo = 1;
    int halo_db = 1;
    int chain = 1;
    int ksplit = 0;
    int xc_ch = 64;
    int l1_fused = 1;
    int stem_fused = 1;
    int xc_full = 0;
    int buf_lds = 1;
    int chain_mask = 1;
    int nchw_tn_major = 1;
    int merge = 1;
    int merge_max_batch = 32;
    int rf_wreg = 3;
    int seq_fuse3 = 0;
    int seq_spoll = 1;
    int wreg = 1;
    int wreg_stages = 0;
    int seq = 1;
    int seq_min_batch = 5, seq_max_batch = 8;
    int seq_extra_batch = 12;
    int seq_mult_max = 24;
    int ablate = 0;
    int seq_tall = 2;
    int seq_kstag = 1;
    int res_nt = 1;
    int seq_fuse = 1;
    int rf_tile2 = 0;
    int pair_launch = 1;
    int corr_head = 1;
    int seq_yres = 1;
    int seq_search = 0;
    int seq_pair2d = 0;
    int seq_halo = 1;
    int seq_kstag_mask = 7;
    int seq_ds128 = 0;
    int seq_deep = 0;
    int seq_first_stage = 1;
    int wreg_policy = 1;
    int npw = 4;
    int a_stage = 0;
    int pp = 1;
    int main_prio = 3;
    int front_occ1 = 0;
    int wreg96 = 1;
    int x3_fused = 1;
    int wreg32 = 140;
    int pipe_late = 1;
};
extern Tuning g_tune;

struct KDecode { int kh_i, kw_i, c; };

SMK_HD KDecode decode_k(int kvec, int Ci, int kw) {
    KDecode d;
    int tap = kvec / Ci;
    d.c = kvec - tap * Ci;
    d.kh_i = tap / kw;
    d.kw_i = tap - d.kh_i * kw;
    return d;
}

struct RowInfo { int b, ly0, lx0, oy_org, ox_org; };

SMK_HD RowInfo row_info(const ConvParams &p, int m, const int *pos) {
    RowInfo r;
    int hw = p.Ho * p.Wo;
    r.b = m / hw;
    int rem = m - r.b * hw;
    int oy = rem / p.Wo;
    int ox = rem - oy * p.Wo;
    r.ly0 = oy * p.stride - p.pad;
    r.lx0 = ox * p.stride_x - p.pad;
    r.oy_org = p.org_y;
    r.ox_org = p.org_x;
    if (pos) {
        r.oy_org += pos[2 * r.b + 0] * p.pos_mul + p.pos_add;
        r.ox_org += pos[2 * r.b + 1] * p.pos_mul + p.pos_add;
    }
    return r;
}

SMK_HD long gather_offset(const ConvParams &p, const RowInfo &r, const KDecode &d, int cin_off) {
    int ly = r.ly0 + d.kh_i * p.dil;
    int lx = r.lx0 + d.kw_i * p.dil;
    if ((unsigned)ly >= (unsigned)p.Hl || (unsigned)lx >= (unsigned)p.Wl) return -1;
    int sy, sx;
    if (p.ups) {
        sy = (ly * p.Hs) / p.Hl;
        sx = (lx * p.Ws) / p.Wl;
    } else {
        sy = ly + r.oy_org;
        sx = lx + r.ox_org;
    }
    if ((unsigned)sy >= (unsigned)p.Hs || (unsigned)sx >= (unsigned)p.Ws) return -1;
    return ((long)(r.b * p.Hs + sy) * p.Ws + sx) * p.Cs + cin_off + d.c;
}

struct XcorrParams {
    const void *x;
    const void *k;
    void *out;
    int B, H, W, kh, kw, Ho, Wo, C, Cs;
};

struct CorrHeadParams {
    const _Float16 *xs;
    const _Float16 *zk;
    _Float16 *corr;
    _Float16 *h0;
    const void *w0_frag;
    const float *b0;
    const void *w3_frag[2];
    const float *b3[2];
    float *out3[2];
    int n3[2];
    unsigned w0_bytes, w3_bytes[2];
    int B, nb, Cs;
    unsigned *start_sem;
};
int launch_corr_head(const CorrHeadParams &p, void *stream);

#ifdef __HIPCC__
__device__ __forceinline__ void set_wave_prio(int prio) {
    if (prio == 3) __builtin_amdgcn_s_setprio(3);
    else if (prio == 2) __builtin_amdgcn_s_setprio(2);
    else if (prio == 1) __builtin_amdgcn_s_setprio(1);
}
#endif
constexpr int X3_PLANES = 2;
struct PoolParams { const void *in; void *out; int B, H, W, C, Ho, Wo; int x3; };
struct StemPoolParams { const float *in; const void *wgt_frag; const float *bias; void *p0; void *x1; int B, S, s0, s1, Kpad; int prio; };

struct CvtInParams { const float *in; void *out; int B, C, H, W, Cpad; int pairs; int x3; };
struct CvtOutParams { const void *in; float *out; int B, C, H, W, Cs, coff; int plane; };

struct DecodeParams {
    const float *cls;
    const float *loc;
    const double *target_wh;
    const double *window;
    int *pos_out;
    double *box_out;
    double *part_val;
    int *part_idx;
    double *part_box;
    unsigned *arrived;
    int B, A, S, stride;
    float anchor_w[8], anchor_h[8];
    double penalty_k, window_influence;
    double *ring_box;
    int *ring_cursor;
    unsigned *ring_done;
    int ring_rows, ring_advance;
    int *ring_also;
    unsigned *mark, *mark_arrived;
    const double *hp;
};

struct RingParams {
    const double *box;
    const float *ref;
    double *box_ring;
    _Float16 *ref_ring;
    int *cursor;
    unsigned *done;
    int rows, B, n;
};

constexpr int CROP_MAX_B = 32;
struct CropParams {
    const unsigned char *frames;
    long frame_stride;
    float *out;
    int H, W, model_sz;
    int box[CROP_MAX_B][3];
    unsigned char avg[CROP_MAX_B][4];
};
struct PasteParams {
    const float *logits;
    unsigned char *mask_out;
    float *prob_out;
    int ms, W, H;
    float seg_thr, border;
    double inv_map[CROP_MAX_B][6];
};

struct TileChoice { int bm, bn, kt, stages; };
TileChoice choose_tile(const ConvParams &p, int dtype);
int launch_conv_mfma(const ConvParams &p, int dtype, TileChoice t, void *stream);
int launch_conv_mfma_batch(ConvBatch &cb, int dtype, TileChoice t, void *stream);
int launch_conv_naive(const ConvParams &p, int dtype, void *stream);
int conv_ksplit(const ConvParams &p, int dtype, const TileChoice &t);
__attribute__((visibility("hidden"))) bool conv_halo_eligible(const ConvParams &p, int dtype, int bm);
int launch_conv_halo(const ConvParams &p, int dtype, int bm, void *stream);
bool conv_wreg_eligible(const ConvParams &p, int dtype);
int launch_conv_wreg_batch(ConvBatch &cb, int bm, int bn, int stages, void *stream);
bool conv_pp_eligible(const ConvParams &p, int dtype);
int launch_conv_pp(const ConvParams &p, void *stream);
int launch_conv_seq(const SeqArgs &a, int grid, void *stream);
int launch_conv_pair(const SeqLayer &L3, const SeqLayer &L1, int code, int M, void *stream, int rows);
int conv_seq_occupancy();
int xcc_census(int grid, int *out_host);
struct RefineChainLayer {
    const void *w;
    const float *bias;
    int Kpad, Ci;
};
struct RefineChainParams {
    const void *d;
    const void *v2, *v1, *v0;
    int v2_cs, v1_cs, v0_cs;
    RefineChainLayer L[9];
    float *out;
    int B;
    unsigned long long *clk;
    _Float16 *ring;
    int *ring_cursor;
    unsigned *ring_done;
    int ring_rows;
    unsigned *tail_sem;
};
int launch_refine_chain(const RefineChainParams &p, void *stream);
int launch_chain_mask(const RefineChainParams &rp, ConvBatch &cb, int stationary, void *stream);
bool mask_head_eligible(const ConvParams &p, int dtype);
int mask_head_nsplit(const ConvParams &p, int cus);
int launch_mask_head(const ConvParams &p, void *stream);
int launch_xcorr(const XcorrParams &p, int dtype, void *stream);
int launch_xcorr_x3(const XcorrParams &p, void *stream);
void xcorr_prepare();
int launch_maxpool(const PoolParams &p, int dtype, void *stream);
int launch_stem_pool(const StemPoolParams &p, void *stream);
struct L1BlockParams {
    const void *x; void *y;
    const void *w1, *w2, *w3, *wd;
    const float *b1, *b2, *b3, *bd;
    int B, S, Cin, K1pad, K2pad, K3pad, Kdpad;
    unsigned long long *clk;
    int prio;
};
int launch_l1_block(const L1BlockParams &p, void *stream);
int launch_cvt_in(const CvtInParams &p, int dtype, void *stream);
int launch_cvt_out(const CvtOutParams &p, int dtype, void *stream);
int launch_cvt_in_x3(const CvtInParams &p, void *stream);
int launch_cvt_out_x3(const CvtOutParams &p, void *stream);
int launch_maxpool_x3(const PoolParams &p, void *stream);
int launch_decode(const DecodeParams &p, void *stream);
int launch_ring_commit(const RingParams &p, void *stream);
int launch_pipe_gate(unsigned *sem, int *err, int *err_host, void *stream, int long_wait = 0, unsigned *started_wait = nullptr, unsigned *started_set = nullptr);
int launch_pipe_done(unsigned *sem, void *stream);
int launch_crop_resize(const CropParams &p, int B, void *stream);
int launch_paste_mask(const PasteParams &p, int B, void *stream);
int launch_paste_labels(const PasteParams &p, int n_obj, void *stream);
struct RboxHdr {
    unsigned long long best;
    int ncomp, err;
};
struct RboxParams {
    const unsigned char *mask;
    int B, W, H, Wq, Wh;
    double min_area;
    RboxHdr *hdr; int *rows; unsigned long long *bits; int *parent;
    double *out;
};
int launch_mask_rbox(const RboxParams &p, void *stream);
const void *zero_page();

}
```

siammask_amd/ops.py:

```python
import ctypes

import numpy as np
import torch

from . import _lib

ALGO = {"mfma": 0, "naive": 1, "mfma_nchw": 2, "naive_nchw": 3, "halo": 4, "wreg": 5, "pp": 6, "mask_head": 7}
WREG_TILE = {(64, 256): 1, (64, 128): 2, (64, 64): 3, (128, 256): 4, (128, 128): 5, (128, 64): 6, (96, 256): 7, (32, 64): 8}
TILE = {None: 0, "auto": 0, (128, 128): 1, (128, 64): 2, (64, 128): 3, (64, 64): 4, (256, 128): 5}


def _chk_cuda(*ts):
    for t in ts:
        if t is not None and not t.is_cuda:
            raise RuntimeError("siammask_amd.ops run on the MI355X only (got a CPU tensor)")


def tile_code(tile=None, kt=0, stages=0):
    return TILE[tile] | ({0: 0, 128: 1, 256: 2}[kt] << 4) | ({0: 0, 2: 1, 3: 2, 4: 3}[stages] << 6)


def wreg_code(tile, stages=0):
    return WREG_TILE[tuple(tile)] | ({0: 0, 8: 1, 3: 2, 4: 3}[stages] << 6)


def conv2d(x, w, b=None, stride=1, pad=0, dil=1, relu=False, res=None, res_mode=1, dtype="f32",
           algo="mfma", tile=None, win=None, ups=None, pos=None, pos_mul=0, pos_add=0, org=(0, 0),
           cin_off=0, cin_len=0, kt=0, stages=0, out=None):
    _chk_cuda(x, res, out)
    x = x.contiguous().float()
    B, Cin, H, W = x.shape
    w = np.ascontiguousarray(w.detach().cpu().numpy() if isinstance(w, torch.Tensor) else w, dtype=np.float32)
    bb = None if b is None else np.ascontiguousarray(
        b.detach().cpu().numpy() if isinstance(b, torch.Tensor) else b, dtype=np.float32)
    g = _lib.ConvGeom()
    g.B, g.Cin, g.H, g.W = B, Cin, H, W
    g.Cout, g.k, g.stride, g.pad, g.dil = w.shape[0], w.shape[2], stride, pad, dil
    g.relu = int(bool(relu))
    g.res_mode = res_mode if res is not None else 0
    g.cin_off, g.cin_len = cin_off, cin_len
    g.org_y, g.org_x = org
    g.pos_mul, g.pos_add = pos_mul, pos_add
    Hl, Wl = H, W
    if win is not None:
        g.win, g.Hl, g.Wl = 1, win[0], win[1]
        Hl, Wl = win
    if ups is not None:
        g.ups, g.Hl, g.Wl = 1, ups[0], ups[1]
        Hl, Wl = ups
    Ho = (Hl + 2 * pad - dil * (g.k - 1) - 1) // stride + 1
    Wo = (Wl + 2 * pad - dil * (g.k - 1) - 1) // stride + 1
    y = out if out is not None else torch.empty((B, g.Cout, Ho, Wo), dtype=torch.float32, device=x.device)
    if tuple(y.shape) != (B, g.Cout, Ho, Wo) or y.dtype != torch.float32 or not y.is_contiguous():
        raise ValueError("out must be a contiguous float32 tensor of shape %s" % ((B, g.Cout, Ho, Wo),))
    p = None if pos is None else np.ascontiguousarray(pos, dtype=np.int32)
    r = None if res is None else res.contiguous().float()
    code = ALGO[algo] | ((wreg_code(tile, stages) if algo == "wreg" else tile_code(tile, kt, stages)) << 8)
    vp = lambda a: a.ctypes.data_as(ctypes.c_void_p) if a is not None else None
    with torch.cuda.device(x.device):
        _lib.check(_lib.lib().smk_op_conv2d_ex(
            _lib.DTYPE[dtype], code, ctypes.byref(g), x.data_ptr(), vp(w), vp(bb),
            r.data_ptr() if r is not None else None, vp(p), y.data_ptr(), _lib.current_stream_ptr()))
    return y


SEQ_CFG = {None: -1, (64, 256): 0, (64, 128): 1, (64, 64): 2, (128, 256): 3, (128, 128): 4, "deep": 5,
           "no_a": 6, "no_w": 7, "no_mfma": 8, (128, 64): 9,
           "abl10": 10, "abl11": 11, "abl12": 12, "abl13": 13, "abl14": 14, "old64x128": 15, "old128x256": 16, "old64x256": 17, "old64x64": 18,
           "halo128": 24, "halo64": 25}


def seq_ops(x_shape, layers):
    B = x_shape[0]
    arr = (_lib.SeqOp * len(layers))()
    keep = []
    shapes = [tuple(x_shape[1:])]
    for i, l in enumerate(layers):
        w = np.ascontiguousarray(l["w"], dtype=np.float32)
        b = None if l.get("b") is None else np.ascontiguousarray(l["b"], dtype=np.float32)
        keep += [w, b]
        src = l.get("src", i - 1)
        cin, H, W = shapes[src + 1]
        k, stride, pad, dil = w.shape[2], l.get("stride", 1), l.get("pad", 0), l.get("dil", 1)
        g = arr[i].g
        g.B, g.Cin, g.H, g.W = B, cin, H, W
        g.Cout, g.k, g.stride, g.pad, g.dil = w.shape[0], k, stride, pad, dil
        g.relu = int(bool(l.get("relu", False)))
        g.res_mode = l.get("res_mode", 1) if "res" in l else 0
        Ho = (H + 2 * pad - dil * (k - 1) - 1) // stride + 1
        Wo = (W + 2 * pad - dil * (k - 1) - 1) // stride + 1
        shapes.append((w.shape[0], Ho, Wo))
        arr[i].src = src
        arr[i].res_src = l.get("res", -2)
        arr[i].sync = int(bool(l.get("sync", True)))
        arr[i].cfg = SEQ_CFG[l.get("tile")]
        arr[i].kstag = l.get("kstag", -1)
        arr[i].w_host = w.ctypes.data
        arr[i].b_host = b.ctypes.data if b is not None else None
    return arr, keep, shapes[1:]


def _wanted(want_outputs, i):
    return want_outputs is True or (want_outputs not in (False, None) and i in want_outputs)


def conv_seq(x, layers, iters=1, want_outputs=True, info=None):
    _chk_cuda(x)
    x = x.contiguous().float()
    B = x.shape[0]
    n = len(layers)
    arr, keep, shapes = seq_ops(x.shape, layers)
    outs = []
    for i, shape in enumerate(shapes):
        if _wanted(want_outputs, i):
            y = torch.empty((B,) + shape, dtype=torch.float32, device=x.device)
            outs.append(y)
            arr[i].y_dev = y.data_ptr()
        elif want_outputs not in (True, False, None):
            outs.append(None)
    us = ctypes.c_float(0.0)
    clk = np.zeros(2 * n, dtype=np.float32)
    nfused = ctypes.c_int(0)
    with torch.cuda.device(x.device):
        _lib.check(_lib.lib().smk_op_conv_seq(arr, n, x.data_ptr(), iters, ctypes.byref(us),
                                              clk.ctypes.data_as(ctypes.c_void_p), ctypes.byref(nfused), _lib.current_stream_ptr()))
    if info is not None:
        info["fused_pairs"] = nfused.value
    return outs, us.value, clk.reshape(n, 2)


def plan_seq(x_shape, layers, want_outputs=True, grid=256):
    arr, keep, _ = seq_ops(x_shape, layers)
    n = len(layers)
    for i in range(n):
        if _wanted(want_outputs, i):
            arr[i].y_dev = 1
    out = [(ctypes.c_int * n)() for _ in range(3)]
    _lib.check(_lib.lib().smk_host_plan_seq(arr, n, grid, *out))
    return list(zip(*[list(o) for o in out]))


def dw_xcorr(x, k, dtype="f32"):
    _chk_cuda(x, k)
    x, k = x.contiguous().float(), k.contiguous().float()
    B, C, H, W = x.shape
    kh, kw = k.shape[2], k.shape[3]
    y = torch.empty((B, C, H - kh + 1, W - kw + 1), dtype=torch.float32, device=x.device)
    with torch.cuda.device(x.device):
        _lib.check(_lib.lib().smk_op_dw_xcorr(_lib.DTYPE[dtype], x.data_ptr(), k.data_ptr(), B, C, H, W, kh, kw,
                                              y.data_ptr(), _lib.current_stream_ptr()))
    return y


def maxpool3x3s2(x, dtype="f32"):
    _chk_cuda(x)
    x = x.contiguous().float()
    B, C, H, W = x.shape
    y = torch.empty((B, C, (H - 1) // 2 + 1, (W - 1) // 2 + 1), dtype=torch.float32, device=x.device)
    with torch.cuda.device(x.device):
        _lib.check(_lib.lib().smk_op_maxpool3x3s2(_lib.DTYPE[dtype], x.data_ptr(), B, C, H, W, y.data_ptr(),
                                                  _lib.current_stream_ptr()))
    return y


def _host_f32(a):
    return np.ascontiguousarray(a.detach().cpu().numpy() if isinstance(a, torch.Tensor) else a, dtype=np.float32)


def stem_pool(x, w, b):
    _chk_cuda(x)
    x = x.contiguous().float()
    B, C, S, S2 = x.shape
    w, b = _host_f32(w), _host_f32(b)
    if C != 3 or S != S2 or w.shape != (64, 3, 7, 7) or b.shape != (64,):
        raise ValueError("stem_pool: x [B,3,S,S], w [64,3,7,7], b [64]")
    s0 = (S - 7) // 2 + 1
    s1 = (s0 - 1) // 2 + 1
    p0 = torch.empty((B, 64, max(s0, 0), max(s0, 0)), dtype=torch.float32, device=x.device)
    x1 = torch.empty((B, 64, max(s1, 0), max(s1, 0)), dtype=torch.float32, device=x.device)
    vp = lambda a: a.ctypes.data_as(ctypes.c_void_p)
    with torch.cuda.device(x.device):
        _lib.check(_lib.lib().smk_op_stem_pool(x.data_ptr(), vp(w), vp(b), S, B, p0.data_ptr(), x1.data_ptr(),
                                               _lib.current_stream_ptr()))
    return p0, x1


def l1_block(x, w1, b1, w2, b2, w3, b3, wd=None, bd=None):
    _chk_cuda(x)
    x = x.contiguous().float()
    B, Cin, S, S2 = x.shape
    hs = [None if a is None else _host_f32(a) for a in (w1, b1, w2, b2, w3, b3, wd, bd)]
    want = [(64, Cin, 1, 1), (64,), (64, 64, 3, 3), (64,), (256, 64, 1, 1), (256,), (256, 64, 1, 1), (256,)]
    if S != S2 or any(a is not None and a.shape != s for a, s in zip(hs, want)):
        raise ValueError("l1_block: x [B,Cin,S,S], w1 [64,Cin,1,1], w2 [64,64,3,3], w3 / wd [256,64,1,1]")
    y = torch.empty((B, 256, S, S), dtype=torch.float32, device=x.device)
    vp = lambda a: a.ctypes.data_as(ctypes.c_void_p) if a is not None else None
    with torch.cuda.device(x.device):
        _lib.check(_lib.lib().smk_op_l1_block(x.data_ptr(), *[vp(a) for a in hs], Cin, S, B, y.data_ptr(),
                                              _lib.current_stream_ptr()))
    return y


def bench_conv(B, Cin, H, W, Cout, k, stride=1, pad=0, dil=1, dtype="f16", tile=None, kt=0, stages=0,
               res=False, nchw=False, win=None, pos_mul=0, pos_add=0, iters=50, halo=False, wreg=False, pp=False):
    g = _lib.ConvGeom()
    g.B, g.Cin, g.H, g.W = B, Cin, H, W
    g.Cout, g.k, g.stride, g.pad, g.dil = Cout, k, stride, pad, dil
    g.relu = 1
    g.pos_mul, g.pos_add = pos_mul, pos_add
    if win is not None:
        g.win, g.Hl, g.Wl = 1, win[0], win[1]
    us = ctypes.c_float(0.0)
    if pp:
        code = 6
    elif wreg:
        code = 5 | (wreg_code(tile, stages) << 8)
    else:
        code = (4 if halo else (2 if nchw else 0)) | (tile_code(tile, kt, stages) << 8)
    _lib.check(_lib.lib().smk_bench_conv(_lib.DTYPE[dtype], code, ctypes.byref(g), int(bool(res)), iters,
                                         ctypes.byref(us), _lib.current_stream_ptr()))
    return us.value
```

Baseline: 14840.

## Launch lean persistent-kernel instantiations carrying only the tile routines each slice needs

Adds a routine-mask template parameter to the persistent conv sequence kernel so that instantiations compile only the tile routines a layer list actually uses. The planner now splits each chunk into slices covered by one of two lean masks, cutting at a legal sync point when needed, and the launcher picks the lean instantiation if its VGPR count fits. The aim is lower register pressure and code size in the persistent kernel. The cost is possibly one extra kernel launch per split chunk, and a fallback to the full kernel when a lean variant does not fit.

```diff
diff --git a/siammask_amd/_lib.py b/siammask_amd/_lib.py
--- a/siammask_amd/_lib.py
+++ b/siammask_amd/_lib.py
@@ -27,6 +27,7 @@
     "smk_crop_resize_dev_v", "smk_crop_exemplar_dev_v", "smk_frame_sums_v", "smk_trk_start_v", "smk_host_trk_start_v",
     "smk_paste_mask_dev_v", "smk_vot_overlap_dev",
     "smk_set_stream_hp", "smk_trk_advance_hp", "smk_host_trk_advance_hp",
+    "smk_host_plan_seq_slices",
 )
 
 
@@ -162,6 +163,7 @@
     L.smk_host_trk_advance_hp.argtypes = [vp, ci, cp, vp, vp, ci, vp, ci]
     L.smk_op_conv_seq.argtypes = [ctypes.POINTER(SeqOp), ci, fp, ci, ctypes.POINTER(ctypes.c_float), fp, ip, vp]
     L.smk_host_plan_seq.argtypes = [ctypes.POINTER(SeqOp), ci, ci, ip, ip, ip]
+    L.smk_host_plan_seq_slices.argtypes = [ip, ip, ip, ci]
     L.smk_bench_conv.argtypes = [ci, ci, gp, ci, ci, ctypes.POINTER(ctypes.c_float), vp]
     for name in SYMBOLS:
         fn = getattr(L, name)
diff --git a/siammask_amd/csrc/conv_plan.cpp b/siammask_amd/csrc/conv_plan.cpp
--- a/siammask_amd/csrc/conv_plan.cpp
+++ b/siammask_amd/csrc/conv_plan.cpp
@@ -261,8 +261,59 @@
     return marked;
 }
 
-SeqPlanStats plan_seq(std::vector<SeqRec> &rec, const SeqPlanEnv &env, const char *locked, const std::vector<const void *> &read_after) {
+int seq_need_mask(const SeqLayer *L, int i0, int i1) {
+    int need = 0;
+    for (int i = i0; i < i1; ++i) {
+        const int cf = L[i].cfg;
+        if (cf == SEQ_CFG_C3C1_2ND) continue;
+        const int bit = seq_routine_bit(cf);
+        if (!bit) return -1;
+        need |= bit;
+    }
+    return need;
+}
+
+int seq_lean_mask_for(int need, int usable) {
+    int best = 0, i = 0;
+    for (int m : SEQ_LEAN_MASKS) {
+        if (need >= 0 && ((usable >> i) & 1) && (need & ~m) == 0 && (!best || __builtin_popcount(m) < __builtin_popcount(best))) best = m;
+        ++i;
+    }
+    return best;
+}
+
+static bool seq_cut_legal(const SeqLayer *L, int i0, int i1, int k) {
+    if (k <= i0 || k >= i1) return false;
+    const int pc = L[k - 1].cfg, cf = L[k].cfg;
+    if (!L[k - 1].sync) return false;
+    if (pc == SEQ_CFG_C3C1_L3 || pc == SEQ_CFG_C3C1_L2 || pc == SEQ_CFG_C3C1P_L3 || pc == SEQ_CFG_C3C1P_L2 || pc == SEQ_CFG_C2C3C1_L3 ||
+        pc == SEQ_CFG_C2C3C1_L2 || pc == SEQ_CFG_C2C3C1_MID)
+        return false;
+    if (cf == SEQ_CFG_C3C1_2ND || cf == SEQ_CFG_C2C3C1_MID) return false;
+    if (L[k].a_stage & (SEQ_YRES_IN | SEQ_LDS_HI)) return false;
+    return true;
+}
+
+static int seq_cut_point(const SeqLayer *L, int i0, int i1, int usable) {
+    for (int k = i1 - SEQ_CUT_MIN; k >= i0 + SEQ_CUT_MIN; --k)
+        if (seq_cut_legal(L, i0, i1, k) && seq_lean_mask_for(seq_need_mask(L, i0, k), usable) && seq_lean_mask_for(seq_need_mask(L, k, i1), usable)) return k;
+    return 0;
+}
+
+static void seq_slices_of_chunk(const SeqLayer *L, int i0, int i1, int usable, std::vector<SeqSlice> &out) {
+    auto put = [&](int a, int b, int mask) { SeqSlice s; s.i0 = a; s.n = b - a; s.mask = mask; out.push_back(s); };
+    if (!g_tune.seq_lean) return put(i0, i1, SEQ_R_ALL);
+    if (const int m = seq_lean_mask_for(seq_need_mask(L, i0, i1), usable)) return put(i0, i1, m);
+    const int k = g_tune.seq_lean >= 2 ? seq_cut_point(L, i0, i1, usable) : 0;
+    if (!k) return put(i0, i1, SEQ_R_ALL);
+    put(i0, k, seq_lean_mask_for(seq_need_mask(L, i0, k), usable));
+    put(k, i1, seq_lean_mask_for(seq_need_mask(L, k, i1), usable));
+}
+
+SeqPlanStats plan_seq(std::vector<SeqRec> &rec, const SeqPlanEnv &env, const char *locked, const std::vector<const void *> &read_after,
+                      std::vector<SeqSlice> *slices) {
     const int n = (int)rec.size();
+    if (slices) slices->clear();
     std::vector<SeqLayer> L(n);
     std::vector<const void *> wstd(n);
     for (int i = 0; i < n; ++i) { L[i] = rec[i].L; wstd[i] = rec[i].wstd; }
@@ -273,6 +324,7 @@
         st.pairs = seq_fuse_pairs(L.data() + i0, i1 - i0, env.B, locked ? locked + i0 : nullptr, xch);
         st.triples = seq_fuse_triples(L.data(), i0, i1, n, wstd.data(), locked, read_after);
         st.resident = seq_mark_resident(L.data(), i0, i1, n, env, read_after);
+        if (slices) seq_slices_of_chunk(L.data(), i0, i1, env.lean_usable, *slices);
     }
     for (int i = 0; i < n; ++i) rec[i].L = L[i];
     return st;
diff --git a/siammask_amd/csrc/conv_plan.h b/siammask_amd/csrc/conv_plan.h
--- a/siammask_amd/csrc/conv_plan.h
+++ b/siammask_amd/csrc/conv_plan.h
@@ -91,10 +91,16 @@
     int B = 0;
     int nslots = 0;
     bool have_xch = false;
+    int lean_usable = ~0;
 };
 struct SeqPlanStats { int pairs = 0, triples = 0, resident = 0; };
+struct SeqSlice { int i0 = 0, n = 0, mask = smk::SEQ_R_ALL; };
 
-SeqPlanStats plan_seq(std::vector<SeqRec> &rec, const SeqPlanEnv &env, const char *locked, const std::vector<const void *> &read_after);
+SeqPlanStats plan_seq(std::vector<SeqRec> &rec, const SeqPlanEnv &env, const char *locked, const std::vector<const void *> &read_after,
+                      std::vector<SeqSlice> *slices = nullptr);
+constexpr int SEQ_CUT_MIN = 8;
+int seq_need_mask(const smk::SeqLayer *L, int i0, int i1);
+int seq_lean_mask_for(int need, int usable = ~0);
 double seq_fabric_bytes(const smk::SeqLayer *L, int n, int B, const void *late_read);
 
 #pragma GCC visibility pop
diff --git a/siammask_amd/csrc/conv_seq.hip b/siammask_amd/csrc/conv_seq.hip
--- a/siammask_amd/csrc/conv_seq.hip
+++ b/siammask_amd/csrc/conv_seq.hip
@@ -1,4 +1,5 @@
 #include <hip/hip_runtime.h>
+#include <cstdio>
 #include <type_traits>
 #include "smk_kernels.h"
 
@@ -69,8 +70,10 @@
     }
 };
 
-template <int NPW, int CLK = 0, int T3 = 0>
+constexpr int SEQ_VGPR_MAX = 248;
+template <int NPW, int CLK = 0, int T3 = 0, int RMASK = SEQ_R_ALL>
 __global__ __launch_bounds__((4 + NPW) * 64, 1) void conv_seq_kernel(const SeqArgs a) {
+    static_assert(T3 == 0 || RMASK == SEQ_R_ALL, "the extended instantiation carries every routine");
     constexpr int SEQ_LDS0 = (!T3 || WregLds<4, 3>::v > C3C1Lds<256, 1024, 256>::vx) ? WregLds<4, 3>::v : C3C1Lds<256, 1024, 256>::vx;
     constexpr int SEQ_LDS = SEQ_LDS0 > SEQ_YRES_BYTES + 2 * HALO_PB ? SEQ_LDS0 : SEQ_YRES_BYTES + 2 * HALO_PB;
     static_assert(4 * 64 * 68 * 4 <= 2 * HALO_PB && C3C1Lds<256, 1024, 256>::A_OFF == SEQ_YRES_BYTES && C3C1Lds<128, 512, 128>::A_OFF <= SEQ_YRES_BYTES, "resident Y");
@@ -108,6 +111,12 @@
         const bool fused = cfg == SEQ_CFG_C3C1_L3 || cfg == SEQ_CFG_C3C1_L2;
         const bool fused3 = cfg == SEQ_CFG_C2C3C1_L3 || cfg == SEQ_CFG_C2C3C1_L2;
         const bool halo = cfg == SEQ_CFG_HALO128 || cfg == SEQ_CFG_HALO64;
+        if constexpr (RMASK != SEQ_R_ALL) {
+            if (!(seq_routine_bit(cfg) & RMASK)) {
+                if (threadIdx.x == 0) seq_raise(a, 4);
+                return;
+            }
+        }
         const int bn = (cfg == 0 || cfg == 3 || cfg == 16 || cfg == 17) ? 256 : ((cfg == 2 || cfg == 9 || cfg == 18) ? 64 : 128);
         const int bm = (cfg == 3 || cfg == 4 || cfg == 9 || cfg == 16) ? 128 : 64;
         const int tilesN = (L.Nst + bn - 1) / bn;
@@ -162,20 +171,20 @@
                 if (T3 != 0 && fused3) {}
                 else if (fused) {
                     const int fm0 = img * hw + t * 32;
-                    if (cfg == SEQ_CFG_C3C1_L3) alive = c3c1_tile<256, 1024, 256, CLK>(L, a.L[li + 1], fm0, m_end, a.B * hw, slot, nslots, smem, tclk, w);
-                    else alive = c3c1_tile<128, 512, 128, CLK>(L, a.L[li + 1], fm0, m_end, a.B * hw, slot, nslots, smem, tclk, w);
+                    if (cfg == SEQ_CFG_C3C1_L3) { if constexpr ((RMASK & SEQ_R_PAIR_L3) != 0) alive = c3c1_tile<256, 1024, 256, CLK>(L, a.L[li + 1], fm0, m_end, a.B * hw, slot, nslots, smem, tclk, w); }
+                    else { if constexpr ((RMASK & SEQ_R_PAIR_L2) != 0) alive = c3c1_tile<128, 512, 128, CLK>(L, a.L[li + 1], fm0, m_end, a.B * hw, slot, nslots, smem, tclk, w); }
                 }
                 else if (halo) {
                     const int ty = t / halo_tn, hn0 = (t - ty * halo_tn) * 64;
                     const bool hi = (L.a_stage & SEQ_LDS_HI) != 0;
                     unsigned char *hsm = smem + (hi ? SEQ_YRES_BYTES : 0);
-                    if (cfg == SEQ_CFG_HALO128) alive = wreg_halo_tile<4, NPW, HALO_D128, HALO_SB128, CLK>(L, img, ty, hn0, hsm, tclk, slot, nslots, w, hi);
-                    else alive = wreg_halo_tile<2, NPW, HALO_D64, 0, CLK>(L, img, ty, hn0, hsm, tclk, slot, nslots, w, hi);
-                }
-                else if (cfg == 0) alive = wreg_tile<2, 4, 1, 3, 16, 2, NPW, CLK>(L, 0, m0, m_end, tn * 256, smem, tclk, kt0, w);
-                else if (cfg == 1) alive = wreg_tile<2, 2, 2, 3, 16, 2, NPW, CLK>(L, 0, m0, m_end, tn * 128, smem, tclk, kt0, w);
-                else if (cfg == 3) alive = wreg_tile<4, 4, 1, 3, 16, 1, NPW, CLK>(L, 0, m0, m_end, tn * 256, smem, tclk, kt0, w);
-                else if (cfg == 4) alive = wreg_tile<4, 2, 2, 3, 16, 1, NPW, CLK>(L, 0, m0, m_end, tn * 128, smem, tclk, kt0, w);
+                    if (cfg == SEQ_CFG_HALO128) { if constexpr ((RMASK & SEQ_R_HALO128) != 0) alive = wreg_halo_tile<4, NPW, HALO_D128, HALO_SB128, CLK>(L, img, ty, hn0, hsm, tclk, slot, nslots, w, hi); }
+                    else { if constexpr ((RMASK & SEQ_R_HALO64) != 0) alive = wreg_halo_tile<2, NPW, HALO_D64, 0, CLK>(L, img, ty, hn0, hsm, tclk, slot, nslots, w, hi); }
+                }
+                else if (cfg == 0) { if constexpr ((RMASK & SEQ_R_64x256) != 0) alive = wreg_tile<2, 4, 1, 3, 16, 2, NPW, CLK>(L, 0, m0, m_end, tn * 256, smem, tclk, kt0, w); }
+                else if (cfg == 1) { if constexpr ((RMASK & SEQ_R_64x128) != 0) alive = wreg_tile<2, 2, 2, 3, 16, 2, NPW, CLK>(L, 0, m0, m_end, tn * 128, smem, tclk, kt0, w); }
+                else if (cfg == 3) { if constexpr ((RMASK & SEQ_R_128x256) != 0) alive = wreg_tile<4, 4, 1, 3, 16, 1, NPW, CLK>(L, 0, m0, m_end, tn * 256, smem, tclk, kt0, w); }
+                else if (cfg == 4) { if constexpr ((RMASK & SEQ_R_128x128) != 0) alive = wreg_tile<4, 2, 2, 3, 16, 1, NPW, CLK>(L, 0, m0, m_end, tn * 128, smem, tclk, kt0, w); }
                 else if (T3 != 0 && cfg == 9) { if constexpr (T3 != 0) alive = wreg_tile<4, 1, 4, 3, 16, 2, NPW, CLK>(L, 0, m0, m_end, tn * 64, smem, tclk, kt0, w); }
                 else if (T3 != 0 && cfg == 5) { if constexpr (T3 != 0) alive = wreg_tile<2, 2, 2, 5, 16, 4, NPW, CLK>(L, 0, m0, m_end, tn * 128, smem, tclk, kt0, w); }
 #ifdef SMK_MEASURE
@@ -192,7 +201,7 @@
                 else if (cfg == 17) alive = wreg_tile<2, 4, 1, 3, 16 | 0x2000, 2, NPW, CLK>(L, 0, m0, m_end, tn * 256, smem, tclk, kt0, w);
                 else if (cfg == 18) alive = wreg_tile<2, 1, 4, 3, 16 | 0x2000, 2, NPW, CLK>(L, 0, m0, m_end, tn * 64, smem, tclk, kt0, w);
 #endif
-                else alive = wreg_tile<2, 1, 4, 3, 16, 2, NPW, CLK>(L, 0, m0, m_end, tn * 64, smem, tclk, kt0, w);
+                else { if constexpr ((RMASK & SEQ_R_64x64) != 0) alive = wreg_tile<2, 1, 4, 3, 16, 2, NPW, CLK>(L, 0, m0, m_end, tn * 64, smem, tclk, kt0, w); }
             }
         }
         if (clk) a.clk[1 + 2 * li] = wall_clock64();
@@ -273,7 +282,30 @@
     if (threadIdx.x == 0) out[blockIdx.x] = (int)(xcc & 0xf);
 }
 
-int launch_conv_seq(const SeqArgs &a_in, int grid, void *stream) {
+template <int RMASK, int CLK>
+static bool seq_lean_fits() {
+    static const bool fits = [] {
+        hipFuncAttributes fa;
+        if (hipFuncGetAttributes(&fa, reinterpret_cast<const void *>(&conv_seq_kernel<4, CLK, 0, RMASK>)) != hipSuccess) return false;
+        if (fa.numRegs > SEQ_VGPR_MAX)
+            fprintf(stderr, "[siammask_hip] conv_seq_kernel<mask %d%s> allocates %d VGPRs (limit %d): its lists run on the full kernel\n", RMASK,
+                    CLK ? ", stamps" : "", fa.numRegs, SEQ_VGPR_MAX);
+        return fa.numRegs <= SEQ_VGPR_MAX;
+    }();
+    return fits;
+}
+template <int RMASK>
+static void seq_launch_lean(const SeqArgs &a, int grid, void *stream, bool stamps, bool alone) {
+    if (stamps) {
+        if (alone || seq_lean_fits<RMASK, 1>()) hipLaunchKernelGGL((conv_seq_kernel<4, 1, 0, RMASK>), dim3(grid), dim3(512), 0, (hipStream_t)stream, a);
+        else hipLaunchKernelGGL((conv_seq_kernel<4, 1>), dim3(grid), dim3(512), 0, (hipStream_t)stream, a);
+    } else {
+        if (alone || seq_lean_fits<RMASK, 0>()) hipLaunchKernelGGL((conv_seq_kernel<4, 0, 0, RMASK>), dim3(grid), dim3(512), 0, (hipStream_t)stream, a);
+        else hipLaunchKernelGGL((conv_seq_kernel<4, 0>), dim3(grid), dim3(512), 0, (hipStream_t)stream, a);
+    }
+}
+
+int launch_conv_seq(const SeqArgs &a_in, int grid, void *stream, int rmask, bool alone) {
     if (a_in.n < 1 || a_in.n > SEQ_MAX || grid < 8 || (grid & 7) || !a_in.bar || !a_in.err) return -1;
     SeqArgs a = a_in;
     unsigned short ord = 0;
@@ -308,23 +340,35 @@
         const int cf = a.L[li].cfg;
         triples = triples || cf == SEQ_CFG_C2C3C1_L3 || cf == SEQ_CFG_C2C3C1_L2 || cf == SEQ_CFG_C3C1P_L3 || cf == SEQ_CFG_C3C1P_L2 || cf == 5 || cf == 9;
     }
+    const bool stamps = a.clk || a.clk2;
     if (triples) {
+        if (rmask != SEQ_R_ALL) return -1;
 #ifdef SMK_MEASURE
-        if (a.clk || a.clk2) hipLaunchKernelGGL((conv_seq_kernel<4, 1, 1>), dim3(grid), dim3(512), 0, (hipStream_t)stream, a);
+        if (stamps) hipLaunchKernelGGL((conv_seq_kernel<4, 1, 1>), dim3(grid), dim3(512), 0, (hipStream_t)stream, a);
         else hipLaunchKernelGGL((conv_seq_kernel<4, 0, 1>), dim3(grid), dim3(512), 0, (hipStream_t)stream, a);
 #else
         return -5;
 #endif
-    } else if (a.clk || a.clk2)
-        hipLaunchKernelGGL((conv_seq_kernel<4, 1>), dim3(grid), dim3(512), 0, (hipStream_t)stream, a);
-    else hipLaunchKernelGGL((conv_seq_kernel<4, 0>), dim3(grid), dim3(512), 0, (hipStream_t)stream, a);
+    } else if (rmask == SEQ_R_ALL) {
+        if (stamps) hipLaunchKernelGGL((conv_seq_kernel<4, 1>), dim3(grid), dim3(512), 0, (hipStream_t)stream, a);
+        else hipLaunchKernelGGL((conv_seq_kernel<4, 0>), dim3(grid), dim3(512), 0, (hipStream_t)stream, a);
+    } else if (rmask == SEQ_LEAN_L2) {
+        seq_launch_lean<SEQ_LEAN_L2>(a, grid, stream, stamps, alone);
+    } else if (rmask == SEQ_LEAN_L3) {
+        seq_launch_lean<SEQ_LEAN_L3>(a, grid, stream, stamps, alone);
+    } else return -1;
     return hipGetLastError() == hipSuccess ? 0 : -4;
 }
 
 int conv_seq_occupancy() {
     int nb = 0;
     if (hipOccupancyMaxActiveBlocksPerMultiprocessor(&nb, conv_seq_kernel<4, 0>, 512, 0) != hipSuccess) return 0;
+    (void)conv_seq_lean_usable();
     return nb;
+}
+
+int conv_seq_lean_usable() {
+    return (seq_lean_fits<SEQ_LEAN_L2, 0>() ? 1 : 0) | (seq_lean_fits<SEQ_LEAN_L3, 0>() ? 2 : 0);
 }
 
 int xcc_census(int grid, int *out_host) {
diff --git a/siammask_amd/csrc/engine.cpp b/siammask_amd/csrc/engine.cpp
--- a/siammask_amd/csrc/engine.cpp
+++ b/siammask_amd/csrc/engine.cpp
@@ -790,6 +790,7 @@
     return 0;
 }
 
+static std::vector<SeqSlice> g_host_slices;
 static SeqPlanStats g_seq_last;
 
 static void seq_print_clk(const SeqArgs &a, const SeqRec *r, const char *idn, const unsigned long long *h,
@@ -854,18 +855,20 @@
     const void *p2 = ACT(c, T_P2).p;
     std::vector<const void *> read_after{p2};
     for (int id : {c->p3_id, (int)T_SEARCH, (int)T_ZF, (int)T_XS}) read_after.push_back(ACT(c, id).p);
-    g_seq_last = plan_seq(c->seq.rec, {B, c->seq_grid >> 3, c->seq_xch != nullptr}, nullptr, read_after);
-    for (size_t i0 = 0; i0 < n; i0 += SEQ_MAX) {
+    std::vector<SeqSlice> slices;
+    g_seq_last = plan_seq(c->seq.rec, {B, c->seq_grid >> 3, c->seq_xch != nullptr, conv_seq_lean_usable()}, nullptr, read_after, &slices);
+    for (const SeqSlice &sl : slices) {
+        const size_t i0 = (size_t)sl.i0;
         SeqArgs a;
         memset(&a, 0, sizeof(a));
-        a.n = (int)(n - i0 < (size_t)SEQ_MAX ? n - i0 : SEQ_MAX);
+        a.n = sl.n;
         a.B = B;
         a.flags = g_tune.seq_spoll ? 1 : 0;
         a.bar = c->seq_bar;
         a.xch = c->seq_xch;
         a.err = c->seq_err;
         a.err_host = c->seq_err_hdev;
-        a.exit_sem = (rec.seq_exit && i0 + SEQ_MAX >= n) ? c->pipe_cnt + 7 : nullptr;
+        a.exit_sem = (rec.seq_exit && i0 + (size_t)sl.n >= n) ? c->pipe_cnt + 7 : nullptr;
         if (a.exit_sem) rec.seq_exit_done = true;
         const SeqRec *r = c->seq.rec.data() + i0;
         for (int i = 0; i < a.n; ++i) a.L[i] = r[i].L;
@@ -882,7 +885,7 @@
         const double fr = (double)a.n / (double)n;
         ProfScope ps(c, s, idn, "conv_seq", c->seq.flop * fr, c->seq.bytes * fr);
         ps.ext_bytes(seq_fabric_bytes(a.L, a.n, B, p2));
-        if (launch_conv_seq(a, c->seq_grid, s))
+        if (launch_conv_seq(a, c->seq_grid, s, sl.mask))
             return fail(SMK_E_HIP, "launch of %s failed: %s", idn, hipGetErrorString(hipGetLastError()));
         c->seq_pending = rec.has_seq = true;
         if (want_clk) {
@@ -929,8 +932,9 @@
     return fail(SMK_E_SEQ, "conv_seq_kernel reported %s: the results of the calls enqueued on this context since then are invalid "
                 "(the cached template included); persistent sequences are now off for this context (per-layer kernels from here "
                 "on): call template() again and re-submit the frame",
-                e == 1 ? "an uneven distribution of workgroups over the XCDs" : "a team-barrier time-out (another kernel held CUs "
-                "for more than 0.2 s, or a second persistent kernel ran beside it)");
+                e == 1 ? "an uneven distribution of workgroups over the XCDs"
+                : e == 4 ? "a record whose tile routine the launched instantiation does not carry (a planner bug)"
+                         : "a team-barrier time-out (another kernel held CUs for more than 0.2 s, or a second persistent kernel ran beside it)");
 }
 
 static bool seq_wanted(const smk_ctx *c, int B) {
@@ -1963,6 +1967,10 @@
     {"seq_fused3_last", &g_seq_last.triples, nullptr, KNOB_RAW, nullptr},
     {"measure_build", &g_measure_build, nullptr, KNOB_RAW, nullptr},
 };
+static const Knob KNOBS_LATER[] = {
+    {"seq_lean", &g_tune.seq_lean, "0..2", KNOB_RAW, nullptr},
+    {"seq_force_mask", &g_tune.seq_force_mask, "0..511", KNOB_RAW, nullptr},
+};
 
 static bool knob_accepts(const char *spec, int v) {
     if (!strcmp(spec, "*")) return true;
@@ -1980,6 +1988,8 @@
 
 static const Knob *find_knob(const char *key) {
     for (const Knob &k : KNOBS)
+        if (!strcmp(key, k.name)) return &k;
+    for (const Knob &k : KNOBS_LATER)
         if (!strcmp(key, k.name)) return &k;
     return nullptr;
 }
@@ -2655,14 +2665,15 @@
     return 0;
 }
 
-static SeqPlanStats plan_seq_ops(const smk_seq_op *ops, std::vector<SeqRec> &rec, const std::vector<Act> &outs, int grid) {
+static SeqPlanStats plan_seq_ops(const smk_seq_op *ops, std::vector<SeqRec> &rec, const std::vector<Act> &outs, int grid,
+                                 std::vector<SeqSlice> *slices = nullptr) {
     std::vector<char> locked(rec.size());
     std::vector<const void *> read_after;
     for (size_t i = 0; i < rec.size(); ++i) {
         locked[i] = ops[i].cfg >= 0;
         if (ops[i].y_dev) read_after.push_back(outs[i].p);
     }
-    return plan_seq(rec, {ops[0].g.B, grid >> 3, true}, locked.data(), read_after);
+    return plan_seq(rec, {ops[0].g.B, grid >> 3, true}, locked.data(), read_after, slices);
 }
 
 int smk_op_conv_seq(const smk_seq_op *ops, int n, const float *x_dev, int iters, float *usec_out, float *clk_us_out,
@@ -2710,7 +2721,10 @@
     std::vector<SeqRec> rec;
     std::vector<Act> outs;
     CHK(seq_op_records(ops, n, xin, dev, pack, [&](void **p, size_t bytes) { return tmp.alloc(p, bytes); }, rec, outs));
-    g_seq_last = plan_seq_ops(ops, rec, outs, grid);
+    std::vector<SeqSlice> slices;
+    g_seq_last = plan_seq_ops(ops, rec, outs, grid, &slices);
+    if (g_tune.seq_force_mask)
+        for (SeqSlice &sl : slices) sl.mask = g_tune.seq_force_mask;
     SeqArgs a;
     memset(&a, 0, sizeof(a));
     a.n = n; a.B = B;
@@ -2724,7 +2738,8 @@
     CHK(tmp.alloc((void **)&clk, sizeof(unsigned long long) * (2 * SEQ_MAX + 1)));
     const char *ck = getenv("SMK_SEQ_CLK");
     const bool want2 = ck && !strcmp(ck, "2");
-    if (want2) CHK(tmp.alloc((void **)&clk2, sizeof(unsigned long long) * (12 + 32) * SEQ_MAX));
+    constexpr size_t CLK2_N = (size_t)(12 + 32) * SEQ_MAX;
+    if (want2) CHK(tmp.alloc((void **)&clk2, sizeof(unsigned long long) * CLK2_N * slices.size()));
     float *xch = nullptr;
     CHK(tmp.alloc((void **)&xch, SEQ_XCH_BYTES));
     a.bar = bar; a.xch = xch; a.err = err; a.err_host = nullptr; a.clk = clk; a.clk2 = clk2;
@@ -2735,14 +2750,24 @@
     hipEvent_t e0, e1;
     HIPCHK(hipEventCreate(&e0));
     HIPCHK(hipEventCreate(&e1));
-    SeqArgs a_run = a;
-    a_run.clk = nullptr; a_run.clk2 = nullptr;
-    if (launch_conv_seq(a_run, grid, s)) return fail(SMK_E_HIP, "conv_seq launch failed: %s", hipGetErrorString(hipGetLastError()));
+    auto launch_list = [&](bool stamps) -> int {
+        for (size_t si = 0; si < slices.size(); ++si) {
+            const SeqSlice &sl = slices[si];
+            SeqArgs as = a;
+            as.n = sl.n;
+            for (int i = 0; i < sl.n; ++i) as.L[i] = a.L[sl.i0 + i];
+            as.clk = clk + 2 * sl.i0;
+            as.clk2 = clk2 ? clk2 + CLK2_N * si : nullptr;
+            if (!stamps) { as.clk = nullptr; as.clk2 = nullptr; }
+            if (launch_conv_seq(as, grid, s, sl.mask, true)) return fail(SMK_E_HIP, "conv_seq launch failed: %s", hipGetErrorString(hipGetLastError()));
+        }
+        return 0;
+    };
+    CHK(launch_list(false));
     HIPCHK(hipEventRecord(e0, s));
-    for (int it = 1; it < iters; ++it)
-        if (launch_conv_seq(a_run, grid, s)) return fail(SMK_E_HIP, "conv_seq launch failed: %s", hipGetErrorString(hipGetLastError()));
+    for (int it = 1; it < iters; ++it) CHK(launch_list(false));
     HIPCHK(hipEventRecord(e1, s));
-    if (launch_conv_seq(a, grid, s)) return fail(SMK_E_HIP, "conv_seq launch failed: %s", hipGetErrorString(hipGetLastError()));
+    CHK(launch_list(true));
     HIPCHK(hipStreamSynchronize(s));
     float ms = 0.f;
     if (iters > 1) HIPCHK(hipEventElapsedTime(&ms, e0, e1));
@@ -2750,6 +2775,7 @@
     if (usec_out) *usec_out = iters > 1 ? ms * 1000.f / (iters - 1) : 0.f;
     int e = 0;
     HIPCHK(hipMemcpy(&e, err, sizeof(int), hipMemcpyDeviceToHost));
+    if (e == 4) return fail(SMK_E_SEQ, "conv_seq_kernel reported a record whose tile routine the launched instantiation does not carry");
     if (e) return fail(SMK_E_HIP, "conv_seq_kernel reported %s", e == 1 ? "an uneven distribution of workgroups over the XCDs" : "a team-barrier time-out");
     {
         unsigned long long h[2 * SEQ_MAX + 1], h2[(12 + 32) * SEQ_MAX];
@@ -2760,7 +2786,17 @@
                 clk_us_out[2 * i + 1] = (float)((h[2 + 2 * i] - h[1 + 2 * i]) / 100.0);
             }
         if (ck) {
-            if (want2) HIPCHK(hipMemcpy(h2, clk2, sizeof(h2), hipMemcpyDeviceToHost));
+            if (want2) {
+                std::vector<unsigned long long> hs(CLK2_N);
+                memset(h2, 0, sizeof(h2));
+                for (size_t si = 0; si < slices.size(); ++si) {
+                    HIPCHK(hipMemcpy(hs.data(), clk2 + CLK2_N * si, sizeof(unsigned long long) * CLK2_N, hipMemcpyDeviceToHost));
+                    for (int i = 0; i < slices[si].n; ++i) {
+                        memcpy(h2 + 12 * (slices[si].i0 + i), hs.data() + 12 * i, 12 * sizeof(unsigned long long));
+                        memcpy(h2 + 12 * SEQ_MAX + 32 * (slices[si].i0 + i), hs.data() + 12 * SEQ_MAX + 32 * i, 32 * sizeof(unsigned long long));
+                    }
+                }
+            }
             seq_print_clk(a, rec.data(), "smk_op_conv_seq", h, want2 ? h2 : nullptr);
         }
     }
@@ -3694,13 +3730,25 @@
     std::vector<Act> outs;
     CHK(seq_op_records(ops, n, xin, -1, [](int, PackedConv &pc) { fake_pack(pc, DT_F16); return 0; },
                        [&](void **p, size_t) { *p = tensors + next++; return 0; }, rec, outs));
-    plan_seq_ops(ops, rec, outs, grid);
+    std::vector<SeqSlice> slices;
+    plan_seq_ops(ops, rec, outs, grid, &slices);
     for (int i = 0; i < n; ++i) {
         cfg[i] = rec[i].L.cfg;
         sync[i] = rec[i].L.sync;
         a_stage[i] = rec[i].L.a_stage;
     }
-    return 0;
+    g_host_slices = slices;
+    return 0;
+}
+
+int smk_host_plan_seq_slices(int *first, int *count, int *mask, int cap) {
+    if (!first || !count || !mask || cap < 0) return fail(SMK_E_ARG, "smk_host_plan_seq_slices: null argument");
+    for (size_t j = 0; j < g_host_slices.size() && (int)j < cap; ++j) {
+        first[j] = g_host_slices[j].i0;
+        count[j] = g_host_slices[j].n;
+        mask[j] = g_host_slices[j].mask;
+    }
+    return (int)g_host_slices.size();
 }
 
 int smk_host_arena_elems(int dtype, int variant, int pipe_depth, uint64_t *elems_per_image) {
diff --git a/siammask_amd/csrc/smk_kernels.h b/siammask_amd/csrc/smk_kernels.h
--- a/siammask_amd/csrc/smk_kernels.h
+++ b/siammask_amd/csrc/smk_kernels.h
@@ -113,6 +113,16 @@
 constexpr int SEQ_YRES_IN = 2, SEQ_YRES_NOSTORE = 4, SEQ_LDS_HI = 8;
 constexpr int SEQ_YRES_BYTES = 65536;
 constexpr int SEQ_MAX = 36;
+constexpr int SEQ_R_64x256 = 1, SEQ_R_64x128 = 2, SEQ_R_64x64 = 4, SEQ_R_128x256 = 8, SEQ_R_128x128 = 16;
+constexpr int SEQ_R_HALO128 = 32, SEQ_R_HALO64 = 64, SEQ_R_PAIR_L3 = 128, SEQ_R_PAIR_L2 = 256, SEQ_R_ALL = 511;
+constexpr int SEQ_LEAN_L2 = SEQ_R_64x256 | SEQ_R_128x128 | SEQ_R_64x64 | SEQ_R_HALO64 | SEQ_R_PAIR_L2;
+constexpr int SEQ_LEAN_L3 = SEQ_R_64x256 | SEQ_R_128x256 | SEQ_R_64x128 | SEQ_R_HALO128 | SEQ_R_PAIR_L3;
+constexpr int SEQ_LEAN_MASKS[2] = {SEQ_LEAN_L2, SEQ_LEAN_L3};
+constexpr int seq_routine_bit(int cfg) {
+    return cfg == 0 ? SEQ_R_64x256 : cfg == 1 ? SEQ_R_64x128 : cfg == 2 ? SEQ_R_64x64 : cfg == 3 ? SEQ_R_128x256 : cfg == 4 ? SEQ_R_128x128
+         : cfg == SEQ_CFG_HALO128 ? SEQ_R_HALO128 : cfg == SEQ_CFG_HALO64 ? SEQ_R_HALO64
+         : cfg == SEQ_CFG_C3C1_L3 ? SEQ_R_PAIR_L3 : cfg == SEQ_CFG_C3C1_L2 ? SEQ_R_PAIR_L2 : 0;
+}
 struct SeqArgs {
     int n, B;
     int flags, pad_;
@@ -173,6 +183,8 @@
     int seq_ds128 = 0;
     int seq_deep = 0;
     int seq_first_stage = 1;
+    int seq_lean = 2;
+    int seq_force_mask = 0;
     int wreg_policy = 1;
     int npw = 4;
     int a_stage = 0;
@@ -334,7 +346,8 @@
 int launch_conv_wreg_batch(ConvBatch &cb, int bm, int bn, int stages, void *stream);
 bool conv_pp_eligible(const ConvParams &p, int dtype);
 int launch_conv_pp(const ConvParams &p, void *stream);
-int launch_conv_seq(const SeqArgs &a, int grid, void *stream);
+int launch_conv_seq(const SeqArgs &a, int grid, void *stream, int rmask = SEQ_R_ALL, bool alone = false);
+int conv_seq_lean_usable();
 int launch_conv_pair(const SeqLayer &L3, const SeqLayer &L1, int code, int M, void *stream, int rows);
 int conv_seq_occupancy();
 int xcc_census(int grid, int *out_host);
diff --git a/siammask_amd/ops.py b/siammask_amd/ops.py
--- a/siammask_amd/ops.py
+++ b/siammask_amd/ops.py
@@ -140,6 +140,16 @@
     return list(zip(*[list(o) for o in out]))
 
 
+def plan_seq_slices(x_shape, layers, want_outputs=True, grid=256):
+    marks = plan_seq(x_shape, layers, want_outputs, grid)
+    cap = len(layers)
+    out = [(ctypes.c_int * cap)() for _ in range(3)]
+    ns = _lib.lib().smk_host_plan_seq_slices(*out, cap)
+    if ns < 0:
+        _lib.check(ns)
+    return marks, [(out[0][j], out[1][j], out[2][j]) for j in range(ns)]
+
+
 def dw_xcorr(x, k, dtype="f32"):
     _chk_cuda(x, k)
     x, k = x.contiguous().float(), k.contiguous().float()
```

Result: no change. 14800 (-0.3%).
